# DJjjjhao/FIRA-ICSE

Measured on NVIDIA H100. Metric: train_commits_per_sec, higher is better.
Workload: dtype bf16

## Files before the change

fira_icse_b200/csrc/attention.cu:

```cuda
#include <stdlib.h>
#include "attn_mma.cuh"
#include "common.cuh"
#include "fira_b200.h"

namespace {

bool use_tc(int dtype) {
  if (dtype != FIRA_BF16) return false;
  const char* e = getenv("FIRA_ATTN_TC");
  return e ? atoi(e) != 0 : true;
}

constexpr int KPAD = DH + 1;
constexpr int NWARPS = 8;
constexpr int NTHR = NWARPS * 32;
constexpr int KC = 128;
constexpr int KCB = 64;

template <typename T>
__device__ __forceinline__ void load_rows(float* dst, const T* src, long ld, const int* rows_idx, int row0, int nrows) {
  constexpr int EPV = 16 / sizeof(T);
  constexpr int VPR = DH / EPV;
#pragma unroll 4
  for (int idx = threadIdx.x; idx < nrows * VPR; idx += NTHR) {
// ... 262 lines not shown
  for (int i = 0; i < nblk; ++i) {
    cp_async_wait<FST - 1>();
    __syncthreads();
    const unsigned char* kt = Ks + (i % FST) * FKB * ROWB;
    const unsigned char* vt = Vs + (i % FST) * FKB * ROWB;
    const int c0 = i * FKB;
    float s[8][4];
#pragma unroll
    for (int n = 0; n < 8; ++n) s[n][0] = s[n][1] = s[n][2] = s[n][3] = 0.f;
    mma_abt(s, qa, kt, lane);
    softmax_pv(s, rk, a.causal, c0, nv, k2, m, l, o, vt, lane);
    __syncthreads();
    if (i + FST < nblk)
      stage_kv(Ks + (i % FST) * FKB * ROWB, Vs + (i % FST) * FKB * ROWB, kh, a.ldk, vh, a.ldv, kidx, (i + FST) * FKB,
               min(FKB, nv - (i + FST) * FKB), FKB, threadIdx.x, blockDim.x);
    cp_async_commit();
  }
  softmax_finish(o, l, m, rk, t, a.Lq, stats ? stats + ((long)b * a.H + h) * a.Lq * 2 : nullptr, lane);
#pragma unroll
  for (int r = 0; r < 2; ++r) {
    if (t[r] >= a.Lq) continue;
    __nv_bfloat16* dst = ctx + ((long)b * a.Lq + t[r]) * ldo + h * DH + 2 * q;
#pragma unroll
    for (int n = 0; n < 4; ++n)
      *reinterpret_cast<__nv_bfloat162*>(dst + 8 * n) = __floats2bfloat162_rn(o[n][2 * r], o[n][2 * r + 1]);
  }
}

__global__ void __launch_bounds__(BWARPS * 32, 1)
attn_mma_bwd_kernel(AttnArgs a, const __nv_bfloat16* __restrict__ out, const __nv_bfloat16* __restrict__ d_ctx, long ldo,
                    const float* __restrict__ stats, __nv_bfloat16* __restrict__ dq, long lddq,
                    __nv_bfloat16* __restrict__ dk, long lddk, __nv_bfloat16* __restrict__ dv, long lddv) {
  pdl_wait(); pdl_trigger();
  extern __shared__ __align__(16) unsigned char mma_smem[];
  __shared__ int nv_s, filled_s;
  __shared__ float delta_s[LQ_MAX], m2_s[LQ_MAX], inv_s[LQ_MAX];
  unsigned char* Qs = mma_smem;
  unsigned char* Os = Qs + LQ_MAX * ROWB;
  unsigned char* Ws = Os + LQ_MAX * ROWB;
  int* kidx = reinterpret_cast<int*>(Ws + BWARPS * BWARP_SMEM);
  const int b = blockIdx.x / a.H, h = blockIdx.x % a.H;
  const int lane = threadIdx.x & 31, warp = threadIdx.x >> 5, q = lane & 3;
  const unsigned char* km = a.key_mask ? a.key_mask + (long)b * a.Lk : nullptr;
  const int* rg = a.ranges ? a.ranges + 4 * b : nullptr;
  const long kvb = rg ? 0 : (long)b * a.Lk;
  const __nv_bfloat16* kh = (const __nv_bfloat16*)a.k + kvb * a.ldk + h * DH;
  const __nv_bfloat16* vh = (const __nv_bfloat16*)a.v + kvb * a.ldv + h * DH;
  unsigned char* Kw = Ws + warp * BWARP_SMEM;
  unsigned char* Vw = Kw + BKB * ROWB;
  unsigned char* Pw = Vw + BKB * ROWB;
  unsigned char* Sw = Pw + LQ_MAX * ROWB;
  float* dQw = reinterpret_cast<float*>(Sw + LQ_MAX * ROWB);
  compact_keys(km, a.Lk, a.causal, kidx, &nv_s, &filled_s, rg);
  const int nv = nv_s;
  const bool filled = filled_s != 0;
  if (warp * BKB < nv) stage_kv(Kw, Vw, kh, a.ldk, vh, a.ldv, kidx, warp * BKB, min(BKB, nv - warp * BKB), BKB, lane, 32);
  for (int i = threadIdx.x; i < 2 * LQ_MAX * 4; i += blockDim.x) {
    const int which = i / (LQ_MAX * 4), r = (i >> 2) & (LQ_MAX - 1), c = i & 3;
    unsigned char* dst = (which ? Os : Qs) + swz(r, c);
    if (r < a.Lq) cp_async16(su32(dst), which ? d_ctx + ((long)b * a.Lq + r) * ldo + h * DH + c * 8
                                              : (const __nv_bfloat16*)a.q + ((long)b * a.Lq + r) * a.ldq + h * DH + c * 8);
    else *reinterpret_cast<uint4*>(dst) = make_uint4(0, 0, 0, 0);
  }
  cp_async_commit();
  if (threadIdx.x < a.Lq) {
    const int t = threadIdx.x;
    const __nv_bfloat16* orow = out + ((long)b * a.Lq + t) * ldo + h * DH;
    const __nv_bfloat16* grow = d_ctx + ((long)b * a.Lq + t) * ldo + h * DH;
    float d = 0.f;
#pragma unroll
    for (int c = 0; c < 4; ++c) {
      float ov[8], gv[8];
      Act<__nv_bfloat16>::load8(orow + c * 8, ov);
      Act<__nv_bfloat16>::load8(grow + c * 8, gv);
#pragma unroll
      for (int e = 0; e < 8; ++e) d = fmaf(ov[e], gv[e], d);
    }
    const float* st = stats + (((long)b * a.H + h) * a.Lq + t) * 2;
    delta_s[t] = d; m2_s[t] = st[0] * kLog2e; inv_s[t] = 1.f / st[1];
  }
  if (!filled && !a.causal && km) {
    const int L = rg ? rg[1] + rg[3] : a.Lk;
    for (int s0 = 32 * warp; s0 < L; s0 += 32 * BWARPS) {
      uint32_t dead = __ballot_sync(0xffffffffu, s0 + lane < L && km[s0 + lane] == 0);
      while (dead) {
        const int s = s0 + __ffs(dead) - 1;
        dead &= dead - 1;
        const long row = rg ? (s < rg[1] ? rg[0] + s : rg[2] + (s - rg[1])) : (long)b * a.Lk + s;
        dk[row * lddk + h * DH + lane] = __float2bfloat16_rn(0.f);
        dv[row * lddv + h * DH + lane] = __float2bfloat16_rn(0.f);
      }
    }
  }
  cp_async_wait<0>();
  __syncthreads();

  const float k2 = a.scale * kLog2e;
  const uint32_t mb = causal_mask_bits(a, km, lane);
  for (int i = lane; i < LQ_MAX * DH / 4; i += 32) reinterpret_cast<float4*>(dQw)[i] = make_float4(0.f, 0.f, 0.f, 0.f);

  for (int blk = warp; blk * BKB < nv; blk += BWARPS) {
    const int c0 = blk * BKB, nc = min(BKB, nv - c0);
    if (blk != warp) {
      __syncwarp();
      stage_kv(Kw, Vw, kh, a.ldk, vh, a.ldv, kidx, c0, nc, BKB, lane, 32);
      cp_async_commit();
      cp_async_wait<0>();
    }
    __syncwarp();
#pragma unroll
    for (int mt = 0; mt < 2; ++mt) {
// ... 72 lines not shown
#pragma unroll
      for (int kk = 0; kk < 2; ++kk) {
        if (16 * kk >= a.Lq) break;
#pragma unroll
        for (int mk = 0; mk < 2; ++mk) {
          uint32_t at[4];
          ldsm4_t(su32(At + swz(16 * kk + (lane & 7) + (lane >> 4) * 8, 2 * mk + ((lane >> 3) & 1))), at);
          mma_ax(acc[mk], at, Bt, kk, lane);
        }
      }
      __nv_bfloat16* dst = which ? dv : dk;
      const long ld = which ? lddv : lddk;
#pragma unroll
      for (int mk = 0; mk < 2; ++mk)
#pragma unroll
        for (int r = 0; r < 2; ++r) {
          const int j = 16 * mk + (lane >> 2) + 8 * r;
          if (j < nc) {
            __nv_bfloat16* row = dst + (kvb + kidx[c0 + j]) * ld + h * DH + 2 * q;
#pragma unroll
            for (int n = 0; n < 4; ++n)
              *reinterpret_cast<__nv_bfloat162*>(row + 8 * n) = __floats2bfloat162_rn(acc[mk][n][2 * r], acc[mk][n][2 * r + 1]);
          }
        }
    }
  }
  __syncthreads();
  for (int i = threadIdx.x; i < a.Lq * DH; i += blockDim.x) {
    const int t = i / DH, f = i % DH;
    float x = 0.f;
#pragma unroll
    for (int w = 0; w < BWARPS; ++w)
      x += reinterpret_cast<const float*>(Ws + w * BWARP_SMEM + 4 * BKB * ROWB)[swz_f32(t, f)];
    dq[((long)b * a.Lq + t) * lddq + h * DH + f] = __float2bfloat16_rn(x);
  }
}

size_t fwd_smem(int Lk) { return (size_t)2 * FST * FKB * ROWB + sizeof(int) * (size_t)Lk; }
size_t bwd_smem(int Lk) { return (size_t)2 * LQ_MAX * ROWB + (size_t)BWARPS * BWARP_SMEM + sizeof(int) * (size_t)Lk; }

}

size_t fwd_smem(int Lq, int Lk) {
  return sizeof(float) * ((size_t)2 * KC * KPAD + (size_t)Lq * KPAD + (size_t)NWARPS * 2 * KC) + sizeof(int) * (size_t)Lk;
}
size_t bwd_smem(int Lq, int Lk) {
  return sizeof(float) * ((size_t)2 * KCB * KPAD + (size_t)2 * Lq * KPAD + (size_t)2 * Lq * (KCB + 1)) +
         sizeof(int) * (size_t)Lk;
}

template <typename K>
int set_smem(K kernel, size_t bytes, const char* name) {
  if (bytes > 227 * 1024) {
    fira_set_error(FIRA_ERR_SHAPE, "%s: needs %zu B shared memory (> 227 KB)", name, bytes);
    return FIRA_ERR_SHAPE;
  }
  if (bytes > 48 * 1024) {
    cudaError_t e = cudaFuncSetAttribute(kernel, cudaFuncAttributeMaxDynamicSharedMemorySize, (int)bytes);
    if (e != cudaSuccess) { fira_set_error(FIRA_ERR_CUDA, "%s: %s", name, cudaGetErrorString(e)); return FIRA_ERR_CUDA; }
  }
  return FIRA_OK;
}

int check_layout(const char* name, const void* p, long ld, int dtype) {
  const long esz = dtype == FIRA_F32 ? 4 : 2;
  if ((reinterpret_cast<uintptr_t>(p) & 15) != 0 || (ld * esz) % 16 != 0) {
    fira_set_error(FIRA_ERR_ALIGN, "%s: operands must be 16-B aligned with 16-B row pitch", name);
// ... 10 lines not shown
                  const unsigned char* key_mask, const int* ranges, int causal, void* ctx, long ldo, float* stats, int B, int H, int Lq, int Lk, int d_head, int dtype, void* stream) {
  FIRA_CHECK_ARG(d_head == DH, FIRA_ERR_SHAPE, "attn_fwd: d_head %d != 32", d_head);
  FIRA_CHECK_ARG(B > 0 && H > 0 && Lq > 0 && Lk > 0 && Lq <= LQ_MAX, FIRA_ERR_SHAPE, "attn_fwd: shape (Lq <= 32)");
  FIRA_CHECK_ARG(!causal || (Lq == Lk && !ranges), FIRA_ERR_SHAPE, "attn_fwd: causal needs Lq == Lk and no ranges");
  FIRA_CHECK_ARG(key_mask || ranges, FIRA_ERR_ARG, "attn_fwd: key_mask may only be NULL with ranges");
  FIRA_CHECK_ARG(dtype == FIRA_F32 || dtype == FIRA_BF16, FIRA_ERR_DTYPE, "attn_fwd: dtype %d", dtype);
  int rc;
  if ((rc = check_layout("attn_fwd", q, ldq, dtype)) || (rc = check_layout("attn_fwd", k, ldk, dtype)) ||
      (rc = check_layout("attn_fwd", v, ldv, dtype)))
    return rc;
  AttnArgs a{q, ldq, k, ldk, v, ldv, key_mask, ranges, causal, B, H, Lq, Lk, 1.f / sqrtf((float)d_head)};
  if (use_tc(dtype)) {
    const size_t smem = mma::fwd_smem(Lk);
    if ((rc = set_smem(mma::attn_mma_fwd_kernel, smem, "attn_fwd"))) return rc;
    launch_k(mma::attn_mma_fwd_kernel, dim3(B * H), dim3(32 * ((Lq + 15) / 16)), smem, (cudaStream_t)stream, a,
             (__nv_bfloat16*)ctx, ldo, stats);
    FIRA_CHECK_LAUNCH("fira_attn_fwd (mma)");
    return FIRA_OK;
  }
  const size_t smem = fwd_smem(Lq, Lk);
  if (dtype == FIRA_F32) {
    if ((rc = set_smem(attn_fwd_kernel<float>, smem, "attn_fwd"))) return rc;
    launch_k(attn_fwd_kernel<float>, dim3(B * H), dim3(NTHR), smem, (cudaStream_t)stream, a, (float*)ctx, ldo, stats);
  } else {
    if ((rc = set_smem(attn_fwd_kernel<__nv_bfloat16>, smem, "attn_fwd"))) return rc;
    launch_k(attn_fwd_kernel<__nv_bfloat16>, dim3(B * H), dim3(NTHR), smem, (cudaStream_t)stream, a, (__nv_bfloat16*)ctx, ldo, stats);
  }
  FIRA_CHECK_LAUNCH("fira_attn_fwd");
  return FIRA_OK;
}

int attn_bwd_impl(const void* q, long ldq, const void* k, long ldk, const void* v, long ldv,
                  const unsigned char* key_mask, const int* ranges, int causal, const void* ctx, const void* d_ctx, long ldo, const float* stats, void* dq, long lddq, void* dk,
                  long lddk, void* dv, long lddv, int B, int H, int Lq, int Lk, int d_head, int dtype, void* stream) {
  FIRA_CHECK_ARG(d_head == DH, FIRA_ERR_SHAPE, "attn_bwd: d_head %d != 32", d_head);
  FIRA_CHECK_ARG(B > 0 && H > 0 && Lq > 0 && Lk > 0 && Lq <= LQ_MAX, FIRA_ERR_SHAPE, "attn_bwd: shape (Lq <= 32)");
  FIRA_CHECK_ARG(key_mask || ranges, FIRA_ERR_ARG, "attn_bwd: key_mask may only be NULL with ranges");
  FIRA_CHECK_ARG(dtype == FIRA_F32 || dtype == FIRA_BF16, FIRA_ERR_DTYPE, "attn_bwd: dtype %d", dtype);
  int rc;
  if ((rc = check_layout("attn_bwd", q, ldq, dtype)) || (rc = check_layout("attn_bwd", k, ldk, dtype)) ||
      (rc = check_layout("attn_bwd", v, ldv, dtype)) || (rc = check_layout("attn_bwd", ctx, ldo, dtype)) ||
      (rc = check_layout("attn_bwd", d_ctx, ldo, dtype)))
    return rc;
  AttnArgs a{q, ldq, k, ldk, v, ldv, key_mask, ranges, causal, B, H, Lq, Lk, 1.f / sqrtf((float)d_head)};
  if (use_tc(dtype) && (lddk % 8) == 0 && (lddv % 8) == 0 && (lddq % 8) == 0) {
    const size_t smem = mma::bwd_smem(Lk);
    if ((rc = set_smem(mma::attn_mma_bwd_kernel, smem, "attn_bwd"))) return rc;
    launch_k(mma::attn_mma_bwd_kernel, dim3(B * H), dim3(mma::BWARPS * 32), smem, (cudaStream_t)stream, a,
             (const __nv_bfloat16*)ctx, (const __nv_bfloat16*)d_ctx, ldo, stats, (__nv_bfloat16*)dq, lddq,
             (__nv_bfloat16*)dk, lddk, (__nv_bfloat16*)dv, lddv);
    FIRA_CHECK_LAUNCH("fira_attn_bwd (mma)");
    return FIRA_OK;
  }
  const size_t smem = bwd_smem(Lq, Lk);
  if (dtype == FIRA_F32) {
    if ((rc = set_smem(attn_bwd_kernel<float>, smem, "attn_bwd"))) return rc;
    launch_k(attn_bwd_kernel<float>, dim3(B * H), dim3(NTHR), smem, (cudaStream_t)stream, 
        a, (const float*)ctx, (const float*)d_ctx, ldo, stats, (float*)dq, lddq, (float*)dk, lddk, (float*)dv, lddv);
  } else {
    if ((rc = set_smem(attn_bwd_kernel<__nv_bfloat16>, smem, "attn_bwd"))) return rc;
    launch_k(attn_bwd_kernel<__nv_bfloat16>, dim3(B * H), dim3(NTHR), smem, (cudaStream_t)stream, 
        a, (const __nv_bfloat16*)ctx, (const __nv_bfloat16*)d_ctx, ldo, stats, (__nv_bfloat16*)dq, lddq,
        (__nv_bfloat16*)dk, lddk, (__nv_bfloat16*)dv, lddv);
  }
  FIRA_CHECK_LAUNCH("fira_attn_bwd");
  return FIRA_OK;
}

}

extern "C" {

int fira_attn_fwd(const void* q, long ldq, const void* k, long ldk, const void* v, long ldv,
                  const unsigned char* key_mask, int causal, void* ctx, long ldo, float* stats, int B, int H, int Lq,
                  int Lk, int d_head, int dtype, void* stream) {
  FIRA_CHECK_ARG(key_mask, FIRA_ERR_ARG, "attn_fwd: null key_mask");
  return attn_fwd_impl(q, ldq, k, ldk, v, ldv, key_mask, nullptr, causal, ctx, ldo, stats,
                       B, H, Lq, Lk, d_head, dtype, stream);
}

int fira_attn_bwd(const void* q, long ldq, const void* k, long ldk, const void* v, long ldv,
                  const unsigned char* key_mask, int causal, const void* ctx, const void* d_ctx, long ldo,
                  const float* stats, void* dq, long lddq, void* dk, long lddk, void* dv, long lddv, int B, int H,
                  int Lq, int Lk, int d_head, int dtype, void* stream) {
  FIRA_CHECK_ARG(key_mask, FIRA_ERR_ARG, "attn_bwd: null key_mask");
  return attn_bwd_impl(q, ldq, k, ldk, v, ldv, key_mask, nullptr, causal, ctx, d_ctx, ldo,
                       stats, dq, lddq, dk, lddk, dv, lddv, B, H, Lq, Lk, d_head, dtype, stream);
}

int fira_attn_packed_fwd(const void* q, long ldq, const void* k, long ldk, const void* v, long ldv, const int* ranges,
                         long kv_rows, const unsigned char* key_mask, int mask_pitch, int max_chunks, void* ctx, long ldo,
                         float* stats, int B, int H, int Lq, int d_head, int dtype, void* stream) {
  FIRA_CHECK_ARG(ranges && kv_rows > 0, FIRA_ERR_ARG, "attn_packed_fwd: ranges / kv_rows");
  return attn_fwd_impl(q, ldq, k, ldk, v, ldv, key_mask, ranges, 0, ctx, ldo, stats, B, H, Lq,
                       mask_pitch, d_head, dtype, stream);
}

int fira_attn_packed_bwd(const void* q, long ldq, const void* k, long ldk, const void* v, long ldv, const int* ranges,
                         long kv_rows, const unsigned char* key_mask, int mask_pitch, int max_chunks, const void* ctx,
                         const void* d_ctx, long ldo, const float* stats, void* dq, long lddq, void* dk, long lddk,
                         void* dv, long lddv, int B, int H, int Lq, int d_head, int dtype, void* stream) {
  FIRA_CHECK_ARG(ranges && kv_rows > 0, FIRA_ERR_ARG, "attn_packed_bwd: ranges / kv_rows");
  return attn_bwd_impl(q, ldq, k, ldk, v, ldv, key_mask, ranges, 0, ctx, d_ctx, ldo, stats, dq, lddq,
                       dk, lddk, dv, lddv, B, H, Lq, mask_pitch, d_head, dtype, stream);
}

}
```

fira_icse_b200/csrc/attn_mma.cuh:

```cuda
#pragma once
#include "common.cuh"

namespace {

constexpr int DH = 32;
constexpr int LQ_MAX = 32;

struct AttnArgs {
  const void* q; long ldq;
  const void* k; long ldk;
  const void* v; long ldv;
  const unsigned char* key_mask;
  const int* ranges;
  int causal;
  int B, H, Lq, Lk;
  float scale;
};

__device__ __forceinline__ void compact_keys(const unsigned char* km, int Lk, int causal, int* kidx, int* nv_out,
                                             int* filled, const int* rg = nullptr) {
  if (threadIdx.x < 32) {
    const int lane = threadIdx.x;
    const int L = rg ? rg[1] + rg[3] : Lk;
    int n = 0;
    for (int s0 = 0; s0 < L && !causal; s0 += 32) {
      const int s = s0 + lane;
      const bool ok = s < L && (km == nullptr || km[s] != 0);
      const unsigned bal = __ballot_sync(0xffffffffu, ok);
      if (ok) kidx[n + __popc(bal & ((1u << lane) - 1u))] = rg ? (s < rg[1] ? rg[0] + s : rg[2] + (s - rg[1])) : s;
      n += __popc(bal);
    }
    if (n == 0) {
      for (int s = lane; s < L; s += 32) kidx[s] = rg ? (s < rg[1] ? rg[0] + s : rg[2] + (s - rg[1])) : s;
      n = L;
      if (lane == 0) *filled = causal ? 0 : 1;
    } else if (lane == 0) *filled = 0;
    if (lane == 0) *nv_out = n;
  }
  __syncthreads();
}

namespace mma {

constexpr int ROWB = DH * 2;
constexpr float kLog2e = 1.4426950408889634f;

__device__ __forceinline__ uint32_t swz(int r, int c) { return r * ROWB + ((c ^ ((r >> 1) & 3)) << 4); }
__device__ __forceinline__ uint32_t su32(const void* p) { return (uint32_t)__cvta_generic_to_shared(p); }

// ... 157 lines not shown
```

fira_icse_b200/csrc/decoder_fwd.cu:

```cuda
#include <string.h>
#include <cooperative_groups.h>
#include "attn_mma.cuh"
#include "common.cuh"
#include "fira_b200.h"

namespace {

namespace cg = cooperative_groups;
using namespace mma;
using bf16 = __nv_bfloat16;

constexpr int D = 256, F = 1024, NH = 8;
constexpr int TP = 32;
constexpr int NWARP = 16, NTHR = NWARP * 32;
constexpr int LDA = D + 32, LDF = F + 32;
constexpr int XT = TP * LDA * 2;
constexpr int HT = TP * ROWB;
constexpr int CKB = 32;
constexpr int MAX_LAYERS = 8;

struct LayerW {
  const bf16* wqkv; const float* bqkv;
  const bf16* swo; const float* sbo; const float* slw; const float* slb;
  const bf16* cwq; const float* cbq;
  const bf16* cwo; const float* cbo; const float* clw; const float* clb;
  const bf16* w1; const float* b1; const bf16* w2; const float* b2;
  const float* flw; const float* flb;
};
static_assert(sizeof(LayerW) == 18 * sizeof(void*), "LayerW is the host's [L][18] pointer table");

struct DecParams {
  const int* tar; const float* emb; const float* pe; const unsigned char* tar_mask;
  const bf16* kv; long ldkv;
  const unsigned char* mem_mask; const int* ranges; int S;
  bf16* X;
  bf16* qkv; bf16* ctx1; float* st1; bf16* z1; float* ls1; bf16* x1;
  bf16* q; bf16* ctx2; float* st2; bf16* z2; float* ls2; bf16* x2;
  bf16* hh; bf16* z3; float* ls3;
  int B, T, L;
  float scale, p_drop;
  uint64_t seed; const uint64_t* seed_ctr; uint32_t stream_id;
  LayerW w[MAX_LAYERS];
};

constexpr int OFF_X = 0, OFF_X1 = XT, OFF_X2 = 2 * XT, OFF_Y = 3 * XT, OFF_Z = 4 * XT, OFF_BIG = 5 * XT;
constexpr int BIG_BYTES = TP * LDF * 2;
static_assert(BIG_BYTES >= 12 * HT && BIG_BYTES >= 4 * HT + 2 * 2 * 4 * CKB * ROWB,
              "the region also holds the q|k|v head tiles of four heads, and their q tiles + two K / V stages");
constexpr int SMEM_FIXED = OFF_BIG + BIG_BYTES;

__device__ __forceinline__ uint32_t word(const uint4& v, int i) { return i == 0 ? v.x : i == 1 ? v.y : i == 2 ? v.z : v.w; }
__device__ __forceinline__ uint4 ldg16(const bf16* p) { return __ldg(reinterpret_cast<const uint4*>(p)); }
__device__ __forceinline__ void pair_bar(int h) { asm volatile("bar.sync %0, 64;" ::"r"(1 + h) : "memory"); }

template <int K, int NT8, int PF>
__device__ __forceinline__ void warp_mma(float (&acc)[2][NT8][4], const bf16* As, const bf16* __restrict__ W, int n0,
                                         int lane) {
  constexpr int lda = K + 32;
  const int g = lane >> 2, q = lane & 3;
#pragma unroll
  for (int mt = 0; mt < 2; ++mt)
#pragma unroll
    for (int j = 0; j < NT8; ++j) acc[mt][j][0] = acc[mt][j][1] = acc[mt][j][2] = acc[mt][j][3] = 0.f;
  const bf16* wp = W + (long)(n0 + g) * K + 8 * q;
  const bf16* ap = As + g * lda + 8 * q;
  constexpr int nks = K / 32;
  uint4 bq[PF][NT8];
#pragma unroll
  for (int s = 0; s < PF; ++s)
#pragma unroll
    for (int j = 0; j < NT8; ++j) bq[s][j] = ldg16(wp + (long)8 * j * K + 32 * s);
// ... 33 lines not shown
  for (int n0 = 8 * NT8 * warp; n0 < N / 2; n0 += 8 * NT8 * NWARP) {
    const int c0 = gcol(n0, rank);
    float acc[2][NT8][4];
    warp_mma<K, NT8, PF>(acc, As, W, c0, lane);
#pragma unroll
    for (int j = 0; j < NT8; ++j) {
      const int n = n0 + 8 * j + 2 * q, c = c0 + 8 * j + 2 * q;
      const float2 bb = *reinterpret_cast<const float2*>(bias + c);
#pragma unroll
      for (int mt = 0; mt < 2; ++mt)
#pragma unroll
        for (int hr = 0; hr < 2; ++hr) {
          float v0 = acc[mt][j][2 * hr] + bb.x, v1 = acc[mt][j][2 * hr + 1] + bb.y;
          if (RELU) { v0 = fmaxf(v0, 0.f); v1 = fmaxf(v1, 0.f); }
          epi(16 * mt + 8 * hr + g, n, c, pack_bf16(v0, v1));
        }
    }
  }
}

__device__ __forceinline__ uint32_t head_off(int t, int n) {
  return (n >> 5) * HT + swz(t, (n & 31) >> 3) + (n & 7) * 2;
}

template <typename Src>
__device__ __forceinline__ void copy_out(bf16* __restrict__ dst, int N, int T, int rank, int warp, int lane, Src src) {
  for (int t = warp; t < T; t += NWARP)
    for (int n = 8 * lane; n < N / 2; n += 256)
      *reinterpret_cast<uint4*>(dst + (long)t * N + gcol(n, rank)) = *reinterpret_cast<const uint4*>(src(t, n));
}

__device__ __forceinline__ void ln_rows(const unsigned char* sm, int off_z, int off_res, int off_out, const float* gamma,
                                        const float* beta, bf16* __restrict__ zg, bf16* __restrict__ og,
                                        float* __restrict__ stats, long rows, long r0, int T, float p_drop, uint64_t seed,
                                        const uint64_t* seed_ctr, uint32_t sid, int rank, int warp, int lane) {
  if (seed_ctr) seed += *seed_ctr;
  float g[8], bt[8];
  Act<float>::load8(gamma + lane * 8, g);
  Act<float>::load8(beta + lane * 8, bt);
  const float keep_scale = p_drop > 0.f ? 1.f / (1.f - p_drop) : 1.f;
  for (int t = 2 * warp; t < 2 * warp + 2; ++t) {
    const int o = (t * LDA + lane * 8) * 2;
    bf16* os = (bf16*)(sm + off_out + o);
    if (t >= T) { *reinterpret_cast<uint4*>(os) = make_uint4(0, 0, 0, 0); continue; }
    const long r = r0 + t;
    const bool mine = (t & 1) == rank;
    const uint4 zraw = *reinterpret_cast<const uint4*>(sm + off_z + o);
    if (mine) *reinterpret_cast<uint4*>(zg + r * D + lane * 8) = zraw;
    float y[8], x[8];
    Act<bf16>::load8((const bf16*)&zraw, y);
    Act<bf16>::load8((const bf16*)(sm + off_res + o), x);
    if (p_drop > 0.f) {
      uint32_t m = dropout_keep8(seed, sid, (uint64_t)r * 32 + lane, p_drop);
#pragma unroll
      for (int i = 0; i < 8; ++i) y[i] = ((m >> i) & 1) ? y[i] * keep_scale : 0.f;
    }
    float s = 0.f;
#pragma unroll
    for (int i = 0; i < 8; ++i) { y[i] += x[i]; s += y[i]; }
    const float mean = warp_sum(s) * (1.f / D);
    float qv = 0.f;
#pragma unroll
    for (int i = 0; i < 8; ++i) { float d = y[i] - mean; qv += d * d; }
    const float rstd = rsqrtf(warp_sum(qv) * (1.f / D) + kLnEps);
#pragma unroll
    for (int i = 0; i < 8; ++i) y[i] = (y[i] - mean) * rstd * g[i] + bt[i];
    Act<bf16>::store8(os, y);
    if (mine) {
      *reinterpret_cast<uint4*>(og + r * D + lane * 8) = *reinterpret_cast<const uint4*>(os);
      if (lane == 0) { stats[r] = mean; stats[rows + r] = rstd; }
    }
  }
}

struct AttnRows {
  int t[2];
  RowKeys rk[2];
  float m[2], l[2], o[4][4];
  uint32_t qa[2][4];
  __device__ __forceinline__ void init(const unsigned char* qtile, int r0, int lane) {
    ld_a(qtile, r0, lane, qa);
    m[0] = m[1] = -INFINITY;
    l[0] = l[1] = 0.f;
#pragma unroll
    for (int n = 0; n < 4; ++n) o[n][0] = o[n][1] = o[n][2] = o[n][3] = 0.f;
#pragma unroll
    for (int r = 0; r < 2; ++r) t[r] = r0 + (lane >> 2) + 8 * r;
  }
  __device__ __forceinline__ void block(const unsigned char* kt, const unsigned char* vt, int causal, int c0, int nv,
                                        float k2, int lane) {
    float s[4][4];
#pragma unroll
    for (int n = 0; n < 4; ++n) s[n][0] = s[n][1] = s[n][2] = s[n][3] = 0.f;
    mma_abt(s, qa, kt, lane);
    softmax_pv(s, rk, causal, c0, nv, k2, m, l, o, vt, lane);
  }
  __device__ __forceinline__ void finish(unsigned char* ytile, unsigned char* ytile_peer, int h, int T, float* st,
                                         int lane) {
    softmax_finish(o, l, m, rk, t, T, st, lane);
#pragma unroll
    for (int r = 0; r < 2; ++r)
#pragma unroll
      for (int n = 0; n < 4; ++n) {
        const int off = (t[r] * LDA + h * DH + 8 * n + 2 * (lane & 3)) * 2;
        const uint32_t v = pack_bf16(o[n][2 * r], o[n][2 * r + 1]);
        *reinterpret_cast<uint32_t*>(ytile + off) = v;
        *reinterpret_cast<uint32_t*>(ytile_peer + off) = v;
      }
  }
};

__global__ void __cluster_dims__(2, 1, 1) __launch_bounds__(NTHR, 1)
decoder_fwd_kernel(const __grid_constant__ DecParams p) {
  pdl_wait(); pdl_trigger();
  extern __shared__ __align__(16) unsigned char sm[];
  __shared__ int nv_s, filled_s;
  cg::cluster_group cluster = cg::this_cluster();
  const int rank = (int)cluster.block_rank();
  unsigned char* peer = cluster.map_shared_rank(sm, rank ^ 1);
  const int b = blockIdx.x >> 1, T = p.T;
  const int lane = threadIdx.x & 31, warp = threadIdx.x >> 5, hl = (warp >> 1) & 3, r0q = 16 * (warp & 1);
  const long Mt = (long)p.B * T, grow0 = (long)b * T;
  int* kidx = reinterpret_cast<int*>(sm + SMEM_FIXED);
  bf16* Xs = (bf16*)(sm + OFF_X);
  bf16* Ys = (bf16*)(sm + OFF_Y);
  unsigned char* big = sm + OFF_BIG;
  auto to_both = [&](int off, uint32_t v) {
    *reinterpret_cast<uint32_t*>(sm + off) = v;
    *reinterpret_cast<uint32_t*>(peer + off) = v;
  };

  compact_keys(p.mem_mask ? p.mem_mask + (long)b * p.S : nullptr, p.S, 0, kidx, &nv_s, &filled_s,
               p.ranges ? p.ranges + 4 * b : nullptr);

  for (int t = warp; t < TP; t += NWARP) {
    float v[8];
    if (t < T) {
      float pe[8];
      Act<float>::load8(p.emb + (long)p.tar[grow0 + t] * D + lane * 8, v);
      Act<float>::load8(p.pe + (long)t * D + lane * 8, pe);
#pragma unroll
      for (int i = 0; i < 8; ++i) v[i] += pe[i];
      if ((t & 1) == rank) Act<bf16>::store8(p.X + (grow0 + t) * D + lane * 8, v);
    } else {
#pragma unroll
      for (int i = 0; i < 8; ++i) v[i] = 0.f;
    }
    Act<bf16>::store8(Xs + t * LDA + lane * 8, v);
  }
  cluster.sync();

  for (int i = 0; i < p.L; ++i) {
    const LayerW& w = p.w[i];
    const long o256 = i * Mt * D;

    product<D, 1, 8, false>(Xs, w.wqkv, w.bqkv, 3 * D, rank, warp, lane,
                            [&](int t, int n, int, uint32_t v) { *reinterpret_cast<uint32_t*>(big + head_off(t, n)) = v; });
    __syncthreads();
    copy_out(p.qkv + (i * Mt + grow0) * 3 * D, 3 * D, T, rank, warp, lane, [&](int t, int n) { return big + head_off(t, n); });
    if (warp < 8) {
      AttnArgs sa{};
      sa.causal = 1;
      sa.Lk = T;
      const uint32_t mb = causal_mask_bits(sa, p.tar_mask + grow0, lane);
      AttnRows ar;
      ar.init(big + hl * HT, r0q, lane);
#pragma unroll
      for (int r = 0; r < 2; ++r) ar.rk[r] = row_keys(sa, mb, T, false, ar.t[r]);
      ar.block(big + (4 + hl) * HT, big + (8 + hl) * HT, 1, 0, T, p.scale * kLog2e, lane);
      const int h = 4 * rank + hl;
      ar.finish(sm + OFF_Y, peer + OFF_Y, h, T, p.st1 + (((long)i * p.B + b) * NH + h) * T * 2, lane);
    }
    cluster.sync();
    copy_out(p.ctx1 + o256 + grow0 * D, D, T, rank, warp, lane, [&](int t, int n) { return Ys + t * LDA + gcol(n, rank); });
    product<D, 1, 8, false>(Ys, w.swo, w.sbo, D, rank, warp, lane,
                            [&](int t, int, int c, uint32_t v) { to_both(OFF_Z + (t * LDA + c) * 2, v); });
    cluster.sync();
    ln_rows(sm, OFF_Z, OFF_X, OFF_X1, w.slw, w.slb, p.z1 + o256, p.x1 + o256, p.ls1 + 2 * i * Mt, Mt, grow0, T,
            p.p_drop, p.seed, p.seed_ctr, p.stream_id + 8 * i + 0, rank, warp, lane);
    __syncthreads();

    product<D, 1, 8, false>((const bf16*)(sm + OFF_X1), w.cwq, w.cbq, D, rank, warp, lane,
                            [&](int t, int n, int, uint32_t v) { *reinterpret_cast<uint32_t*>(big + head_off(t, n)) = v; });
    __syncthreads();
    copy_out(p.q + o256 + grow0 * D, D, T, rank, warp, lane, [&](int t, int n) { return big + head_off(t, n); });
    if (warp < 8) {
      const int h = 4 * rank + hl;
      const int nv = nv_s, nblk = (nv + CKB - 1) / CKB;
      const float k2 = p.scale * kLog2e;
      const long kvb = p.ranges ? 0 : (long)b * p.S;
      const bf16* kh = p.kv + kvb * p.ldkv + (long)i * 2 * D + h * DH;
      const bf16* vh = kh + D;
      unsigned char* stage = big + 4 * HT;
      auto kt = [&](int s) { return stage + ((s * 2 + 0) * 4 + hl) * CKB * ROWB; };
      auto vt = [&](int s) { return stage + ((s * 2 + 1) * 4 + hl) * CKB * ROWB; };
      const int tid = threadIdx.x & 63;
#pragma unroll
      for (int s = 0; s < 2; ++s) {
        if (s < nblk) stage_kv(kt(s), vt(s), kh, p.ldkv, vh, p.ldkv, kidx, s * CKB, min(CKB, nv - s * CKB), CKB, tid, 64);
        cp_async_commit();
      }
      AttnRows ar;
      ar.init(big + hl * HT, r0q, lane);
      ar.rk[0] = ar.rk[1] = RowKeys{0u, filled_s != 0};
      for (int blk = 0; blk < nblk; ++blk) {
        cp_async_wait<1>();
        pair_bar(hl);
        ar.block(kt(blk & 1), vt(blk & 1), 0, blk * CKB, nv, k2, lane);
        pair_bar(hl);
        if (blk + 2 < nblk)
          stage_kv(kt(blk & 1), vt(blk & 1), kh, p.ldkv, vh, p.ldkv, kidx, (blk + 2) * CKB,
                   min(CKB, nv - (blk + 2) * CKB), CKB, tid, 64);
        cp_async_commit();
      }
      ar.finish(sm + OFF_Y, peer + OFF_Y, h, T, p.st2 + (((long)i * p.B + b) * NH + h) * T * 2, lane);
    }
    cluster.sync();
    copy_out(p.ctx2 + o256 + grow0 * D, D, T, rank, warp, lane, [&](int t, int n) { return Ys + t * LDA + gcol(n, rank); });
    product<D, 1, 8, false>(Ys, w.cwo, w.cbo, D, rank, warp, lane,
                            [&](int t, int, int c, uint32_t v) { to_both(OFF_Z + (t * LDA + c) * 2, v); });
    cluster.sync();
    ln_rows(sm, OFF_Z, OFF_X1, OFF_X2, w.clw, w.clb, p.z2 + o256, p.x2 + o256, p.ls2 + 2 * i * Mt, Mt, grow0, T,
            p.p_drop, p.seed, p.seed_ctr, p.stream_id + 8 * i + 1, rank, warp, lane);
    __syncthreads();

    bf16* Hs = (bf16*)big;
    product<D, 2, 4, true>((const bf16*)(sm + OFF_X2), w.w1, w.b1, F, rank, warp, lane,
                           [&](int t, int, int c, uint32_t v) { to_both(OFF_BIG + (t * LDF + c) * 2, v); });
    cluster.sync();
    copy_out(p.hh + (i * Mt + grow0) * F, F, T, rank, warp, lane, [&](int t, int n) { return Hs + t * LDF + gcol(n, rank); });
    product<F, 1, 8, false>(Hs, w.w2, w.b2, D, rank, warp, lane,
                            [&](int t, int, int c, uint32_t v) { to_both(OFF_Z + (t * LDA + c) * 2, v); });
    cluster.sync();
    ln_rows(sm, OFF_Z, OFF_X2, OFF_X, w.flw, w.flb, p.z3 + o256, p.X + o256 + Mt * D, p.ls3 + 2 * i * Mt, Mt, grow0, T,
            p.p_drop, p.seed, p.seed_ctr, p.stream_id + 8 * i + 2, rank, warp, lane);
    __syncthreads();
  }
}

}

extern "C" int fira_decoder_fwd(const int* tar, const float* dec_emb, const float* pos_table,
                                const unsigned char* tar_mask, const void* kv, long ldkv, const unsigned char* mem_mask,
                                const int* ranges, int S, const void* const* layer_ptrs, int L, void* X, void* qkv,
                                void* ctx1, float* st1, void* z1, float* ls1, void* x1, void* q, void* ctx2, float* st2,
                                void* z2, float* ls2, void* x2, void* hh, void* z3, float* ls3, int B, int T,
                                float p_drop, uint64_t seed, const uint64_t* seed_ctr, uint32_t stream_id,
                                void* stream) {
  FIRA_CHECK_ARG(B > 0 && T > 0 && T <= TP, FIRA_ERR_SHAPE, "decoder_fwd: B %d, T %d (T <= 32)", B, T);
  FIRA_CHECK_ARG(L > 0 && L <= MAX_LAYERS, FIRA_ERR_SHAPE, "decoder_fwd: %d layers (1..%d)", L, MAX_LAYERS);
  FIRA_CHECK_ARG(S > 0, FIRA_ERR_SHAPE, "decoder_fwd: S %d", S);
  FIRA_CHECK_ARG(mem_mask || ranges, FIRA_ERR_ARG, "decoder_fwd: mem_mask may only be NULL with ranges");
  FIRA_CHECK_ARG(layer_ptrs && tar && dec_emb && pos_table && tar_mask && kv, FIRA_ERR_ARG, "decoder_fwd: null input");
  FIRA_CHECK_ARG(fira_aligned16(kv) && ldkv % 8 == 0 && ldkv >= (long)L * 2 * D, FIRA_ERR_ALIGN,
                 "decoder_fwd: kv must be 16-B aligned with ldkv a multiple of 8 and >= L*512");
  void* outs[] = {X, qkv, ctx1, z1, x1, q, ctx2, z2, x2, hh, z3};
  for (void* o : outs) FIRA_CHECK_ARG(o && fira_aligned16(o), FIRA_ERR_ALIGN, "decoder_fwd: outputs must be 16-B aligned");
  FIRA_CHECK_ARG(st1 && ls1 && st2 && ls2 && ls3, FIRA_ERR_ARG, "decoder_fwd: null statistics");
  DecParams p{tar, dec_emb, pos_table, tar_mask, (const bf16*)kv, ldkv, mem_mask, ranges, S,
              (bf16*)X, (bf16*)qkv, (bf16*)ctx1, st1, (bf16*)z1, ls1, (bf16*)x1,
              (bf16*)q, (bf16*)ctx2, st2, (bf16*)z2, ls2, (bf16*)x2, (bf16*)hh, (bf16*)z3, ls3,
              B, T, L, 1.f / sqrtf((float)DH), p_drop, seed, seed_ctr, stream_id, {}};
  for (int i = 0; i < L; ++i) {
    const void* const* t = layer_ptrs + 18 * i;
    for (int j = 0; j < 18; ++j)
      FIRA_CHECK_ARG(t[j] && fira_aligned16(t[j]), FIRA_ERR_ALIGN, "decoder_fwd: layer %d pointer %d null or unaligned", i, j);
    memcpy(&p.w[i], t, sizeof(LayerW));
  }
  const size_t smem = SMEM_FIXED + sizeof(int) * (size_t)S;
  FIRA_CHECK_ARG(smem <= 227 * 1024, FIRA_ERR_SHAPE, "decoder_fwd: S %d needs %zu B shared memory", S, smem);
  cudaError_t e = cudaFuncSetAttribute(decoder_fwd_kernel, cudaFuncAttributeMaxDynamicSharedMemorySize, (int)smem);
  if (e != cudaSuccess) { fira_set_error(FIRA_ERR_CUDA, "decoder_fwd: %s", cudaGetErrorString(e)); return FIRA_ERR_CUDA; }
  launch_k(decoder_fwd_kernel, dim3(2 * B), dim3(NTHR), smem, (cudaStream_t)stream, p);
  FIRA_CHECK_LAUNCH("fira_decoder_fwd");
  return FIRA_OK;
}
```

fira_icse_b200/csrc/head.cu:

```cuda
#include "common.cuh"
#include "fira_b200.h"

namespace {

constexpr int D = 256;
constexpr int TMAX = 32;

__device__ __forceinline__ long src_row(const int* __restrict__ ranges, int b, int S, int s) {
  if (!ranges) return (long)b * S + s;
  const int* r = ranges + 4 * b;
  if (s < r[1]) return r[0] + s;
  s -= r[1];
  return s < r[3] ? (long)(r[2] + s) : -1;
}

template <typename T>
__global__ void __launch_bounds__(256) copy_scores_fwd_kernel(const T* __restrict__ src, const T* __restrict__ tgt,
                                                              const float* __restrict__ w_res,
                                                              const float* __restrict__ b_res_p,
                                                              const unsigned char* __restrict__ src_mask,
                                                              const unsigned char* __restrict__ row_mask,
                                                              const int* __restrict__ ranges,
                                                              float* __restrict__ sc, int B, int Tn, int S) {
  pdl_wait(); pdl_trigger();
// ... 143 lines not shown
    u.s = __shfl_xor_sync(0xffffffffu, v.s, o);
    v = ms_merge(v, u);
  }
  return v;
}
struct ArgMax { float v; int i; };
__device__ __forceinline__ ArgMax am_better(ArgMax a, ArgMax b) {
  return (b.v > a.v || (b.v == a.v && b.i < a.i)) ? b : a;
}

constexpr int kRowsThreads = 1024;
__global__ void __launch_bounds__(kRowsThreads) vocab_rows_kernel(const int* __restrict__ label, long rows, int V,
                                                                  int* __restrict__ vslot, int* __restrict__ vrows,
                                                                  int cap) {
  pdl_wait(); pdl_trigger();
  __shared__ int warp_sum_s[kRowsThreads / 32];
  const int lane = threadIdx.x & 31, warp = threadIdx.x >> 5;
  const long per = (rows + kRowsThreads - 1) / kRowsThreads;
  const long r0 = min(rows, (long)threadIdx.x * per), r1 = min(rows, r0 + per);
  int n = 0;
  for (long r = r0; r < r1; ++r) n += (label[r] != 0 && label[r] < V);
  int incl = n;
#pragma unroll
  for (int o = 1; o < 32; o <<= 1) { const int u = __shfl_up_sync(0xffffffffu, incl, o); if (lane >= o) incl += u; }
  if (lane == 31) warp_sum_s[warp] = incl;
  for (int s = threadIdx.x; s < cap; s += kRowsThreads) vrows[s] = -1;
  __syncthreads();
  int slot = incl - n;
  for (int w = 0; w < warp; ++w) slot += warp_sum_s[w];
  for (long r = r0; r < r1; ++r) {
    const bool v = label[r] != 0 && label[r] < V && slot < cap;
    vslot[r] = v ? slot : -1;
    if (v) vrows[slot++] = (int)r;
  }
}

template <typename T>
__global__ void __launch_bounds__(256) gather_rows_kernel(const T* __restrict__ src, long ld_src,
                                                          const int* __restrict__ idx, T* __restrict__ dst, long ld_dst,
                                                          long n, int width) {
  pdl_wait(); pdl_trigger();
  const int lane = threadIdx.x & 31;
  for (long i = (long)blockIdx.x * 8 + (threadIdx.x >> 5); i < n; i += (long)gridDim.x * 8) {
    const int r = idx[i];
    for (int c = lane * 8; c < width; c += 256) {
      float x[8] = {0.f, 0.f, 0.f, 0.f, 0.f, 0.f, 0.f, 0.f};
      if (r >= 0) Act<T>::load8(src + (long)r * ld_src + c, x);
      Act<T>::store8(dst + i * ld_dst + c, x);
    }
  }
}

template <typename T>
__global__ void __launch_bounds__(256) head_fwd_kernel(const T* __restrict__ logits, long ldl,
                                                       const float* __restrict__ sc, const float* __restrict__ gate_logit,
                                                       const unsigned char* __restrict__ mem_mask,
                                                       const int* __restrict__ label, const int* __restrict__ vslot,
                                                       float* __restrict__ stats, float* __restrict__ nll,
                                                       int* __restrict__ argmax_out, int Tn, int V, int S) {
  pdl_wait(); pdl_trigger();
  __shared__ MaxSum sh_ms[8];
  __shared__ ArgMax sh_am[8];
  __shared__ float bc[8];
  const long row = blockIdx.x;
  const int b = (int)(row / Tn);
  const int lane = threadIdx.x & 31, warp = threadIdx.x >> 5;
// ... 775 lines not shown
                         const unsigned char* src_mask, const unsigned char* row_mask, float* scores,
                         int B, int T_len, int S, int dim, int dtype, void* stream) {
  return copy_scores_fwd_impl(src_proj, tgt_proj, w_res, b_res, src_mask, row_mask, nullptr, scores, B, T_len, S, dim,
                              dtype, stream);
}

int fira_copy_scores_bwd(const void* src_proj, const void* tgt_proj, const float* w_res, const float* d_scores,
                         const unsigned char* row_active, void* d_src_proj, float* d_tgt_proj, float* d_w_res,
                         float* d_b_res, int B, int T_len, int S, int dim, int dtype, void* stream) {
  return copy_scores_bwd_impl(src_proj, tgt_proj, w_res, d_scores, row_active, nullptr, d_src_proj, d_tgt_proj, d_w_res,
                              d_b_res, B, T_len, S, dim, dtype, stream);
}

int fira_copy_scores_packed_fwd(const void* src_proj, const void* tgt_proj, const float* w_res, const float* b_res,
                                const int* ranges, const unsigned char* src_mask, const unsigned char* row_mask,
                                float* scores, int B, int T_len, int S, int dim, int dtype, void* stream) {
  FIRA_CHECK_ARG(ranges, FIRA_ERR_ARG, "copy_scores_packed_fwd: null ranges");
  return copy_scores_fwd_impl(src_proj, tgt_proj, w_res, b_res, src_mask, row_mask, ranges, scores, B, T_len, S, dim,
                              dtype, stream);
}

int fira_copy_scores_packed_bwd(const void* src_proj, const void* tgt_proj, const float* w_res, const float* d_scores,
                                const unsigned char* row_active, const int* ranges, void* d_src_proj, float* d_tgt_proj,
                                float* d_w_res, float* d_b_res, int B, int T_len, int S, int dim, int dtype, void* stream) {
  FIRA_CHECK_ARG(ranges, FIRA_ERR_ARG, "copy_scores_packed_bwd: null ranges");
  return copy_scores_bwd_impl(src_proj, tgt_proj, w_res, d_scores, row_active, ranges, d_src_proj, d_tgt_proj, d_w_res,
                              d_b_res, B, T_len, S, dim, dtype, stream);
}

int fira_vocab_rows(const int* label, long rows, int V, int* vslot, int* vrows, int cap, void* stream) {
  FIRA_CHECK_ARG(label && vslot && vrows && rows >= 0 && V > 0 && cap >= 0, FIRA_ERR_ARG, "vocab_rows: arguments");
  launch_k(vocab_rows_kernel, dim3(1), dim3(kRowsThreads), 0, (cudaStream_t)stream, label, rows, V, vslot, vrows, cap);
  FIRA_CHECK_LAUNCH("fira_vocab_rows");
  return FIRA_OK;
}

int fira_gather_rows(const void* src, long ld_src, const int* idx, void* dst, long ld_dst, long n, int width, int dtype,
                     void* stream) {
  FIRA_CHECK_ARG(idx && n >= 0 && width > 0 && width % 8 == 0 && ld_src >= width && ld_dst >= width, FIRA_ERR_ARG,
                 "gather_rows: arguments");
  FIRA_CHECK_ARG(fira_aligned16(src) && fira_aligned16(dst) && ld_src % 8 == 0 && ld_dst % 8 == 0, FIRA_ERR_ALIGN,
                 "gather_rows: 16-B alignment");
  if (n == 0) return FIRA_OK;
  const long g = (n + 7) / 8, gmax = (long)fira_num_sms() * 16;
  DISPATCH_T(dtype, launch_k(gather_rows_kernel<T>, dim3((unsigned)(g < gmax ? g : gmax)), dim3(256), 0,
      (cudaStream_t)stream, (const T*)src, ld_src, idx, (T*)dst, ld_dst, n, width);)
  FIRA_CHECK_LAUNCH("fira_gather_rows");
  return FIRA_OK;
}

int fira_pointer_mix_nll_fwd_rows(const void* logits, long ld_logits, const float* copy_scores, const float* gate_logits,
                                  const unsigned char* mem_mask, const int* label, const int* vslot, float* stats,
                                  float* nll, int* argmax_out, long rows, int T_len, int V, int S, int dtype,
                                  void* stream) {
  FIRA_CHECK_ARG(rows >= 0 && T_len > 0 && V > 0 && S > 0, FIRA_ERR_SHAPE, "pointer_mix_nll_fwd: shape");
  FIRA_CHECK_ARG(fira_aligned16(logits) && ld_logits % 8 == 0, FIRA_ERR_ALIGN,
                 "pointer_mix_nll_fwd: logits must be 16-byte aligned with a leading dimension that is a multiple of 8");
  FIRA_CHECK_ARG(!(vslot && argmax_out), FIRA_ERR_ARG, "pointer_mix_nll_fwd: the argmax needs the logits of every row");
  if (rows == 0) return FIRA_OK;
  DISPATCH_T(dtype, launch_k(head_fwd_kernel<T>, dim3((unsigned)rows), dim3(256), 0, (cudaStream_t)stream,
      (const T*)logits, ld_logits, copy_scores, gate_logits, mem_mask, label, vslot, stats, nll, argmax_out, T_len, V,
      S);)
  FIRA_CHECK_LAUNCH("fira_pointer_mix_nll_fwd");
  return FIRA_OK;
}

// ... 289 lines not shown
```

fira_icse_b200/csrc/rowops.cu:

```cuda
#include "common.cuh"
#include "fira_b200.h"

namespace {

constexpr int D = 256;
constexpr int ROWS_PER_CTA = 8;
constexpr int CTA = ROWS_PER_CTA * kWarp;

__host__ inline int row_grid(long rows) {
  long g = (rows + ROWS_PER_CTA - 1) / ROWS_PER_CTA;
  const long cap = (long)fira_num_sms() * 16;
  return (int)(g < cap ? (g > 0 ? g : 1) : cap);
}

template <typename T>
__global__ void embed_nodes_kernel(const int* __restrict__ sou, const int* __restrict__ sub, const int* __restrict__ ast,
                                   const float* __restrict__ emb, const float* __restrict__ ast_emb,
                                   const float* __restrict__ pe, const int* __restrict__ pos_idx,
                                   T* __restrict__ out_code, T* __restrict__ out_rest, int B, int n_code, int n_sub,
                                   int n_ast) {
  pdl_wait(); pdl_trigger();
  const long R = (long)B * (n_code + n_sub + n_ast);
  const int lane = threadIdx.x & 31;
  for (long r = (long)blockIdx.x * ROWS_PER_CTA + (threadIdx.x >> 5); r < R; r += (long)gridDim.x * ROWS_PER_CTA) {
// ... 24 lines not shown
                                       float* __restrict__ d_ast_emb, int B, int n_code, int n_sub, int n_ast) {
  pdl_wait(); pdl_trigger();
  const long R = (long)B * (n_code + n_sub + n_ast);
  const int lane = threadIdx.x & 31;
  for (long r = (long)blockIdx.x * ROWS_PER_CTA + (threadIdx.x >> 5); r < R; r += (long)gridDim.x * ROWS_PER_CTA) {
    int id; float* dst; const T* g;
    if (r < (long)B * n_code) { id = sou[r]; dst = d_emb; g = d_code + r * D; }
    else if (r < (long)B * (n_code + n_sub)) { id = sub[r - (long)B * n_code]; dst = d_emb; g = d_rest + r * D; }
    else { id = ast[r - (long)B * (n_code + n_sub)]; dst = d_ast_emb; g = d_rest + r * D; }
    if (id == 0) continue;
    float v[8];
    Act<T>::load8(g + lane * 8, v);
    float* o = dst + (long)id * D + lane * 8;
    atomicAdd(reinterpret_cast<float4*>(o), make_float4(v[0], v[1], v[2], v[3]));
    atomicAdd(reinterpret_cast<float4*>(o + 4), make_float4(v[4], v[5], v[6], v[7]));
  }
}

template <typename T>
__global__ void embed_rows_kernel(const int* __restrict__ ids, const float* __restrict__ emb,
                                  const float* __restrict__ pe, T* __restrict__ out, long rows, int period) {
  pdl_wait(); pdl_trigger();
  const int lane = threadIdx.x & 31;
  for (long r = (long)blockIdx.x * ROWS_PER_CTA + (threadIdx.x >> 5); r < rows; r += (long)gridDim.x * ROWS_PER_CTA) {
    float v[8], q[8];
    Act<float>::load8(emb + (long)ids[r] * D + lane * 8, v);
    Act<float>::load8(pe + (r % period) * D + lane * 8, q);
#pragma unroll
    for (int i = 0; i < 8; ++i) v[i] += q[i];
    Act<T>::store8(out + r * D + lane * 8, v);
  }
}
template <typename T>
__global__ void embed_rows_bwd_kernel(const int* __restrict__ ids, const T* __restrict__ g, float* __restrict__ d_emb,
                                      long rows) {
  pdl_wait(); pdl_trigger();
  const int lane = threadIdx.x & 31;
  for (long r = (long)blockIdx.x * ROWS_PER_CTA + (threadIdx.x >> 5); r < rows; r += (long)gridDim.x * ROWS_PER_CTA) {
    float v[8];
    Act<T>::load8(g + r * D + lane * 8, v);
    bool nz = false;
#pragma unroll
    for (int i = 0; i < 8; ++i) nz |= v[i] != 0.f;
    if (!__any_sync(0xffffffffu, nz)) continue;
    float* o = d_emb + (long)ids[r] * D + lane * 8;
    atomicAdd(reinterpret_cast<float4*>(o), make_float4(v[0], v[1], v[2], v[3]));
    atomicAdd(reinterpret_cast<float4*>(o + 4), make_float4(v[4], v[5], v[6], v[7]));
  }
}

template <typename T>
__global__ void ln_fwd_kernel(const T* __restrict__ z, const T* __restrict__ resid, const float* __restrict__ gamma,
                              const float* __restrict__ beta, T* __restrict__ outA, T* __restrict__ outB, long split,
                              float* __restrict__ mean_out, float* __restrict__ rstd_out, long rows, float p_drop,
                              uint64_t seed, const uint64_t* __restrict__ seed_ctr, uint32_t stream_id) {
  pdl_wait(); pdl_trigger();
  if (seed_ctr) seed += *seed_ctr;
  const int lane = threadIdx.x & 31;
  float g[8], bt[8];
  Act<float>::load8(gamma + lane * 8, g);
  Act<float>::load8(beta + lane * 8, bt);
  const float keep_scale = p_drop > 0.f ? 1.f / (1.f - p_drop) : 1.f;
  for (long r = (long)blockIdx.x * ROWS_PER_CTA + (threadIdx.x >> 5); r < rows; r += (long)gridDim.x * ROWS_PER_CTA) {
    float y[8], x[8];
    Act<T>::load8(z + r * D + lane * 8, y);
    Act<T>::load8(resid + r * D + lane * 8, x);
    if (p_drop > 0.f) {
      uint32_t m = dropout_keep8(seed, stream_id, (uint64_t)r * 32 + lane, p_drop);
#pragma unroll
      for (int i = 0; i < 8; ++i) y[i] = ((m >> i) & 1) ? y[i] * keep_scale : 0.f;
    }
    float s = 0.f;
#pragma unroll
    for (int i = 0; i < 8; ++i) { y[i] += x[i]; s += y[i]; }
    const float mean = warp_sum(s) * (1.f / D);
    float q = 0.f;
#pragma unroll
    for (int i = 0; i < 8; ++i) { float d = y[i] - mean; q += d * d; }
    const float rstd = rsqrtf(warp_sum(q) * (1.f / D) + kLnEps);
#pragma unroll
    for (int i = 0; i < 8; ++i) y[i] = (y[i] - mean) * rstd * g[i] + bt[i];
    T* dst = (r < split ? outA : outB) + r * D + lane * 8;
    Act<T>::store8(dst, y);
    if (lane == 0 && mean_out) { mean_out[r] = mean; rstd_out[r] = rstd; }
  }
}

template <typename T>
__global__ void ln_bwd_kernel(const T* __restrict__ doutA, const T* __restrict__ doutB, long split,
                              const T* __restrict__ z, const T* __restrict__ resid, const float* __restrict__ mean_in,
                              const float* __restrict__ rstd_in, const float* __restrict__ gamma, T* __restrict__ d_z,
                              T* __restrict__ d_resid, int d_resid_accum, float* __restrict__ d_gamma,
                              float* __restrict__ d_beta, long rows, float p_drop, uint64_t seed,
                              const uint64_t* __restrict__ seed_ctr, uint32_t stream_id) {
  pdl_wait(); pdl_trigger();
  if (seed_ctr) seed += *seed_ctr;
  __shared__ __align__(16) float red[2][ROWS_PER_CTA][D];
  const int lane = threadIdx.x & 31, warp = threadIdx.x >> 5;
  float g[8], dg[8], db[8];
  Act<float>::load8(gamma + lane * 8, g);
#pragma unroll
  for (int i = 0; i < 8; ++i) { dg[i] = 0.f; db[i] = 0.f; }
  const float keep_scale = p_drop > 0.f ? 1.f / (1.f - p_drop) : 1.f;
  for (long r = (long)blockIdx.x * ROWS_PER_CTA + warp; r < rows; r += (long)gridDim.x * ROWS_PER_CTA) {
    float y[8], x[8], go[8];
    Act<T>::load8(z + r * D + lane * 8, y);
    Act<T>::load8(resid + r * D + lane * 8, x);
    Act<T>::load8((r < split ? doutA : doutB) + r * D + lane * 8, go);
    uint32_t m = 0xffu;
    if (p_drop > 0.f) {
      m = dropout_keep8(seed, stream_id, (uint64_t)r * 32 + lane, p_drop);
#pragma unroll
      for (int i = 0; i < 8; ++i) y[i] = ((m >> i) & 1) ? y[i] * keep_scale : 0.f;
    }
    const float mean = mean_in[r], rstd = rstd_in[r];
    float s1 = 0.f, s2 = 0.f;
#pragma unroll
    for (int i = 0; i < 8; ++i) {
      float xh = (y[i] + x[i] - mean) * rstd;
      float dxh = go[i] * g[i];
      dg[i] += go[i] * xh; db[i] += go[i];
      s1 += dxh; s2 += dxh * xh;
      y[i] = xh; x[i] = dxh;
    }
    s1 = warp_sum(s1) * (1.f / D);
    s2 = warp_sum(s2) * (1.f / D);
    float dy[8], dz[8];
#pragma unroll
    for (int i = 0; i < 8; ++i) {
      dy[i] = rstd * (x[i] - s1 - y[i] * s2);
      dz[i] = ((m >> i) & 1) ? dy[i] * keep_scale : 0.f;
    }
    Act<T>::store8(d_z + r * D + lane * 8, dz);
    if (d_resid) {
      if (d_resid_accum) {
        float old[8];
        Act<T>::load8(d_resid + r * D + lane * 8, old);
#pragma unroll
        for (int i = 0; i < 8; ++i) dy[i] += old[i];
      }
      Act<T>::store8(d_resid + r * D + lane * 8, dy);
    }
  }
#pragma unroll
// ... 304 lines not shown
  return FIRA_OK;
}

int fira_zero_pad_rows(void* x, long ld, int width, const int* off, int B, int Rc, int Rs, int dtype, void* stream) {
  FIRA_CHECK_ARG(x && off && B > 0 && width > 0 && width % 8 == 0 && ld >= width, FIRA_ERR_ARG, "zero_pad_rows: arguments");
  FIRA_CHECK_ARG(fira_aligned16(x) && (ld % 8) == 0, FIRA_ERR_ALIGN, "zero_pad_rows: 16-B alignment");
  DISPATCH_T(dtype, launch_k(zero_pad_rows_kernel<T>, dim3(fira_num_sms()), dim3(256), 0, (cudaStream_t)stream, (T*)x, ld, width, off, B, Rc, Rs);)
  FIRA_CHECK_LAUNCH("fira_zero_pad_rows");
  return FIRA_OK;
}

int fira_embed_nodes_bwd(const int* sou, const int* sub_token, const int* ast_change, const void* d_code,
                         const void* d_rest, float* d_emb, float* d_ast_emb, int B, int n_code, int n_sub, int n_ast,
                         int dim, int dtype, void* stream) {
  FIRA_CHECK_ARG(dim == D, FIRA_ERR_SHAPE, "embed_nodes_bwd: dim %d != 256", dim);
  const long R = (long)B * (n_code + n_sub + n_ast);
  DISPATCH_T(dtype, launch_k(embed_nodes_bwd_kernel<T>, dim3(row_grid(R)), dim3(CTA), 0, (cudaStream_t)stream, 
      sou, sub_token, ast_change, (const T*)d_code, (const T*)d_rest, d_emb, d_ast_emb, B, n_code, n_sub, n_ast);)
  FIRA_CHECK_LAUNCH("fira_embed_nodes_bwd");
  return FIRA_OK;
}

int fira_embed_rows_fwd(const int* ids, const float* emb, const float* pos_table, void* out, long rows, int period,
                        int dim, int dtype, void* stream) {
  FIRA_CHECK_ARG(dim == D, FIRA_ERR_SHAPE, "embed_rows: dim %d != 256", dim);
  FIRA_CHECK_ARG(period > 0, FIRA_ERR_SHAPE, "embed_rows: period");
  DISPATCH_T(dtype, launch_k(embed_rows_kernel<T>, dim3(row_grid(rows)), dim3(CTA), 0, (cudaStream_t)stream, ids, emb, pos_table,
                                                                                         (T*)out, rows, period);)
  FIRA_CHECK_LAUNCH("fira_embed_rows_fwd");
  return FIRA_OK;
}

int fira_embed_rows_bwd(const int* ids, const void* d_out, float* d_emb, long rows, int dim, int dtype, void* stream) {
  FIRA_CHECK_ARG(dim == D, FIRA_ERR_SHAPE, "embed_rows_bwd: dim %d != 256", dim);
  DISPATCH_T(dtype, launch_k(embed_rows_bwd_kernel<T>, dim3(row_grid(rows)), dim3(CTA), 0, (cudaStream_t)stream, ids, (const T*)d_out,
                                                                                             d_emb, rows);)
  FIRA_CHECK_LAUNCH("fira_embed_rows_bwd");
  return FIRA_OK;
}

int fira_ln_residual_fwd(const void* z, const void* resid, const float* gamma, const float* beta, void* outA,
                         void* outB, long split, float* mean, float* rstd, long rows, int dim, float p_drop,
                         uint64_t seed, const uint64_t* seed_ctr, uint32_t stream_id, int dtype, void* stream) {
  FIRA_CHECK_ARG(dim == D, FIRA_ERR_SHAPE, "ln_residual_fwd: dim %d != 256", dim);
  FIRA_CHECK_ARG(p_drop >= 0.f && p_drop < 1.f, FIRA_ERR_ARG, "ln_residual_fwd: p_drop %f", p_drop);
  FIRA_CHECK_ARG(fira_aligned16(z) && fira_aligned16(resid) && fira_aligned16(outA) && fira_aligned16(outB),
                 FIRA_ERR_ALIGN, "ln_residual_fwd: 16-B alignment");
  if (rows == 0) return FIRA_OK;
  DISPATCH_T(dtype, launch_k(ln_fwd_kernel<T>, dim3(row_grid(rows)), dim3(CTA), 0, (cudaStream_t)stream, 
      (const T*)z, (const T*)resid, gamma, beta, (T*)outA, (T*)outB, split, mean, rstd, rows, p_drop, seed, seed_ctr, stream_id);)
  FIRA_CHECK_LAUNCH("fira_ln_residual_fwd");
  return FIRA_OK;
}

int fira_ln_residual_bwd(const void* d_outA, const void* d_outB, long split, const void* z, const void* resid,
                         const float* mean, const float* rstd, const float* gamma, void* d_z, void* d_resid,
                         int d_resid_accum, float* d_gamma, float* d_beta, long rows, int dim, float p_drop,
                         uint64_t seed, const uint64_t* seed_ctr, uint32_t stream_id, int dtype, void* stream) {
  FIRA_CHECK_ARG(dim == D, FIRA_ERR_SHAPE, "ln_residual_bwd: dim %d != 256", dim);
  if (rows == 0) return FIRA_OK;
  long g = (rows + ROWS_PER_CTA - 1) / ROWS_PER_CTA;
  int grid = (int)(g < (long)fira_num_sms() * 4 ? g : (long)fira_num_sms() * 4);
  DISPATCH_T(dtype, launch_k(ln_bwd_kernel<T>, dim3(grid), dim3(CTA), 0, (cudaStream_t)stream, 
      (const T*)d_outA, (const T*)d_outB, split, (const T*)z, (const T*)resid, mean, rstd, gamma, (T*)d_z,
      (T*)d_resid, d_resid_accum, d_gamma, d_beta, rows, p_drop, seed, seed_ctr, stream_id);)
  FIRA_CHECK_LAUNCH("fira_ln_residual_bwd");
  return FIRA_OK;
}

int fira_comb_gate_fwd(const void* qk, long ld_qk, const float* vtab, const int* mark, void* out, long rows, int dim,
                       int d_head, float p_drop, uint64_t seed, const uint64_t* seed_ctr, uint32_t stream_id, int dtype, void* stream) {
  FIRA_CHECK_ARG(dim == D, FIRA_ERR_SHAPE, "comb_gate_fwd: dim %d != 256", dim);
  FIRA_CHECK_ARG(ld_qk >= 2 * D && (ld_qk % 8) == 0, FIRA_ERR_SHAPE, "comb_gate_fwd: ld_qk %ld", ld_qk);
  if (rows == 0) return FIRA_OK;
  const float scale = 1.f / sqrtf((float)d_head);
  DISPATCH_T(dtype, launch_k(comb_gate_fwd_kernel<T>, dim3(row_grid(rows)), dim3(CTA), 0, (cudaStream_t)stream, 
      (const T*)qk, ld_qk, vtab, mark, (T*)out, rows, scale, p_drop, seed, seed_ctr, stream_id);)
  FIRA_CHECK_LAUNCH("fira_comb_gate_fwd");
  return FIRA_OK;
}

int fira_comb_gate_bwd(const void* qk, long ld_qk, const float* vtab, const int* mark, const void* d_out, void* d_qk,
                       float* d_vtab, long rows, int dim, int d_head, float p_drop, uint64_t seed, const uint64_t* seed_ctr,
                       uint32_t stream_id, int dtype, void* stream) {
  FIRA_CHECK_ARG(dim == D, FIRA_ERR_SHAPE, "comb_gate_bwd: dim %d != 256", dim);
  if (rows == 0) return FIRA_OK;
  const float scale = 1.f / sqrtf((float)d_head);
  long g = (rows + ROWS_PER_CTA - 1) / ROWS_PER_CTA;
  int grid = (int)(g < (long)fira_num_sms() * 4 ? g : (long)fira_num_sms() * 4);
  DISPATCH_T(dtype, launch_k(comb_gate_bwd_kernel<T>, dim3(grid), dim3(CTA), 0, (cudaStream_t)stream, 
      (const T*)qk, ld_qk, vtab, mark, (const T*)d_out, (T*)d_qk, d_vtab, rows, scale, p_drop, seed, seed_ctr, stream_id);)
  FIRA_CHECK_LAUNCH("fira_comb_gate_bwd");
  return FIRA_OK;
}

int fira_comb_gate3_fwd(const void* q, const void* k, const void* v, void* out, long rows, int dim, int d_head,
                        float p_drop, uint64_t seed, const uint64_t* seed_ctr, uint32_t stream_id, int dtype, void* stream) {
  FIRA_CHECK_ARG(dim == D, FIRA_ERR_SHAPE, "comb_gate3_fwd: dim %d != 256", dim);
// ... 68 lines not shown
```

fira_icse_b200/data.py:

```python
import json
import os
import random

import numpy as np
import torch
from torch.utils.data import Dataset

from ._lib import host_call

num_train, num_valid, num_test = 75000, 8000, 7661
lemmatization = {"added": "add", "fixed": "fix", "removed": "remove",
                 "adding": "add", "fixing": "fix", "removing": "remove"}
RAW_FILES = ["difftoken", "diffatt", "diffmark", "msg", "variable", "change", "ast",
             "edge_change_code", "edge_change_ast", "edge_ast_code", "edge_ast"]


def _lower(tok, upper):
    return tok if tok in upper else tok.lower()


def _to_ids(tokens, vocab, upper):
    out = []
    for t in tokens:
        t = _lower(t, upper)
# ... 245 lines not shown


class _Slot:

    def __init__(self, B, lens, msg_len, edge_cap, pin):
        n0, n1, n2 = lens

        def buf(n, dt):
            t = torch.empty(n, dtype=dt)
            return t.pin_memory() if pin else t
        self.sou, self.mark = buf(B * n0, torch.int64), buf(B * n0, torch.int64)
        self.sub_token, self.ast_change = buf(B * n1, torch.int64), buf(B * n2, torch.int64)
        self.tar, self.tar_label = buf(B * msg_len, torch.int64), buf(B * msg_len, torch.int64)
        self.rowptr = buf(B * (n0 + n1 + n2) + 1, torch.int32)
        self.col, self.val = buf(edge_cap, torch.int32), buf(edge_cap, torch.float32)
        self.event = None
        self.batch = None


class PackedBatchLoader:

    def __init__(self, dataset, batch_size, vocab_size, shuffle=False, indices=None, multiples=(8, 8, 8),
                 max_shapes=None, drop_last=False, prefetch=2, pin=None, bucket=0, packed=False, row_buckets=None):
        self.ds, self.B, self.V = dataset, int(batch_size), int(vocab_size)
        self.shuffle, self.drop_last = shuffle, drop_last
        self.bucket = int(bucket)
        self.indices = np.arange(len(dataset), dtype=np.int64) if indices is None else np.asarray(indices, np.int64)
        if len(self.indices) and (self.indices.min() < 0 or self.indices.max() >= len(dataset)):
            raise IndexError(f"PackedBatchLoader: indices must lie in [0, {len(dataset)}) "
                             f"(got {int(self.indices.min())}..{int(self.indices.max())}); the native gather does not "
                             "bounds-check")
        self.multiples = (0, 0, 0) if multiples is None else tuple(int(m) for m in multiples)
        self.max_shapes = max_shapes
        self.shapes = {}
        self.lens = (dataset.diff_len, dataset.sub_token_len, dataset.ast_change_len)
        self.msg_len = dataset.msg_len
        d = dataset.d
        self.tab = {k: np.ascontiguousarray(d[k], dtype=np.int32) for k in TransDataset.ID_KEYS}
        self.deg = np.ascontiguousarray(d["deg"], dtype=np.uint8)
        self.col = np.ascontiguousarray(d["col"], dtype=np.int16)
        self.val = np.ascontiguousarray(d["val"], dtype=np.float64)
        self.edge_ptr = np.ascontiguousarray(d["edge_ptr"], dtype=np.int64)
        self.size = sum((self.tab[k] != 0).sum(1) for k in ("sou", "sub_token", "ast_change"))
        per_commit = int(np.diff(self.edge_ptr).max()) if len(self.edge_ptr) > 1 else 0
        self.edge_cap = max(1, per_commit * self.B)
        self.pin = torch.cuda.is_available() if pin is None else pin
        self.n_slots = max(2, int(prefetch) + 1)
        self.packed = bool(packed)
        if self.packed:
            from . import packed as P
            self.tables = P.PackedTables(dataset)
            self.row_buckets = tuple(row_buckets) if row_buckets else P.SEGMENT_BUCKETS
            self.slots = [P.PackedSlot(self.B, self.lens, self.msg_len, self.edge_cap, self.pin)
                          for _ in range(self.n_slots)]
        else:
            self.slots = [_Slot(self.B, self.lens, self.msg_len, self.edge_cap, self.pin) for _ in range(self.n_slots)]

    def __len__(self):
        n = len(self.indices)
        return n // self.B if self.drop_last else -(-n // self.B)

    def _choose_dims(self, need):
        need = tuple(int(x) for x in need)
        if need in self.shapes or self.max_shapes is None or len(self.shapes) < self.max_shapes:
            self.shapes[need] = self.shapes.get(need, 0) + 1
            return need
        fits = [s for s in self.shapes if all(a >= b for a, b in zip(s, need))]
        if self.packed and not fits:
            self.shapes[need] = 1
            return need
        best = min(fits, key=sum) if fits else self.lens
        self.shapes[best] = self.shapes.get(best, 0) + 1
        return best

    def gather(self, index, slot=None):
        slot = self.slots[0] if slot is None else slot
        index = np.ascontiguousarray(index, dtype=np.int64)
        if self.packed:
            from . import packed as P
            want = P.packed_needs(self.tables, index, self.V, self.row_buckets)
            return P.gather_packed(self.tables, index, self.V, slot, pad_dims=self._choose_dims(want))
        b = len(index)
        n0, n1, n2 = self.lens
        t = self.tab
        dims = np.zeros(3, np.int32)
        host_call("fira_host_batch_dims", t["sou"].ctypes.data, t["sub_token"].ctypes.data,
                  t["ast_change"].ctypes.data, index.ctypes.data, b, n0, n1, n2, *self.multiples, dims.ctypes.data)
        dims = np.asarray(self._choose_dims(dims), np.int32)
        nnz = np.zeros(1, np.int32)
        host_call("fira_host_gather_batch", t["sou"].ctypes.data, t["tar"].ctypes.data, t["mark"].ctypes.data,
                  t["ast_change"].ctypes.data, t["tar_label"].ctypes.data, t["sub_token"].ctypes.data,
                  self.deg.ctypes.data, self.col.ctypes.data, self.val.ctypes.data, self.edge_ptr.ctypes.data,
                  index.ctypes.data, b, n0, n1, n2, self.msg_len, self.V, dims.ctypes.data,
                  slot.sou.data_ptr(), slot.tar.data_ptr(), slot.mark.data_ptr(), slot.ast_change.data_ptr(),
                  slot.tar_label.data_ptr(), slot.sub_token.data_ptr(), slot.rowptr.data_ptr(), slot.col.data_ptr(),
                  slot.val.data_ptr(), self.edge_cap, nnz.ctypes.data)
        c0, c1, c2 = (int(x) for x in dims)
        e = int(nnz[0])
        slot.batch = [slot.sou[:b * c0].view(b, c0), slot.tar[:b * self.msg_len].view(b, self.msg_len), None,
                      slot.mark[:b * c0].view(b, c0), slot.ast_change[:b * c2].view(b, c2),
                      (slot.rowptr[:b * (c0 + c1 + c2) + 1], slot.col[:e], slot.val[:e]),
                      slot.tar_label[:b * self.msg_len].view(b, self.msg_len), slot.sub_token[:b * c1].view(b, c1)]
        return slot.batch

    def epoch_batches(self):
# ... 69 lines not shown
```

fira_icse_b200/engine.py:

```python
import os

import torch
import torch.distributed as dist

from . import optim as _optim
from .graph import PackedEdges
from .optim import FlatAdam
from .packed import PackedBatch
from .parallel import FlatGradBucket

ID_KEYS = ("sou", "tar", "mark", "ast_change", "tar_label", "sub_token")


class _Captured:

    def __init__(self, shapes, B, n_nodes, cap, dev):
        self.ids = {k: torch.zeros((B, n), dtype=torch.int64, device=dev) for k, n in zip(ID_KEYS, shapes)}
        self.rowptr = torch.zeros(B * n_nodes + 1, dtype=torch.int32, device=dev)
        self.col = torch.zeros(cap, dtype=torch.int32, device=dev)
        self.val = torch.zeros(cap, dtype=torch.float32, device=dev)
        self.B, self.n_nodes, self.cap = B, n_nodes, cap
        self.graph = None
        self.grads = None


class _CapturedPacked:

    def __init__(self, pb, cap, dev):
        def z(t, n=None):
            return torch.zeros(t.shape if n is None else (n,), dtype=t.dtype, device=dev)
        t = {k: z(getattr(pb, k)) for k in PackedBatch.FIELDS if k not in ("col", "val")}
        t["col"], t["val"] = z(pb.col, cap), z(pb.val, cap)
        self.pb = PackedBatch(pb.B, pb.Rc, pb.Rs, pb.Ra, pb.S, pb.T, cap, pb.chunks, pb.Rv, **t)
        self.B, self.cap = pb.B, cap
        self.graph = None
        self.grads = None
        self.packed = True

    def copy_from(self, pb):
        for k in PackedBatch.FIELDS:
            src, dst = getattr(pb, k), getattr(self.pb, k)
            if k in ("col", "val"):
                dst[:src.numel()].copy_(src, non_blocking=True)
            else:
                dst.copy_(src, non_blocking=True)


class _OptimizerPair:

    def __init__(self, pair):
        self.pair = pair

    def step(self):
        for o in self.pair:
            o.step()

    def zero_grad(self, set_to_none=True):
        for o in self.pair:
            o.zero_grad(set_to_none=set_to_none)

    def state_dict(self):
        return [o.state_dict() for o in self.pair]


class GraphedTrainStep:
    def __init__(self, model, batch_size, optimizer_factory, edge_capacity=None, group=None, split=None):
# ... 316 lines not shown
```

fira_icse_b200/model.py:

```python
import os

import torch
import torch.nn as nn

from . import ops
from . import optim as _optim
from .modules import Decoder, Encoder, _i32, _u8


class _OutFc(nn.Linear):

    def forward(self, x):
        return ops.LinearFn.apply(x, self.weight, self.bias)


class CopyNet(nn.Module):

    def __init__(self, args):
        super().__init__()
        self.embedding_size = args.embedding_dim
        self.LinearSource = nn.Linear(self.embedding_size, self.embedding_size, bias=False)
        self.LinearTarget = nn.Linear(self.embedding_size, self.embedding_size, bias=False)
        self.LinearRes = nn.Linear(self.embedding_size, 1)
        self.LinearProb = nn.Linear(self.embedding_size, 2)
# ... 39 lines not shown
        dead = {id(p) for p in self.dead_parameters()}
        return [p for p in self.parameters() if id(p) not in dead]

    def flat_groups(self):
        g = []
        for comb, gcn in zip(self.encoder.combination_list2, self.encoder.gcn_list):
            l = comb.linear_layers
            g += [[l[0].weight, l[1].weight], [l[0].bias, l[1].bias], [comb.layernorm.weight, comb.layernorm.bias],
                  [gcn.layernorm.weight, gcn.layernorm.bias]]
        dec = self.decoder
        for a, c, f in zip(dec.attention_list, dec.cross_attention_list, dec.feed_forward_list):
            g += [[a.fc_q.weight, a.fc_k.weight, a.fc_v.weight], [a.fc_q.bias, a.fc_k.bias, a.fc_v.bias],
                  [a.layernorm.weight, a.layernorm.bias], [c.layernorm.weight, c.layernorm.bias],
                  [f.layernorm.weight, f.layernorm.bias]]
        g.append([t for c in dec.cross_attention_list for t in (c.fc_k.weight, c.fc_v.weight)])
        g.append([t for c in dec.cross_attention_list for t in (c.fc_k.bias, c.fc_v.bias)])
        return g

    @staticmethod
    def shifted_label(tar_label):
        pad = torch.zeros((tar_label.shape[0], 1), dtype=tar_label.dtype, device=tar_label.device)
        return torch.cat((tar_label[:, 1:], pad), dim=1)

    def forward_packed(self, pb, stage="train"):
        bf16 = self.precision == "bf16"
        if bf16:
            _optim.ensure_fresh(self)
        self.decoder.prefetch_weights()
        pf_head = ops.prefetch_head(bf16, self.out_fc.weight, self.copy_net.LinearSource.weight,
                                    self.copy_net.LinearTarget.weight)
        memory = self.encoder.encode_memory_packed(pb)
        if self._memory_hook is not None:
            memory = self._memory_hook(memory)
        dec = self.decoder(pb.tar, memory, pb.mem_mask, pb.tar_mask, packed=pb)
        want_ids = stage != "train"
        loss_sum, _, ids = ops.HeadFn.apply(want_ids, bf16, pf_head, memory, dec, pb.mem_mask, pb.label.view(-1),
                                            self.out_fc.weight, self.out_fc.bias, *self.copy_net.flat_params(), pb)
        if stage == "train":
            return loss_sum, (pb.label != 0).sum()
        elif stage == "dev" or stage == "test":
            return ids.long()
        raise ValueError(f"unknown stage {stage!r}")

    def forward(self, sou, tar, attr, mark, ast_change, edge, tar_label, sub_token, stage="train"):
        dev = self.out_fc.weight.device
        sou, tar, mark, ast_change, tar_label, sub_token = (
            t.to(dev, non_blocking=True) for t in (sou, tar, mark, ast_change, tar_label, sub_token))
        mem_mask = torch.cat((sou != 0, sub_token != 0), dim=1)
        bf16 = self.precision == "bf16"
        if bf16:
            _optim.ensure_fresh(self)
        self.decoder.prefetch_weights()
        pf_head = ops.prefetch_head(bf16, self.out_fc.weight, self.copy_net.LinearSource.weight,
                                    self.copy_net.LinearTarget.weight) if sou.is_cuda else None
        memory = self.encoder.encode_memory(sou, mark, ast_change, edge, sub_token)
        if self._memory_hook is not None:
            memory = self._memory_hook(memory)
        dec = self.decoder(tar, memory, mem_mask, tar != 0)
        label = self.shifted_label(tar_label)
        want_ids = stage != "train"
        loss_sum, _, ids = ops.HeadFn.apply(want_ids, bf16, pf_head, memory, dec, _u8(mem_mask),
                                            _i32(label).view(-1),
                                            self.out_fc.weight, self.out_fc.bias, *self.copy_net.flat_params())
        if stage == "train":
            return loss_sum, (label != 0).sum()
        elif stage == "dev" or stage == "test":
            return ids.long()
        raise ValueError(f"unknown stage {stage!r}")
# ... 1 lines not shown
```

fira_icse_b200/modules.py:

```python
import math

import torch
import torch.nn as nn

from . import ops
from .graph import PackedEdges


def position_encoding(length, dmodel):
    inv = [10000 ** (2 * j / dmodel) for j in range(dmodel // 2)]
    rows = []
    for i in range(length):
        row = [0.0] * dmodel
        for j, f in enumerate(inv):
            a = i / f
            row[2 * j] = math.sin(a)
            row[2 * j + 1] = math.cos(a)
        rows.append(row)
    return torch.tensor(rows)


def _i32(t):
    return t.to(torch.int32).contiguous()

# ... 168 lines not shown
    def forward(self, input_token, sou_mask, attr, mark, ast_change, edge, sub_token):
        memory = self.encode_memory(input_token, mark, ast_change, edge, sub_token)
        n_code = input_token.shape[1]
        return memory[:, :n_code], memory[:, n_code:]


class Decoder(nn.Module):

    def __init__(self, args, pad_token_id):
        super().__init__()
        self.embedding_dim = args.embedding_dim
        self.num_head = args.num_head
        self.pad_token_id = pad_token_id
        self.embedding = nn.Embedding(num_embeddings=args.vocab_size, embedding_dim=args.embedding_dim)
        self.pos_encode = position_encoding(args.tar_len, self.embedding_dim)
        self.tar_mask_pos = torch.tril(torch.ones(args.tar_len, args.tar_len))
        self.attention_list = nn.ModuleList(
            [Attention(dmodel=args.embedding_dim, num_head=args.num_head) for _ in range(6)])
        self.cross_attention_list = nn.ModuleList(
            [Attention(dmodel=args.embedding_dim, num_head=args.num_head) for _ in range(6)])
        self.feed_forward_list = nn.ModuleList([FeedForward(args.embedding_dim) for _ in range(6)])

    def _flat(self):
        lp = []
        for a, c, f in zip(self.attention_list, self.cross_attention_list, self.feed_forward_list):
            lp += a.flat_params() + c.flat_params() + f.flat_params()
        return lp

    def prefetch_weights(self):
        dev = self.embedding.weight.device
        if dev.type == "cuda":
            self._prefetched = ops.prefetch_decoder(bool(getattr(self, "bf16", False)), self._flat(), dev)

    def forward(self, output_token, input_em, sou_mask, tar_mask_pad, packed=None):
        dev = self.embedding.weight.device
        if self.pos_encode.device != dev:
            self.pos_encode = self.pos_encode.to(dev)
        cfg = _run_cfg(self)
        cfg.update(p_dec=self.attention_list[0].dropout.p, prefetch=getattr(self, "_prefetched", None), packed=packed)
        self._prefetched = None
        lp = self._flat()
        return ops.DecoderFn.apply(cfg, _i32(output_token), input_em, _u8(sou_mask), _u8(tar_mask_pad),
                                   self.pos_encode, self.embedding.weight, *lp)
```

fira_icse_b200/ops.py:

```python
import ctypes
import os

import torch

from . import _lib
from . import optim as _optim
from ._lib import FIRA_BF16, FIRA_F32, call

D = 256

if hasattr(torch.autograd.graph, "set_warn_on_accumulate_grad_stream_mismatch"):
    torch.autograd.graph.set_warn_on_accumulate_grad_stream_mismatch(False)


def _stream():
    return torch.cuda.current_stream().cuda_stream


def _ptr(t, off=0):
    if t is None:
        return None
    return t.data_ptr() + off * t.element_size()


# ... 145 lines not shown
            out = torch.empty((M, K), dtype=torch.bfloat16, device=dy.device)
            call("fira_gemm_bf16_tc_dx_relu", _ptr(dy), ld_dy, _ptr(self.w(W)), K, _ptr(out), K, _ptr(h), M, K, N, _stream())
            return out
        out = self.linear_dx(dy, ld_dy, W, M)
        call("fira_relu_bwd", _ptr(h), _ptr(out), M * K, self.code, _stream())
        return out

    def linear_dw(self, dy, ld_dy, x, ldx, M, N, K, dy_off=0, x_off=0, out=None, dbias=None):
        if not self.bf16:
            if dbias is not None:
                colsum(dy, ld_dy, M, N, x_off=dy_off, out=dbias)
            return linear_dw(dy, ld_dy, x, ldx, M, N, K, dy_off=dy_off, x_off=x_off, out=out)
        dW = torch.empty((N, K), dtype=torch.float32, device=dy.device) if out is None else out
        bn = 256 if K > 128 else (128 if K > 64 else 64)
        splits = _tc_splits(_ceil(N, 128) * _ceil(K, bn), _ceil(M, 64))
        if dbias is not None and os.environ.get("FIRA_DBIAS_FUSED", "1") != "0":
            call("fira_gemm_bf16_tc_dbias", _ptr(dy, dy_off), ld_dy, _ptr(x, x_off), ldx, 0, _ptr(dW), K, 0, N, K, M, 0, splits,
                 _ptr(dbias), _stream())
            return dW
        if dbias is not None:
            colsum(dy, ld_dy, M, N, x_off=dy_off, out=dbias)
        return gemm_tc(dy, ld_dy, 0, x, ldx, 0, dW, K, N, K, M, splits=splits, a_off=dy_off, b_off=x_off)

    def linear_ln(self, x, W, b, resid, gamma, beta, outA, outB, split, rows, p, seed, sid, rs=None, rc=None):
        z = self.linear(x, W, b, rs=rs, rc=rc, M=rows)
        return z, self.ln_fwd(z, resid, gamma, beta, outA, outB, split, rows, p, seed, sid)

    def ln_fwd(self, z, resid, gamma, beta, outA, outB, split, rows, p, seed, sid):
        stats = torch.empty((2, rows), dtype=torch.float32, device=z.device)
        call("fira_ln_residual_fwd", _ptr(z), _ptr(resid), _ptr(gamma), _ptr(beta), _ptr(outA), _ptr(outB), split,
             _ptr(stats), _ptr(stats, rows), rows, D, float(p), seed, _ptr(self.seed_ctr), sid, self.code, _stream())
        return stats

    def ln_bwd(self, dA, dB, split, z, resid, stats, gamma, rows, p, seed, sid, d_resid=None, accum=False, beta=None):
        dz = torch.empty_like(z)
        if d_resid is None:
            d_resid = torch.empty_like(z)
        dgb = _gdest((gamma, beta), (2, D), zero=True) if beta is not None else \
            torch.zeros((2, D), dtype=torch.float32, device=z.device)
        call("fira_ln_residual_bwd", _ptr(dA), _ptr(dB), split, _ptr(z), _ptr(resid), _ptr(stats), _ptr(stats, rows),
             _ptr(gamma), _ptr(dz), _ptr(d_resid), int(accum), _ptr(dgb), _ptr(dgb, D), rows, D, float(p), seed,
             _ptr(self.seed_ctr), sid, self.code, _stream())
        return dz, d_resid, dgb[0], dgb[1]


_F32 = Prec(False)


def ln_fwd(z, resid, gamma, beta, outA, outB, split, rows, p, seed, sid):
    return _F32.ln_fwd(z, resid, gamma, beta, outA, outB, split, rows, p, seed, sid)


def ln_bwd(dA, dB, split, z, resid, stats, gamma, rows, p, seed, sid, d_resid=None, accum=False):
    return _F32.ln_bwd(dA, dB, split, z, resid, stats, gamma, rows, p, seed, sid, d_resid=d_resid, accum=accum)


_SIDE_STREAMS = {}
N_SIDE = max(1, int(os.environ.get("FIRA_SIDE_STREAMS", "8")))
FUSE_DX_RELU = os.environ.get("FIRA_DX_RELU", "1") != "0" and os.environ.get("FIRA_GEMM_TMA_STORE", "1") != "0"
MERGE_SPLITS = max(1, int(os.environ.get("FIRA_MERGE_SPLITS", "4")))
_TURN = [0]


class Fork:

    def __init__(self, device, n_side=None):
        self.main = torch.cuda.current_stream(device)
        key = (device.index if device.index is not None else torch.cuda.current_device())
        if key not in _SIDE_STREAMS:
            _SIDE_STREAMS[key] = [torch.cuda.Stream(device=device) for _ in range(N_SIDE)]
        self.sides = _SIDE_STREAMS[key][:n_side] if n_side else _SIDE_STREAMS[key]
        self.side = self.sides[0]
        self.keep = []
        self.used = set()

# ... 278 lines not shown
class DecoderFn(torch.autograd.Function):

    @staticmethod
    def forward(ctx, cfg, tar, memory, mem_mask, tar_mask, pos_table, dec_emb, *lp):
        _require_cuda(tar, memory, dec_emb)
        B, T = tar.shape
        pk = cfg.get("packed")
        S = pk.S if pk is not None else memory.shape[1]
        Mt, Ms = B * T, memory.shape[0] * memory.shape[1]
        L = len(lp) // DEC_LAYER_PARAMS
        H = cfg["heads"]
        training, seed = cfg["training"], cfg["seed"]
        p = cfg["p_dec"] if training else 0.0
        pr = Prec(cfg.get("bf16", False), seed_ctr=cfg.get("seed_ctr"))
        dev = dec_emb.device
        f32 = dict(dtype=torch.float32, device=dev)
        st = _stream()
        mem_dtype = memory.dtype
        memory = memory.contiguous().to(pr.tdt)

        if not pr.bf16:
            X = pr.empty((Mt, D), dev)
            call("fira_embed_rows_fwd", _ptr(tar), _ptr(dec_emb), _ptr(pos_table), _ptr(X), Mt, T, D, pr.code, st)
        pf = cfg.get("prefetch")
        if pf is None:
            pf = prefetch_decoder(pr.bf16, lp, dev)
        torch.cuda.current_stream().wait_event(pf.event)
        pf.fork.join()
        pr.wcache.update(pf.wcache)
        Wkv, bkv, qkv_layers = pf.items
        ldkv = L * 2 * D
        KV = pr.linear(memory.view(Ms, D), Wkv, bkv)
        if pr.bf16:
            bf = dict(dtype=torch.bfloat16, device=dev)
            Xs = torch.empty((L + 1, Mt, D), **bf)
            QKV, Hh = torch.empty((L, Mt, 3 * D), **bf), torch.empty((L, Mt, 4 * D), **bf)
            ctx1, Z1, X1, Q, ctx2, Z2, X2, Z3 = torch.empty((8, L, Mt, D), **bf)
            st1, st2 = torch.empty((2, L, B, H, T, 2), **f32)
            ls1, ls2, ls3 = torch.empty((3, L, 2, Mt), **f32)
            call("fira_decoder_fwd", _ptr(tar), _ptr(dec_emb), _ptr(pos_table), _ptr(tar_mask), _ptr(KV), ldkv,
                 _ptr(mem_mask), _ptr(pk.ranges) if pk is not None else None, S, ctypes.addressof(pf.layer_table), L,
                 _ptr(Xs), _ptr(QKV), _ptr(ctx1), _ptr(st1), _ptr(Z1), _ptr(ls1), _ptr(X1), _ptr(Q), _ptr(ctx2),
                 _ptr(st2), _ptr(Z2), _ptr(ls2), _ptr(X2), _ptr(Hh), _ptr(Z3), _ptr(ls3), B, T, float(p), seed,
                 _ptr(pr.seed_ctr), cfg["stream_base"] + 64, st)
            ctx.saved = [(Xs[i], qkv_layers[i][0], QKV[i], ctx1[i], st1[i], Z1[i], ls1[i], X1[i], Q[i], ctx2[i], st2[i],
                          Z2[i], ls2[i], X2[i], Hh[i], Z3[i], ls3[i]) for i in range(L)]
            ctx.wcache = pr.wcache
            ctx.misc = (cfg, tar, memory, mem_mask, tar_mask, KV, Wkv, B, T, S, p, mem_dtype, Ms)
            ctx.save_for_backward(dec_emb, *lp)
            return Xs[L].view(B, T, D)
        saved = []
        for i in range(L):
            (sWq, sbq, sWk, sbk, sWv, sbv, sWo, sbo, slw, slb,
             cWq, cbq, cWk, cbk, cWv, cbv, cWo, cbo, clw, clb,
             fW1, fb1, fW2, fb2, flw, flb) = lp[i * 26:(i + 1) * 26]
            sid = cfg["stream_base"] + 64 + i * 8
            Wqkv, bqkv = qkv_layers[i]
            QKV = pr.linear(X, Wqkv, bqkv)
            ctx1 = pr.empty((Mt, D), dev)
            st1 = torch.empty((B, H, T, 2), **f32)
            call("fira_attn_fwd", _ptr(QKV), 3 * D, _ptr(QKV, D), 3 * D, _ptr(QKV, 2 * D), 3 * D, _ptr(tar_mask), 1,
                 _ptr(ctx1), D, _ptr(st1), B, H, T, T, D // H, pr.code, st)
            X1 = pr.empty((Mt, D), dev)
            Z1, ls1 = pr.linear_ln(ctx1, sWo, sbo, X, slw, slb, X1, X1, Mt, Mt, p, seed, sid + 0)
            Q = pr.linear(X1, cWq, cbq)
            ctx2 = pr.empty((Mt, D), dev)
            st2 = torch.empty((B, H, T, 2), **f32)
            if pk is not None:
                call("fira_attn_packed_fwd", _ptr(Q), D, _ptr(KV, i * 2 * D), ldkv, _ptr(KV, i * 2 * D + D), ldkv,
                     _ptr(pk.ranges), Ms, _ptr(mem_mask), S, pk.chunks, _ptr(ctx2), D, _ptr(st2), B, H, T, D // H, pr.code, st)
            else:
                call("fira_attn_fwd", _ptr(Q), D, _ptr(KV, i * 2 * D), ldkv, _ptr(KV, i * 2 * D + D), ldkv,
                     _ptr(mem_mask), 0, _ptr(ctx2), D, _ptr(st2), B, H, T, S, D // H, pr.code, st)
            X2 = pr.empty((Mt, D), dev)
            Z2, ls2 = pr.linear_ln(ctx2, cWo, cbo, X1, clw, clb, X2, X2, Mt, Mt, p, seed, sid + 1)
            Hh = pr.linear(X2, fW1, fb1, relu=True)
            X3 = pr.empty((Mt, D), dev)
            Z3, ls3 = pr.linear_ln(Hh, fW2, fb2, X2, flw, flb, X3, X3, Mt, Mt, p, seed, sid + 2)
            saved.append((X, Wqkv, QKV, ctx1, st1, Z1, ls1, X1, Q, ctx2, st2, Z2, ls2, X2, Hh, Z3, ls3))
            X = X3
        ctx.saved = saved
        ctx.wcache = pr.wcache
        ctx.misc = (cfg, tar, memory, mem_mask, tar_mask, KV, Wkv, B, T, S, p, mem_dtype, Ms)
        ctx.save_for_backward(dec_emb, *lp)
        return X.view(B, T, D)

    @staticmethod
    def backward(ctx, d_out):
        cfg, tar, memory, mem_mask, tar_mask, KV, Wkv, B, T, S, p, mem_dtype, Ms = ctx.misc
        dec_emb, *lp = ctx.saved_tensors
        Mt = B * T
        pk = cfg.get("packed")
        L = len(lp) // DEC_LAYER_PARAMS
        H, seed = cfg["heads"], cfg["seed"]
        pr = Prec(cfg.get("bf16", False), ctx.wcache, seed_ctr=cfg.get("seed_ctr"))
        dev = dec_emb.device
        st = _stream()
        ldkv = L * 2 * D
        dX = d_out.contiguous().to(pr.tdt).view(Mt, D)
        dKV = pr.empty((Ms, ldkv), dev)
        if pk is not None:
            call("fira_zero_pad_rows", _ptr(dKV), ldkv, ldkv, _ptr(pk.off), B, pk.Rc, pk.Rs, pr.code, st)
        grads = [None] * len(lp)
        F = 4 * D
        fork = Fork(dev)
        for i in reversed(range(L)):
            (sWq, sbq, sWk, sbk, sWv, sbv, sWo, sbo, slw, slb,
             cWq, cbq, cWk, cbk, cWv, cbv, cWo, cbo, clw, clb,
             fW1, fb1, fW2, fb2, flw, flb) = lp[i * 26:(i + 1) * 26]
            X, Wqkv, QKV, ctx1, st1, Z1, ls1, X1, Q, ctx2, st2, Z2, ls2, X2, Hh, Z3, ls3 = ctx.saved[i]
            sid = cfg["stream_base"] + 64 + i * 8
            dZ3, dX2, d_flw, d_flb = pr.ln_bwd(dX, dX, Mt, Z3, X2, ls3, flw, Mt, p, seed, sid + 2, beta=flb)
            with fork(dZ3, Hh):
                d_fb2 = _gdest(fb2, (D,), zero=True)
                d_fW2 = pr.linear_dw(dZ3, D, Hh, F, Mt, D, F, out=_gdest(fW2, (D, F)), dbias=d_fb2)
            dHh = pr.linear_dx_relu(dZ3, D, fW2, Mt, Hh)
            with fork(dHh, X2):
                d_fb1 = _gdest(fb1, (F,), zero=True)
                d_fW1 = pr.linear_dw(dHh, F, X2, D, Mt, F, D, out=_gdest(fW1, (F, D)), dbias=d_fb1)
            pr.linear_dx(dHh, F, fW1, Mt, out=dX2, accumulate=True)
            dZ2, dX1, d_clw, d_clb = pr.ln_bwd(dX2, dX2, Mt, Z2, X1, ls2, clw, Mt, p, seed, sid + 1, beta=clb)
            with fork(dZ2, ctx2):
                d_cbo = _gdest(cbo, (D,), zero=True)
                d_cWo = pr.linear_dw(dZ2, D, ctx2, D, Mt, D, D, out=_gdest(cWo, (D, D)), dbias=d_cbo)
            dctx2 = pr.linear_dx(dZ2, D, cWo, Mt)
            dQ = pr.empty((Mt, D), dev)
            if pk is not None:
                call("fira_attn_packed_bwd", _ptr(Q), D, _ptr(KV, i * 2 * D), ldkv, _ptr(KV, i * 2 * D + D), ldkv,
                     _ptr(pk.ranges), Ms, _ptr(mem_mask), S, pk.chunks, _ptr(ctx2), _ptr(dctx2), D, _ptr(st2), _ptr(dQ), D,
                     _ptr(dKV, i * 2 * D), ldkv, _ptr(dKV, i * 2 * D + D), ldkv, B, H, T, D // H, pr.code, st)
            else:
                call("fira_attn_bwd", _ptr(Q), D, _ptr(KV, i * 2 * D), ldkv, _ptr(KV, i * 2 * D + D), ldkv,
                     _ptr(mem_mask), 0, _ptr(ctx2), _ptr(dctx2), D, _ptr(st2), _ptr(dQ), D, _ptr(dKV, i * 2 * D), ldkv,
                     _ptr(dKV, i * 2 * D + D), ldkv, B, H, T, S, D // H, pr.code, st)
            with fork(dQ, X1):
                d_cbq = _gdest(cbq, (D,), zero=True)
                d_cWq = pr.linear_dw(dQ, D, X1, D, Mt, D, D, out=_gdest(cWq, (D, D)), dbias=d_cbq)
            pr.linear_dx(dQ, D, cWq, Mt, out=dX1, accumulate=True)
            dZ1, dX0, d_slw, d_slb = pr.ln_bwd(dX1, dX1, Mt, Z1, X, ls1, slw, Mt, p, seed, sid + 0, beta=slb)
            with fork(dZ1, ctx1):
                d_sbo = _gdest(sbo, (D,), zero=True)
                d_sWo = pr.linear_dw(dZ1, D, ctx1, D, Mt, D, D, out=_gdest(sWo, (D, D)), dbias=d_sbo)
            dctx1 = pr.linear_dx(dZ1, D, sWo, Mt)
            dQKV = pr.empty((Mt, 3 * D), dev)
            call("fira_attn_bwd", _ptr(QKV), 3 * D, _ptr(QKV, D), 3 * D, _ptr(QKV, 2 * D), 3 * D, _ptr(tar_mask), 1,
                 _ptr(ctx1), _ptr(dctx1), D, _ptr(st1), _ptr(dQKV), 3 * D, _ptr(dQKV, D), 3 * D, _ptr(dQKV, 2 * D), 3 * D,
                 B, H, T, T, D // H, pr.code, st)
            with fork(dQKV, X):
                d_bqkv = _gdest((sbq, sbk, sbv), (3 * D,), zero=True)
                d_Wqkv = pr.linear_dw(dQKV, 3 * D, X, D, Mt, 3 * D, D, out=_gdest((sWq, sWk, sWv), (3 * D, D)), dbias=d_bqkv)
            pr.linear_dx(dQKV, 3 * D, Wqkv, Mt, out=dX0, accumulate=True)
            grads[i * 26:(i + 1) * 26] = [
                d_Wqkv[:D], d_bqkv[:D], d_Wqkv[D:2 * D], d_bqkv[D:2 * D], d_Wqkv[2 * D:], d_bqkv[2 * D:],
                d_sWo, d_sbo, d_slw, d_slb,
                d_cWq, d_cbq, None, None, None, None, d_cWo, d_cbo, d_clw, d_clb,
                d_fW1, d_fb1, d_fW2, d_fb2, d_flw, d_flb]
            dX = dX0
            ctx.saved[i] = None
        mem2 = memory.view(Ms, D)
        with fork(dKV, mem2):
            kv_w = [t for i in range(L) for t in (lp[i * 26 + 12], lp[i * 26 + 14])]
            kv_b = [t for i in range(L) for t in (lp[i * 26 + 13], lp[i * 26 + 15])]
            d_bkv = _gdest(kv_b, (ldkv,), zero=True)
            d_Wkv = pr.linear_dw(dKV, ldkv, mem2, D, Ms, ldkv, D, out=_gdest(kv_w, (ldkv, D)), dbias=d_bkv)
        d_mem = pr.linear_dx(dKV, ldkv, Wkv, Ms).view(memory.shape).to(mem_dtype)
        for i in range(L):
            o = i * 2 * D
            grads[i * 26 + 12], grads[i * 26 + 13] = d_Wkv[o:o + D], d_bkv[o:o + D]
            grads[i * 26 + 14], grads[i * 26 + 15] = d_Wkv[o + D:o + 2 * D], d_bkv[o + D:o + 2 * D]
        d_emb = _gdest(dec_emb, tuple(dec_emb.shape), zero=True)
        call("fira_embed_rows_bwd", _ptr(tar), _ptr(dX), _ptr(d_emb), Mt, D, pr.code, st)
        fork.join()
        return (None, None, d_mem, None, None, None, d_emb, *grads)


def _ld_logits(V):
    return (V + 63) // 64 * 64


def copy_scores_fwd(pr, memory2, dec2, Ws, Wt, wres, bres, B, T, S, src_mask=None, row_mask=None, ranges=None):
    src = pr.linear(memory2, Ws)
    tgt = pr.linear(dec2, Wt)
    sc = torch.empty((B, T, S), dtype=torch.float32, device=dec2.device)
    if ranges is not None:
        call("fira_copy_scores_packed_fwd", _ptr(src), _ptr(tgt), _ptr(wres), _ptr(bres), _ptr(ranges), _ptr(src_mask),
             _ptr(row_mask), _ptr(sc), B, T, S, D, pr.code, _stream())
    else:
        call("fira_copy_scores_fwd", _ptr(src), _ptr(tgt), _ptr(wres), _ptr(bres), _ptr(src_mask), _ptr(row_mask),
             _ptr(sc), B, T, S, D, pr.code, _stream())
    return src, tgt, sc


class HeadFn(torch.autograd.Function):

    @staticmethod
    def forward(ctx, want_argmax, bf16, pf, memory, dec, mem_mask, label, Wout, bout, Ws, Wt, Wres, bres, Wp, bp,
                pk=None, seq_weight=None):
        _require_cuda(memory, dec, Wout)
        B, T = dec.shape[0], dec.shape[1]
        S = pk.S if pk is not None else memory.shape[1]
        V = Wout.shape[0]
        if seq_weight is not None:
            if pk is not None or want_argmax:
                raise ValueError("HeadFn: seq_weight applies to the padded training path only")
# ... 168 lines not shown
```

fira_icse_b200/packed.py:

```python
import numpy as np
import torch

from ._lib import host_call

SEGMENT_BUCKETS = (1024, 512, 512, 64)
VOCAB_ROW_BUCKET = 128


class PackedBatch:

    FIELDS = ("code", "mark", "pos", "sub", "ast", "off", "ranges", "mem_mask", "tar", "label", "tar_mask",
              "rowptr", "col", "val")

    def __init__(self, B, Rc, Rs, Ra, S, T, nnz, chunks=4, Rv=None, **tensors):
        self.B, self.Rc, self.Rs, self.Ra, self.S, self.T, self.nnz = B, Rc, Rs, Ra, S, T, nnz
        self.chunks = int(chunks)
        self.Rv = B * T if Rv is None else int(Rv)
        for k in self.FIELDS:
            setattr(self, k, tensors[k])

    @property
    def shape_key(self):
        return (self.B, self.Rc, self.Rs, self.Ra, self.S, self.chunks, self.Rv)

    @property
    def rows(self):
        return self.Rc + self.Rs + self.Ra

    @property
    def mem_rows(self):
        return self.Rc + self.Rs

    def to(self, device, non_blocking=True):
        t = {k: getattr(self, k).to(device, non_blocking=non_blocking) for k in self.FIELDS}
        return PackedBatch(self.B, self.Rc, self.Rs, self.Ra, self.S, self.T, self.nnz, self.chunks, self.Rv, **t)

    def h2d_bytes(self):
        return sum(getattr(self, k).numel() * getattr(self, k).element_size() for k in self.FIELDS)


def _round_up(x, m):
    return max(m, -(-int(x) // m) * m)


class PackedTables:

    ID_KEYS = ("sou", "tar", "mark", "ast_change", "tar_label", "sub_token")

    def __init__(self, dataset):
        d = dataset.d
        self.tab = {k: np.ascontiguousarray(d[k], dtype=np.int32) for k in self.ID_KEYS}
        self.deg = np.ascontiguousarray(d["deg"], dtype=np.uint8)
        self.col = np.ascontiguousarray(d["col"], dtype=np.int16)
        self.val = np.ascontiguousarray(d["val"], dtype=np.float64)
        self.edge_ptr = np.ascontiguousarray(d["edge_ptr"], dtype=np.int64)
        self.lens = (dataset.diff_len, dataset.sub_token_len, dataset.ast_change_len)
        self.msg_len = dataset.msg_len
        self.n = len(self.tab["sou"])

    def dims(self, index):
        index = np.ascontiguousarray(index, dtype=np.int64)
        t = self.tab
        out = np.zeros(6, np.int32)
        host_call("fira_host_packed_dims", t["sou"].ctypes.data, t["sub_token"].ctypes.data, t["ast_change"].ctypes.data,
                  self.deg.ctypes.data, index.ctypes.data, len(index), *self.lens, out.ctypes.data)
        return tuple(int(x) for x in out)

    def vocab_rows(self, index, vocab_size):
        lab = self.tab["tar_label"][np.asarray(index, dtype=np.int64), 1:]
        return int(np.count_nonzero((lab > 0) & (lab < vocab_size)))


class PackedSlot:

    def __init__(self, B, lens, msg_len, edge_cap, pin):
        n0, n1, n2 = lens

        def buf(n, dt):
            t = torch.empty(n, dtype=dt)
            return t.pin_memory() if pin else t
        i32, u8 = torch.int32, torch.uint8
        self.cap = (_round_up(B * n0, SEGMENT_BUCKETS[0]), _round_up(B * n1, SEGMENT_BUCKETS[1]),
                    _round_up(B * n2, SEGMENT_BUCKETS[2]), _round_up(n0 + n1, SEGMENT_BUCKETS[3]))
        Rc, Rs, Ra, S = self.cap
        self.code, self.mark, self.pos = buf(Rc, i32), buf(Rc, i32), buf(Rc, i32)
        self.sub, self.ast = buf(Rs, i32), buf(Ra, i32)
        self.off, self.ranges = buf(3 * (B + 1), i32), buf(4 * B, i32)
        self.mem_mask = buf(B * S, u8)
        self.tar, self.label, self.tar_mask = buf(B * msg_len, i32), buf(B * msg_len, i32), buf(B * msg_len, u8)
        self.rowptr = buf(Rc + Rs + Ra + 1, i32)
        self.col, self.val = buf(edge_cap, i32), buf(edge_cap, torch.float32)
        self.edge_cap = edge_cap
        self.event = None
        self.batch = None


def gather_packed(tables, index, vocab_size, slot, pad_dims=None, buckets=SEGMENT_BUCKETS):
    index = np.ascontiguousarray(index, dtype=np.int64)
    b = len(index)
    need = tables.dims(index)
    if pad_dims is None:
        pad_dims = packed_needs(tables, index, vocab_size, buckets)
    elif len(pad_dims) == 4:
        pad_dims = tuple(pad_dims) + packed_needs(tables, index, vocab_size, buckets)[4:]
    Rc, Rs, Ra, S, Rv = (int(x) for x in pad_dims)
    if Rc > slot.cap[0] or Rs > slot.cap[1] or Ra > slot.cap[2] or S > slot.cap[3]:
        raise ValueError(f"packed batch {pad_dims} exceeds the staging capacity {slot.cap}")
    if Rv < tables.vocab_rows(index, vocab_size):
        raise ValueError(f"packed batch: Rv = {Rv} is below its vocabulary-label rows")
    t = tables.tab
    pd = np.asarray((Rc, Rs, Ra, S), np.int32)
    nnz = np.zeros(1, np.int32)
    host_call("fira_host_gather_packed", t["sou"].ctypes.data, t["tar"].ctypes.data, t["mark"].ctypes.data,
              t["ast_change"].ctypes.data, t["tar_label"].ctypes.data, t["sub_token"].ctypes.data,
              tables.deg.ctypes.data, tables.col.ctypes.data, tables.val.ctypes.data, tables.edge_ptr.ctypes.data,
              index.ctypes.data, b, *tables.lens, tables.msg_len, int(vocab_size), pd.ctypes.data,
              slot.code.data_ptr(), slot.mark.data_ptr(), slot.pos.data_ptr(), slot.sub.data_ptr(), slot.ast.data_ptr(),
              slot.off.data_ptr(), slot.ranges.data_ptr(), slot.mem_mask.data_ptr(), slot.tar.data_ptr(),
              slot.label.data_ptr(), slot.tar_mask.data_ptr(), slot.rowptr.data_ptr(), slot.col.data_ptr(),
              slot.val.data_ptr(), slot.edge_cap, nnz.ctypes.data)
    e, T = int(nnz[0]), tables.msg_len
    slot.batch = PackedBatch(
        b, Rc, Rs, Ra, S, T, e, max(3, need[5]), min(Rv, b * T),
        code=slot.code[:Rc], mark=slot.mark[:Rc], pos=slot.pos[:Rc], sub=slot.sub[:Rs], ast=slot.ast[:Ra],
        off=slot.off[:3 * (b + 1)].view(3, b + 1), ranges=slot.ranges[:4 * b].view(b, 4),
        mem_mask=slot.mem_mask[:b * S].view(b, S), tar=slot.tar[:b * T].view(b, T), label=slot.label[:b * T].view(b, T),
        tar_mask=slot.tar_mask[:b * T].view(b, T), rowptr=slot.rowptr[:Rc + Rs + Ra + 1], col=slot.col[:e],
        val=slot.val[:e])
    return slot.batch


def packed_needs(tables, index, vocab_size, buckets=SEGMENT_BUCKETS):
    need = tables.dims(index)
    return tuple(_round_up(need[i], buckets[i]) for i in range(4)) + \
        (_round_up(tables.vocab_rows(index, vocab_size), VOCAB_ROW_BUCKET),)


def pack_from_dataset(dataset, index, vocab_size, pin=False, pad_dims=None, buckets=SEGMENT_BUCKETS):
    tables = dataset if isinstance(dataset, PackedTables) else PackedTables(dataset)
    per_commit = int(np.diff(tables.edge_ptr).max()) if len(tables.edge_ptr) > 1 else 0
    slot = PackedSlot(len(index), tables.lens, tables.msg_len, max(1, per_commit * len(index)), pin)
    return gather_packed(tables, index, vocab_size, slot, pad_dims=pad_dims, buckets=buckets)
```

include/fira_b200.h:

```cpp
#ifndef FIRA_B200_H_
#define FIRA_B200_H_

#include <stdint.h>

#ifdef __cplusplus
extern "C" {
#endif

#define FIRA_F32 0
#define FIRA_BF16 1
#define FIRA_EDGE_F32 0
#define FIRA_EDGE_BF16 1
#define FIRA_EDGE_F64 2

int fira_version(void);
const char* fira_last_error_string(void);
int fira_built_arch(void);
int fira_num_sms(void);
int fira_set_pdl(int on);
int fira_get_pdl(void);

int fira_gemm_f32(const float* A, long lda, int a_kcontig, const float* B, long ldb, int b_kcontig, float* C,
                  long ldc, int M, int N, int K, const float* bias, const float* rs, const float* rc, int relu,
                  int accumulate, int splits, void* stream);

int fira_gemm_bf16_tc(const void* A, long lda, int a_kmajor, const void* B, long ldb, int b_kmajor, void* C,
                      long ldc, int c_is_bf16, int M, int N, int K, const float* bias, const float* rs,
                      const float* rc, int relu, int accumulate, int splits, void* stream);

int fira_gemm_bf16_tc_dbias(const void* A, long lda, const void* B, long ldb, int b_kmajor, void* C, long ldc,
                            int c_is_bf16, int M, int N, int K, int accumulate, int splits, float* d_bias, void* stream);

int fira_gemm_bf16_tc_dx_relu(const void* dy, long lddy, const void* W, long ldw, void* dx, long lddx, const void* h,
                              int M, int N, int K, void* stream);

int fira_debug_set_probe(void* probe);

int fira_embed_nodes_fwd(const int* sou, const int* sub_token, const int* ast_change, const float* emb,
                         const float* ast_emb, const float* pos_table, void* out_code, void* out_rest, int B,
                         int n_code, int n_sub, int n_ast, int dim, int dtype, void* stream);
int fira_embed_nodes_pos_fwd(const int* sou, const int* pos, const int* sub_token, const int* ast_change,
                             const float* emb, const float* ast_emb, const float* pos_table, void* out_code,
                             void* out_rest, int B, int n_code, int n_sub, int n_ast, int dim, int dtype, void* stream);
int fira_zero_pad_rows(void* x, long ld, int width, const int* off, int B, int Rc, int Rs, int dtype, void* stream);
int fira_embed_nodes_bwd(const int* sou, const int* sub_token, const int* ast_change, const void* d_code,
                         const void* d_rest, float* d_emb, float* d_ast_emb, int B, int n_code, int n_sub, int n_ast,
                         int dim, int dtype, void* stream);
int fira_embed_rows_fwd(const int* ids, const float* emb, const float* pos_table, void* out, long rows, int period,
                        int dim, int dtype, void* stream);
int fira_embed_rows_bwd(const int* ids, const void* d_out, float* d_emb, long rows, int dim, int dtype, void* stream);

int fira_ln_residual_fwd(const void* z, const void* resid, const float* gamma, const float* beta, void* outA,
                         void* outB, long split, float* mean, float* rstd, long rows, int dim, float p_drop,
                         uint64_t seed, const uint64_t* seed_ctr, uint32_t stream_id, int dtype, void* stream);
int fira_ln_residual_bwd(const void* d_outA, const void* d_outB, long split, const void* z, const void* resid,
                         const float* mean, const float* rstd, const float* gamma, void* d_z, void* d_resid,
                         int d_resid_accum, float* d_gamma, float* d_beta, long rows, int dim, float p_drop,
                         uint64_t seed, const uint64_t* seed_ctr, uint32_t stream_id, int dtype, void* stream);

int fira_comb_gate_fwd(const void* qk, long ld_qk, const float* vtab, const int* mark, void* out, long rows, int dim,
                       int d_head, float p_drop, uint64_t seed, const uint64_t* seed_ctr, uint32_t stream_id, int dtype, void* stream);
int fira_comb_gate_bwd(const void* qk, long ld_qk, const float* vtab, const int* mark, const void* d_out, void* d_qk,
                       float* d_vtab, long rows, int dim, int d_head, float p_drop, uint64_t seed, const uint64_t* seed_ctr,
                       uint32_t stream_id, int dtype, void* stream);

int fira_comb_gate3_fwd(const void* q, const void* k, const void* v, void* out, long rows, int dim, int d_head,
                        float p_drop, uint64_t seed, const uint64_t* seed_ctr, uint32_t stream_id, int dtype, void* stream);
int fira_comb_gate3_bwd(const void* q, const void* k, const void* v, const void* d_out, void* d_q, void* d_k, void* d_v,
                        long rows, int dim, int d_head, float p_drop, uint64_t seed, const uint64_t* seed_ctr,
                        uint32_t stream_id, int dtype, void* stream);

int fira_relu_bwd(const void* h, void* d, long n, int dtype, void* stream);
int fira_colsum(const void* x, long ld, long M, int N, const float* row_weight, float* out, int dtype, void* stream);

int fira_adam_flat(float* p, const float* g, float* m, float* v, void* p_bf16, long n, float lr, float beta1, float beta2,
                   float eps, const float* step, const float* grad_scale, void* stream);
int fira_cast_bf16(const float* x, void* y, long n, void* stream);

int fira_pack_memory(const void* code, const void* rest, void* mem, int B, int n_code, int n_sub, int dim, int dtype,
                     void* stream);
int fira_unpack_memory(const void* d_mem, void* d_code, void* d_rest, int B, int n_code, int n_sub, int n_ast, int dim,
                       int dtype, void* stream);

int fira_csr_count_dense(const void* edge, int edge_dtype, long stride_b, long stride_i, long stride_j, int B, int N,
                         int* counts, int* rowptr, void* stream);
int fira_csr_fill_dense(const void* edge, int edge_dtype, long stride_b, long stride_i, long stride_j, int B, int N,
                        const int* rowptr, int* col, float* val, void* stream);
int fira_csr_rowsum(const int* rowptr, const float* val, int B, int n_code, int n_sub, int n_ast, float* out,
                    void* stream);
int fira_gcn_aggregate(const int* rowptr, const int* col, const float* val, const void* x, const void* addend,
                       void* y, int B, int n_code, int n_sub, int n_ast, int dim, int dtype, void* stream);

int fira_csr_to_rows(const int* rowptr, const int* col, const float* val, int B, int n_code, int n_sub, int n_ast,
                     int* counts, int* rowptr_rows, int* col_rows, float* val_rows, void* stream);
int fira_gcn_layer_fwd(const int* rowptr_rows, const int* col_rows, const float* val_rows, const void* h,
                       const void* w_merged, const float* bias, const float* c1, const float* gamma, const float* beta,
                       void* z, void* outA, void* outB, long split, float* mean, float* rstd, long rows, int dim,
                       float p_drop, uint64_t seed, const uint64_t* seed_ctr, uint32_t stream_id, void* stream);
int fira_gcn_layer_bwd(const int* rowptr_rows_t, const int* col_rows_t, const float* val_rows_t, const void* d_z,
                       const void* w_merged_t, const void* d_resid, void* agg_dz, void* d_h, long rows, int dim,
                       void* stream);

int fira_attn_fwd(const void* q, long ldq, const void* k, long ldk, const void* v, long ldv,
                  const unsigned char* key_mask, int causal, void* ctx, long ldo, float* stats, int B, int H, int Lq,
                  int Lk, int d_head, int dtype, void* stream);
int fira_attn_bwd(const void* q, long ldq, const void* k, long ldk, const void* v, long ldv,
                  const unsigned char* key_mask, int causal, const void* ctx, const void* d_ctx, long ldo,
                  const float* stats, void* dq, long lddq, void* dk, long lddk, void* dv, long lddv, int B, int H,
                  int Lq, int Lk, int d_head, int dtype, void* stream);

int fira_attn_packed_fwd(const void* q, long ldq, const void* k, long ldk, const void* v, long ldv, const int* ranges,
                         long kv_rows, const unsigned char* key_mask, int mask_pitch, int max_chunks, void* ctx, long ldo,
                         float* stats, int B, int H, int Lq, int d_head, int dtype, void* stream);
int fira_attn_packed_bwd(const void* q, long ldq, const void* k, long ldk, const void* v, long ldv, const int* ranges,
                         long kv_rows, const unsigned char* key_mask, int mask_pitch, int max_chunks, const void* ctx,
                         const void* d_ctx, long ldo, const float* stats, void* dq, long lddq, void* dk, long lddk,
                         void* dv, long lddv, int B, int H, int Lq, int d_head, int dtype, void* stream);

int fira_decoder_fwd(const int* tar, const float* dec_emb, const float* pos_table, const unsigned char* tar_mask,
                     const void* kv, long ldkv, const unsigned char* mem_mask, const int* ranges, int S,
                     const void* const* layer_ptrs, int L, void* X, void* qkv, void* ctx1, float* st1, void* z1,
                     float* ls1, void* x1, void* q, void* ctx2, float* st2, void* z2, float* ls2, void* x2, void* hh,
                     void* z3, float* ls3, int B, int T, float p_drop, uint64_t seed, const uint64_t* seed_ctr,
                     uint32_t stream_id, void* stream);

int fira_copy_scores_fwd(const void* src_proj, const void* tgt_proj, const float* w_res, const float* b_res,
                         const unsigned char* src_mask, const unsigned char* row_mask, float* scores,
                         int B, int T_len, int S, int dim, int dtype, void* stream);
int fira_copy_scores_bwd(const void* src_proj, const void* tgt_proj, const float* w_res, const float* d_scores,
                         const unsigned char* row_active, void* d_src_proj, float* d_tgt_proj, float* d_w_res,
                         float* d_b_res, int B, int T_len, int S, int dim, int dtype, void* stream);

int fira_copy_scores_packed_fwd(const void* src_proj, const void* tgt_proj, const float* w_res, const float* b_res,
                                const int* ranges, const unsigned char* src_mask, const unsigned char* row_mask,
                                float* scores, int B, int T_len, int S, int dim, int dtype, void* stream);
int fira_copy_scores_packed_bwd(const void* src_proj, const void* tgt_proj, const float* w_res, const float* d_scores,
                                const unsigned char* row_active, const int* ranges, void* d_src_proj, float* d_tgt_proj,
                                float* d_w_res, float* d_b_res, int B, int T_len, int S, int dim, int dtype, void* stream);

int fira_pointer_mix_nll_fwd(const void* logits, long ld_logits, const float* copy_scores, const float* gate_logits,
                             const unsigned char* mem_mask, const int* label, float* stats, float* nll,
                             int* argmax_out, long rows, int T_len, int V, int S, int dtype, void* stream);
int fira_pointer_mix_nll_bwd(const void* logits, long ld_logits, const float* copy_scores,
                             const unsigned char* mem_mask, const int* label, const float* stats,
                             const float* upstream, void* d_logits, float* d_copy_scores, float* d_gate_logits,
                             unsigned char* row_active, long rows, int T_len, int V, int S, int dtype, void* stream);

int fira_vocab_rows(const int* label, long rows, int V, int* vslot, int* vrows, int cap, void* stream);
int fira_gather_rows(const void* src, long ld_src, const int* idx, void* dst, long ld_dst, long n, int width, int dtype,
                     void* stream);
int fira_pointer_mix_nll_fwd_rows(const void* logits, long ld_logits, const float* copy_scores, const float* gate_logits,
                                  const unsigned char* mem_mask, const int* label, const int* vslot, float* stats,
                                  float* nll, int* argmax_out, long rows, int T_len, int V, int S, int dtype,
                                  void* stream);
int fira_pointer_mix_nll_bwd_rows(const void* logits, long ld_logits, const float* copy_scores,
                                  const unsigned char* mem_mask, const int* label, const int* vslot, const int* vrows,
                                  int cap, const float* stats, const float* upstream, void* d_logits,
                                  float* d_copy_scores, float* d_gate_logits, unsigned char* row_active, long rows,
                                  int T_len, int V, int S, int dtype, void* stream);
int fira_pointer_mix_nll_bwd_rows_weighted(const void* logits, long ld_logits, const float* copy_scores,
                                           const unsigned char* mem_mask, const int* label, const int* vslot,
                                           const int* vrows, int cap, const float* stats, const float* upstream,
                                           void* d_logits, float* d_copy_scores, float* d_gate_logits,
                                           unsigned char* row_active, long rows, int T_len, int V, int S, int dtype,
                                           void* stream, const float* seq_weight);

int fira_pointer_mix_sample(const void* logits, long ld_logits, const float* copy_scores, const float* gate_logits,
                            const unsigned char* mem_mask, const int* copy_src, const uint64_t* seed,
                            const int* first_index, const float* uniforms, float temperature, int top_k, float top_p,
                            int eos_id, int pad_id, int* next_tok, int* seq, int* raw, float* token_logprob,
                            unsigned char* tok_mask, long ld_out, int pos, unsigned char* finished, int* length,
                            float* logprob, int B, int N, int V, int S, int dtype, void* stream);

int fira_pointer_mix_beam_step(const void* logits, long ld_logits, const float* copy_scores, const float* gate_logits,
                               const unsigned char* mem_mask, const int* copy_src, float length_penalty, int eos_id,
                               int pad_id, uint64_t* workspace, int* seq, int* raw, float* token_logprob, int* length,
                               float* logprob, float* score, unsigned char* status, long* parent, int* next_tok,
                               int T_len, int pos, int B, int K, int V, int S, int dtype, void* stream);

int fira_pointer_mix_diverse_beam_step(const void* logits, long ld_logits, const float* copy_scores,
                                       const float* gate_logits, const unsigned char* mem_mask, const int* copy_src,
// ... 91 lines not shown
```

Baseline: 21140.

## Pack decoder target rows to live tokens and skip padded rows

Adds a packed-row decoder path. Per-batch target lengths and offsets (toff/tlen) let the decoder forward, the attention backward, the LN backward and the embedding backward work only on live target rows (up to the last non-zero label) and store activations compactly in R rows instead of B*T. Padding rows are zero-filled, and the Python packer computes a new Rt bucket. The aim is less memory traffic and fewer GEMM rows for short messages, at the cost of more index bookkeeping and new shape keys that can trigger recompiles or graph captures.

```diff
diff --git a/fira_icse_b200/csrc/attention.cu b/fira_icse_b200/csrc/attention.cu
--- a/fira_icse_b200/csrc/attention.cu
+++ b/fira_icse_b200/csrc/attention.cu
@@ -318,6 +318,25 @@
                     const float* __restrict__ stats, __nv_bfloat16* __restrict__ dq, long lddq,
                     __nv_bfloat16* __restrict__ dk, long lddk, __nv_bfloat16* __restrict__ dv, long lddv) {
   pdl_wait(); pdl_trigger();
+  const int sp = a.Lq, kp = a.Lk;
+  const long qb = a.qoff ? (long)a.qoff[blockIdx.x / a.H] : (long)(blockIdx.x / a.H) * sp;
+  if (a.qoff) {
+    a.Lq = a.qoff[blockIdx.x / a.H + 1] - (int)qb;
+    if (a.causal) a.Lk = a.Lq;
+    if (blockIdx.x / a.H == a.B - 1) {
+      const int h = blockIdx.x % a.H;
+      const long p0 = a.qoff[a.B];
+      for (long i = threadIdx.x; i < (a.qrows - p0) * 4; i += blockDim.x) {
+        const long r = p0 + (i >> 2);
+        const int c = (int)(i & 3) * 8 + h * DH;
+        *reinterpret_cast<uint4*>(dq + r * lddq + c) = make_uint4(0, 0, 0, 0);
+        if (a.causal) {
+          *reinterpret_cast<uint4*>(dk + r * lddk + c) = make_uint4(0, 0, 0, 0);
+          *reinterpret_cast<uint4*>(dv + r * lddv + c) = make_uint4(0, 0, 0, 0);
+        }
+      }
+    }
+  }
   extern __shared__ __align__(16) unsigned char mma_smem[];
   __shared__ int nv_s, filled_s;
   __shared__ float delta_s[LQ_MAX], m2_s[LQ_MAX], inv_s[LQ_MAX];
@@ -327,9 +346,9 @@
   int* kidx = reinterpret_cast<int*>(Ws + BWARPS * BWARP_SMEM);
   const int b = blockIdx.x / a.H, h = blockIdx.x % a.H;
   const int lane = threadIdx.x & 31, warp = threadIdx.x >> 5, q = lane & 3;
-  const unsigned char* km = a.key_mask ? a.key_mask + (long)b * a.Lk : nullptr;
+  const unsigned char* km = a.key_mask ? a.key_mask + (long)b * kp : nullptr;
   const int* rg = a.ranges ? a.ranges + 4 * b : nullptr;
-  const long kvb = rg ? 0 : (long)b * a.Lk;
+  const long kvb = rg ? 0 : a.qoff && a.causal ? qb : (long)b * kp;
   const __nv_bfloat16* kh = (const __nv_bfloat16*)a.k + kvb * a.ldk + h * DH;
   const __nv_bfloat16* vh = (const __nv_bfloat16*)a.v + kvb * a.ldv + h * DH;
   unsigned char* Kw = Ws + warp * BWARP_SMEM;
@@ -344,15 +363,15 @@
   for (int i = threadIdx.x; i < 2 * LQ_MAX * 4; i += blockDim.x) {
     const int which = i / (LQ_MAX * 4), r = (i >> 2) & (LQ_MAX - 1), c = i & 3;
     unsigned char* dst = (which ? Os : Qs) + swz(r, c);
-    if (r < a.Lq) cp_async16(su32(dst), which ? d_ctx + ((long)b * a.Lq + r) * ldo + h * DH + c * 8
-                                              : (const __nv_bfloat16*)a.q + ((long)b * a.Lq + r) * a.ldq + h * DH + c * 8);
+    if (r < a.Lq) cp_async16(su32(dst), which ? d_ctx + (qb + r) * ldo + h * DH + c * 8
+                                              : (const __nv_bfloat16*)a.q + (qb + r) * a.ldq + h * DH + c * 8);
     else *reinterpret_cast<uint4*>(dst) = make_uint4(0, 0, 0, 0);
   }
   cp_async_commit();
   if (threadIdx.x < a.Lq) {
     const int t = threadIdx.x;
-    const __nv_bfloat16* orow = out + ((long)b * a.Lq + t) * ldo + h * DH;
-    const __nv_bfloat16* grow = d_ctx + ((long)b * a.Lq + t) * ldo + h * DH;
+    const __nv_bfloat16* orow = out + (qb + t) * ldo + h * DH;
+    const __nv_bfloat16* grow = d_ctx + (qb + t) * ldo + h * DH;
     float d = 0.f;
 #pragma unroll
     for (int c = 0; c < 4; ++c) {
@@ -362,7 +381,7 @@
 #pragma unroll
       for (int e = 0; e < 8; ++e) d = fmaf(ov[e], gv[e], d);
     }
-    const float* st = stats + (((long)b * a.H + h) * a.Lq + t) * 2;
+    const float* st = stats + (((long)b * a.H + h) * sp + t) * 2;
     delta_s[t] = d; m2_s[t] = st[0] * kLog2e; inv_s[t] = 1.f / st[1];
   }
   if (!filled && !a.causal && km) {
@@ -501,7 +520,7 @@
 #pragma unroll
     for (int w = 0; w < BWARPS; ++w)
       x += reinterpret_cast<const float*>(Ws + w * BWARP_SMEM + 4 * BKB * ROWB)[swz_f32(t, f)];
-    dq[((long)b * a.Lq + t) * lddq + h * DH + f] = __float2bfloat16_rn(x);
+    dq[(qb + t) * lddq + h * DH + f] = __float2bfloat16_rn(x);
   }
 }
 
@@ -578,7 +597,8 @@
 
 int attn_bwd_impl(const void* q, long ldq, const void* k, long ldk, const void* v, long ldv,
                   const unsigned char* key_mask, const int* ranges, int causal, const void* ctx, const void* d_ctx, long ldo, const float* stats, void* dq, long lddq, void* dk,
-                  long lddk, void* dv, long lddv, int B, int H, int Lq, int Lk, int d_head, int dtype, void* stream) {
+                  long lddk, void* dv, long lddv, int B, int H, int Lq, int Lk, int d_head, int dtype, void* stream,
+                  const int* qoff = nullptr, long qrows = 0) {
   FIRA_CHECK_ARG(d_head == DH, FIRA_ERR_SHAPE, "attn_bwd: d_head %d != 32", d_head);
   FIRA_CHECK_ARG(B > 0 && H > 0 && Lq > 0 && Lk > 0 && Lq <= LQ_MAX, FIRA_ERR_SHAPE, "attn_bwd: shape (Lq <= 32)");
   FIRA_CHECK_ARG(key_mask || ranges, FIRA_ERR_ARG, "attn_bwd: key_mask may only be NULL with ranges");
@@ -588,8 +608,11 @@
       (rc = check_layout("attn_bwd", v, ldv, dtype)) || (rc = check_layout("attn_bwd", ctx, ldo, dtype)) ||
       (rc = check_layout("attn_bwd", d_ctx, ldo, dtype)))
     return rc;
-  AttnArgs a{q, ldq, k, ldk, v, ldv, key_mask, ranges, causal, B, H, Lq, Lk, 1.f / sqrtf((float)d_head)};
-  if (use_tc(dtype) && (lddk % 8) == 0 && (lddv % 8) == 0 && (lddq % 8) == 0) {
+  AttnArgs a{q, ldq, k, ldk, v, ldv, key_mask, ranges, causal, B, H, Lq, Lk, 1.f / sqrtf((float)d_head), qoff, qrows};
+  FIRA_CHECK_ARG(!qoff || (dtype == FIRA_BF16 && (lddk % 8) == 0 && (lddv % 8) == 0 && (lddq % 8) == 0 &&
+                           (!causal || (Lq == Lk && !ranges))),
+                 FIRA_ERR_ARG, "attn_bwd_rows: bf16, 16-B gradient pitches, causal with Lq == Lk and no ranges");
+  if (qoff || (use_tc(dtype) && (lddk % 8) == 0 && (lddv % 8) == 0 && (lddq % 8) == 0)) {
     const size_t smem = mma::bwd_smem(Lk);
     if ((rc = set_smem(mma::attn_mma_bwd_kernel, smem, "attn_bwd"))) return rc;
     launch_k(mma::attn_mma_bwd_kernel, dim3(B * H), dim3(mma::BWARPS * 32), smem, (cudaStream_t)stream, a,
@@ -651,4 +674,13 @@
                        dk, lddk, dv, lddv, B, H, Lq, mask_pitch, d_head, dtype, stream);
 }
 
-}
+int fira_attn_bwd_rows(const void* q, long ldq, const void* k, long ldk, const void* v, long ldv, const int* ranges,
+                       const unsigned char* key_mask, int mask_pitch, int causal, const int* qoff, long rows,
+                       const void* ctx, const void* d_ctx, long ldo, const float* stats, void* dq, long lddq, void* dk,
+                       long lddk, void* dv, long lddv, int B, int H, int Lq, int d_head, int dtype, void* stream) {
+  FIRA_CHECK_ARG(qoff && rows > 0, FIRA_ERR_ARG, "attn_bwd_rows: null qoff or no rows");
+  return attn_bwd_impl(q, ldq, k, ldk, v, ldv, key_mask, ranges, causal, ctx, d_ctx, ldo, stats, dq, lddq, dk, lddk,
+                       dv, lddv, B, H, Lq, mask_pitch, d_head, dtype, stream, qoff, rows);
+}
+
+}
diff --git a/fira_icse_b200/csrc/attn_mma.cuh b/fira_icse_b200/csrc/attn_mma.cuh
--- a/fira_icse_b200/csrc/attn_mma.cuh
+++ b/fira_icse_b200/csrc/attn_mma.cuh
@@ -15,6 +15,8 @@
   int causal;
   int B, H, Lq, Lk;
   float scale;
+  const int* qoff = nullptr;
+  long qrows = 0;
 };
 
 __device__ __forceinline__ void compact_keys(const unsigned char* km, int Lk, int causal, int* kidx, int* nv_out,
diff --git a/fira_icse_b200/csrc/decoder_fwd.cu b/fira_icse_b200/csrc/decoder_fwd.cu
--- a/fira_icse_b200/csrc/decoder_fwd.cu
+++ b/fira_icse_b200/csrc/decoder_fwd.cu
@@ -34,9 +34,12 @@
   const bf16* kv; long ldkv;
   const unsigned char* mem_mask; const int* ranges; int S;
   bf16* X;
+  bf16* out;
   bf16* qkv; bf16* ctx1; float* st1; bf16* z1; float* ls1; bf16* x1;
   bf16* q; bf16* ctx2; float* st2; bf16* z2; float* ls2; bf16* x2;
   bf16* hh; bf16* z3; float* ls3;
+  const int* tlen; const int* toff;
+  long R;
   int B, T, L;
   float scale, p_drop;
   uint64_t seed; const uint64_t* seed_ctr; uint32_t stream_id;
@@ -136,8 +139,9 @@
 
 __device__ __forceinline__ void ln_rows(const unsigned char* sm, int off_z, int off_res, int off_out, const float* gamma,
                                         const float* beta, bf16* __restrict__ zg, bf16* __restrict__ og,
-                                        float* __restrict__ stats, long rows, long r0, int T, float p_drop, uint64_t seed,
-                                        const uint64_t* seed_ctr, uint32_t sid, int rank, int warp, int lane) {
+                                        float* __restrict__ stats, long rows, long r0, long s0, int T, int n, int tl,
+                                        bool out_rows, float p_drop, uint64_t seed, const uint64_t* seed_ctr,
+                                        uint32_t sid, int rank, int warp, int lane) {
   if (seed_ctr) seed += *seed_ctr;
   float g[8], bt[8];
   Act<float>::load8(gamma + lane * 8, g);
@@ -147,10 +151,10 @@
     const int o = (t * LDA + lane * 8) * 2;
     bf16* os = (bf16*)(sm + off_out + o);
     if (t >= T) { *reinterpret_cast<uint4*>(os) = make_uint4(0, 0, 0, 0); continue; }
-    const long r = r0 + t;
+    const long r = r0 + t, sl = s0 + t;
     const bool mine = (t & 1) == rank;
     const uint4 zraw = *reinterpret_cast<const uint4*>(sm + off_z + o);
-    if (mine) *reinterpret_cast<uint4*>(zg + r * D + lane * 8) = zraw;
+    if (mine && t < n) *reinterpret_cast<uint4*>(zg + sl * D + lane * 8) = zraw;
     float y[8], x[8];
     Act<bf16>::load8((const bf16*)&zraw, y);
     Act<bf16>::load8((const bf16*)(sm + off_res + o), x);
@@ -171,8 +175,14 @@
     for (int i = 0; i < 8; ++i) y[i] = (y[i] - mean) * rstd * g[i] + bt[i];
     Act<bf16>::store8(os, y);
     if (mine) {
-      *reinterpret_cast<uint4*>(og + r * D + lane * 8) = *reinterpret_cast<const uint4*>(os);
-      if (lane == 0) { stats[r] = mean; stats[rows + r] = rstd; }
+      if (out_rows) {
+        const uint32_t fill = t < tl ? 0x7fc07fc0u : 0u;
+        *reinterpret_cast<uint4*>(og + r * D + lane * 8) =
+            t < n ? *reinterpret_cast<const uint4*>(os) : make_uint4(fill, fill, fill, fill);
+      } else if (t < n) {
+        *reinterpret_cast<uint4*>(og + sl * D + lane * 8) = *reinterpret_cast<const uint4*>(os);
+      }
+      if (lane == 0 && t < n) { stats[sl] = mean; stats[rows + sl] = rstd; }
     }
   }
 }
@@ -218,13 +228,13 @@
 decoder_fwd_kernel(const __grid_constant__ DecParams p) {
   pdl_wait(); pdl_trigger();
   extern __shared__ __align__(16) unsigned char sm[];
-  __shared__ int nv_s, filled_s;
+  __shared__ int nv_s, filled_s, s0_s, n_s, tl_s;
   cg::cluster_group cluster = cg::this_cluster();
   const int rank = (int)cluster.block_rank();
   unsigned char* peer = cluster.map_shared_rank(sm, rank ^ 1);
   const int b = blockIdx.x >> 1, T = p.T;
   const int lane = threadIdx.x & 31, warp = threadIdx.x >> 5, hl = (warp >> 1) & 3, r0q = 16 * (warp & 1);
-  const long Mt = (long)p.B * T, grow0 = (long)b * T;
+  const long grow0 = (long)b * T, R = p.R;
   int* kidx = reinterpret_cast<int*>(sm + SMEM_FIXED);
   bf16* Xs = (bf16*)(sm + OFF_X);
   bf16* Ys = (bf16*)(sm + OFF_Y);
@@ -234,6 +244,33 @@
     *reinterpret_cast<uint32_t*>(peer + off) = v;
   };
 
+  if (threadIdx.x == 0) {
+    s0_s = p.toff ? p.toff[b] : (int)grow0;
+    n_s = p.toff ? p.toff[b + 1] - s0_s : T;
+    tl_s = p.tlen ? p.tlen[b] : T;
+  }
+  if (p.toff) {
+    const int c = 8 * threadIdx.x;
+    for (long sl = p.toff[p.B] + blockIdx.x; sl < R; sl += gridDim.x)
+      for (int i = 0; i < p.L; ++i) {
+        const long ro = i * R + sl;
+        bf16* dst;
+        switch (c >> 8) {
+          case 0: dst = p.X + ro * D + c; break;
+          case 1: dst = p.ctx1 + ro * D + c - 256; break;
+          case 2: dst = p.z1 + ro * D + c - 512; break;
+          case 3: dst = p.x1 + ro * D + c - 768; break;
+          case 4: dst = p.q + ro * D + c - 1024; break;
+          case 5: dst = p.ctx2 + ro * D + c - 1280; break;
+          case 6: dst = p.z2 + ro * D + c - 1536; break;
+          case 7: dst = p.x2 + ro * D + c - 1792; break;
+          case 8: dst = p.z3 + ro * D + c - 2048; break;
+          case 9: case 10: case 11: dst = p.qkv + ro * 3 * D + c - 2304; break;
+          default: dst = p.hh + ro * F + c - 3072; break;
+        }
+        *reinterpret_cast<uint4*>(dst) = make_uint4(0, 0, 0, 0);
+      }
+  }
   compact_keys(p.mem_mask ? p.mem_mask + (long)b * p.S : nullptr, p.S, 0, kidx, &nv_s, &filled_s,
                p.ranges ? p.ranges + 4 * b : nullptr);
 
@@ -245,7 +282,7 @@
       Act<float>::load8(p.pe + (long)t * D + lane * 8, pe);
 #pragma unroll
       for (int i = 0; i < 8; ++i) v[i] += pe[i];
-      if ((t & 1) == rank) Act<bf16>::store8(p.X + (grow0 + t) * D + lane * 8, v);
+      if ((t & 1) == rank && t < n_s) Act<bf16>::store8(p.X + ((long)s0_s + t) * D + lane * 8, v);
     } else {
 #pragma unroll
       for (int i = 0; i < 8; ++i) v[i] = 0.f;
@@ -256,12 +293,13 @@
 
   for (int i = 0; i < p.L; ++i) {
     const LayerW& w = p.w[i];
-    const long o256 = i * Mt * D;
+    const long o256 = i * R * D, s0 = s0_s;
+    const int n = n_s;
 
     product<D, 1, 8, false>(Xs, w.wqkv, w.bqkv, 3 * D, rank, warp, lane,
                             [&](int t, int n, int, uint32_t v) { *reinterpret_cast<uint32_t*>(big + head_off(t, n)) = v; });
     __syncthreads();
-    copy_out(p.qkv + (i * Mt + grow0) * 3 * D, 3 * D, T, rank, warp, lane, [&](int t, int n) { return big + head_off(t, n); });
+    copy_out(p.qkv + (i * R + s0) * 3 * D, 3 * D, n, rank, warp, lane, [&](int t, int n) { return big + head_off(t, n); });
     if (warp < 8) {
       AttnArgs sa{};
       sa.causal = 1;
@@ -276,18 +314,18 @@
       ar.finish(sm + OFF_Y, peer + OFF_Y, h, T, p.st1 + (((long)i * p.B + b) * NH + h) * T * 2, lane);
     }
     cluster.sync();
-    copy_out(p.ctx1 + o256 + grow0 * D, D, T, rank, warp, lane, [&](int t, int n) { return Ys + t * LDA + gcol(n, rank); });
+    copy_out(p.ctx1 + o256 + s0 * D, D, n, rank, warp, lane, [&](int t, int n) { return Ys + t * LDA + gcol(n, rank); });
     product<D, 1, 8, false>(Ys, w.swo, w.sbo, D, rank, warp, lane,
                             [&](int t, int, int c, uint32_t v) { to_both(OFF_Z + (t * LDA + c) * 2, v); });
     cluster.sync();
-    ln_rows(sm, OFF_Z, OFF_X, OFF_X1, w.slw, w.slb, p.z1 + o256, p.x1 + o256, p.ls1 + 2 * i * Mt, Mt, grow0, T,
-            p.p_drop, p.seed, p.seed_ctr, p.stream_id + 8 * i + 0, rank, warp, lane);
+    ln_rows(sm, OFF_Z, OFF_X, OFF_X1, w.slw, w.slb, p.z1 + o256, p.x1 + o256, p.ls1 + 2 * i * R, R, grow0, s0, T, n,
+            T, false, p.p_drop, p.seed, p.seed_ctr, p.stream_id + 8 * i + 0, rank, warp, lane);
     __syncthreads();
 
     product<D, 1, 8, false>((const bf16*)(sm + OFF_X1), w.cwq, w.cbq, D, rank, warp, lane,
                             [&](int t, int n, int, uint32_t v) { *reinterpret_cast<uint32_t*>(big + head_off(t, n)) = v; });
     __syncthreads();
-    copy_out(p.q + o256 + grow0 * D, D, T, rank, warp, lane, [&](int t, int n) { return big + head_off(t, n); });
+    copy_out(p.q + o256 + s0 * D, D, n, rank, warp, lane, [&](int t, int n) { return big + head_off(t, n); });
     if (warp < 8) {
       const int h = 4 * rank + hl;
       const int nv = nv_s, nblk = (nv + CKB - 1) / CKB;
@@ -320,28 +358,68 @@
       ar.finish(sm + OFF_Y, peer + OFF_Y, h, T, p.st2 + (((long)i * p.B + b) * NH + h) * T * 2, lane);
     }
     cluster.sync();
-    copy_out(p.ctx2 + o256 + grow0 * D, D, T, rank, warp, lane, [&](int t, int n) { return Ys + t * LDA + gcol(n, rank); });
+    copy_out(p.ctx2 + o256 + s0 * D, D, n, rank, warp, lane, [&](int t, int n) { return Ys + t * LDA + gcol(n, rank); });
     product<D, 1, 8, false>(Ys, w.cwo, w.cbo, D, rank, warp, lane,
                             [&](int t, int, int c, uint32_t v) { to_both(OFF_Z + (t * LDA + c) * 2, v); });
     cluster.sync();
-    ln_rows(sm, OFF_Z, OFF_X1, OFF_X2, w.clw, w.clb, p.z2 + o256, p.x2 + o256, p.ls2 + 2 * i * Mt, Mt, grow0, T,
-            p.p_drop, p.seed, p.seed_ctr, p.stream_id + 8 * i + 1, rank, warp, lane);
+    ln_rows(sm, OFF_Z, OFF_X1, OFF_X2, w.clw, w.clb, p.z2 + o256, p.x2 + o256, p.ls2 + 2 * i * R, R, grow0, s0, T, n,
+            T, false, p.p_drop, p.seed, p.seed_ctr, p.stream_id + 8 * i + 1, rank, warp, lane);
     __syncthreads();
 
     bf16* Hs = (bf16*)big;
     product<D, 2, 4, true>((const bf16*)(sm + OFF_X2), w.w1, w.b1, F, rank, warp, lane,
                            [&](int t, int, int c, uint32_t v) { to_both(OFF_BIG + (t * LDF + c) * 2, v); });
     cluster.sync();
-    copy_out(p.hh + (i * Mt + grow0) * F, F, T, rank, warp, lane, [&](int t, int n) { return Hs + t * LDF + gcol(n, rank); });
+    copy_out(p.hh + (i * R + s0) * F, F, n, rank, warp, lane, [&](int t, int n) { return Hs + t * LDF + gcol(n, rank); });
     product<F, 1, 8, false>(Hs, w.w2, w.b2, D, rank, warp, lane,
                             [&](int t, int, int c, uint32_t v) { to_both(OFF_Z + (t * LDA + c) * 2, v); });
     cluster.sync();
-    ln_rows(sm, OFF_Z, OFF_X2, OFF_X, w.flw, w.flb, p.z3 + o256, p.X + o256 + Mt * D, p.ls3 + 2 * i * Mt, Mt, grow0, T,
-            p.p_drop, p.seed, p.seed_ctr, p.stream_id + 8 * i + 2, rank, warp, lane);
+    const bool last = i == p.L - 1;
+    ln_rows(sm, OFF_Z, OFF_X2, OFF_X, w.flw, w.flb, p.z3 + o256, last ? p.out : p.X + o256 + R * D, p.ls3 + 2 * i * R, R,
+            grow0, s0, T, n, tl_s, last, p.p_drop, p.seed, p.seed_ctr, p.stream_id + 8 * i + 2, rank, warp, lane);
     __syncthreads();
   }
 }
 
+}
+
+extern "C" int fira_decoder_fwd_rows(const int* tar, const float* dec_emb, const float* pos_table,
+                                     const unsigned char* tar_mask, const void* kv, long ldkv,
+                                     const unsigned char* mem_mask, const int* ranges, int S,
+                                     const void* const* layer_ptrs, int L, void* X, void* out, void* qkv, void* ctx1,
+                                     float* st1, void* z1, float* ls1, void* x1, void* q, void* ctx2, float* st2,
+                                     void* z2, float* ls2, void* x2, void* hh, void* z3, float* ls3, const int* tlen,
+                                     const int* toff, long R, int B, int T, float p_drop, uint64_t seed,
+                                     const uint64_t* seed_ctr, uint32_t stream_id, void* stream) {
+  FIRA_CHECK_ARG(B > 0 && T > 0 && T <= TP, FIRA_ERR_SHAPE, "decoder_fwd: B %d, T %d (T <= 32)", B, T);
+  FIRA_CHECK_ARG(L > 0 && L <= MAX_LAYERS, FIRA_ERR_SHAPE, "decoder_fwd: %d layers (1..%d)", L, MAX_LAYERS);
+  FIRA_CHECK_ARG(S > 0, FIRA_ERR_SHAPE, "decoder_fwd: S %d", S);
+  FIRA_CHECK_ARG(!tlen == !toff && (toff ? R > 0 && R <= (long)B * T : R == (long)B * T), FIRA_ERR_ARG,
+                 "decoder_fwd: tlen and toff both or neither, 0 < R <= B*T (R = B*T without them)");
+  FIRA_CHECK_ARG(mem_mask || ranges, FIRA_ERR_ARG, "decoder_fwd: mem_mask may only be NULL with ranges");
+  FIRA_CHECK_ARG(layer_ptrs && tar && dec_emb && pos_table && tar_mask && kv, FIRA_ERR_ARG, "decoder_fwd: null input");
+  FIRA_CHECK_ARG(fira_aligned16(kv) && ldkv % 8 == 0 && ldkv >= (long)L * 2 * D, FIRA_ERR_ALIGN,
+                 "decoder_fwd: kv must be 16-B aligned with ldkv a multiple of 8 and >= L*512");
+  void* outs[] = {X, out, qkv, ctx1, z1, x1, q, ctx2, z2, x2, hh, z3};
+  for (void* o : outs) FIRA_CHECK_ARG(o && fira_aligned16(o), FIRA_ERR_ALIGN, "decoder_fwd: outputs must be 16-B aligned");
+  FIRA_CHECK_ARG(st1 && ls1 && st2 && ls2 && ls3, FIRA_ERR_ARG, "decoder_fwd: null statistics");
+  DecParams p{tar, dec_emb, pos_table, tar_mask, (const bf16*)kv, ldkv, mem_mask, ranges, S,
+              (bf16*)X, (bf16*)out, (bf16*)qkv, (bf16*)ctx1, st1, (bf16*)z1, ls1, (bf16*)x1,
+              (bf16*)q, (bf16*)ctx2, st2, (bf16*)z2, ls2, (bf16*)x2, (bf16*)hh, (bf16*)z3, ls3, tlen, toff, R,
+              B, T, L, 1.f / sqrtf((float)DH), p_drop, seed, seed_ctr, stream_id, {}};
+  for (int i = 0; i < L; ++i) {
+    const void* const* t = layer_ptrs + 18 * i;
+    for (int j = 0; j < 18; ++j)
+      FIRA_CHECK_ARG(t[j] && fira_aligned16(t[j]), FIRA_ERR_ALIGN, "decoder_fwd: layer %d pointer %d null or unaligned", i, j);
+    memcpy(&p.w[i], t, sizeof(LayerW));
+  }
+  const size_t smem = SMEM_FIXED + sizeof(int) * (size_t)S;
+  FIRA_CHECK_ARG(smem <= 227 * 1024, FIRA_ERR_SHAPE, "decoder_fwd: S %d needs %zu B shared memory", S, smem);
+  cudaError_t e = cudaFuncSetAttribute(decoder_fwd_kernel, cudaFuncAttributeMaxDynamicSharedMemorySize, (int)smem);
+  if (e != cudaSuccess) { fira_set_error(FIRA_ERR_CUDA, "decoder_fwd: %s", cudaGetErrorString(e)); return FIRA_ERR_CUDA; }
+  launch_k(decoder_fwd_kernel, dim3(2 * B), dim3(NTHR), smem, (cudaStream_t)stream, p);
+  FIRA_CHECK_LAUNCH("fira_decoder_fwd");
+  return FIRA_OK;
 }
 
 extern "C" int fira_decoder_fwd(const int* tar, const float* dec_emb, const float* pos_table,
@@ -351,31 +429,9 @@
                                 void* z2, float* ls2, void* x2, void* hh, void* z3, float* ls3, int B, int T,
                                 float p_drop, uint64_t seed, const uint64_t* seed_ctr, uint32_t stream_id,
                                 void* stream) {
-  FIRA_CHECK_ARG(B > 0 && T > 0 && T <= TP, FIRA_ERR_SHAPE, "decoder_fwd: B %d, T %d (T <= 32)", B, T);
-  FIRA_CHECK_ARG(L > 0 && L <= MAX_LAYERS, FIRA_ERR_SHAPE, "decoder_fwd: %d layers (1..%d)", L, MAX_LAYERS);
-  FIRA_CHECK_ARG(S > 0, FIRA_ERR_SHAPE, "decoder_fwd: S %d", S);
-  FIRA_CHECK_ARG(mem_mask || ranges, FIRA_ERR_ARG, "decoder_fwd: mem_mask may only be NULL with ranges");
-  FIRA_CHECK_ARG(layer_ptrs && tar && dec_emb && pos_table && tar_mask && kv, FIRA_ERR_ARG, "decoder_fwd: null input");
-  FIRA_CHECK_ARG(fira_aligned16(kv) && ldkv % 8 == 0 && ldkv >= (long)L * 2 * D, FIRA_ERR_ALIGN,
-                 "decoder_fwd: kv must be 16-B aligned with ldkv a multiple of 8 and >= L*512");
-  void* outs[] = {X, qkv, ctx1, z1, x1, q, ctx2, z2, x2, hh, z3};
-  for (void* o : outs) FIRA_CHECK_ARG(o && fira_aligned16(o), FIRA_ERR_ALIGN, "decoder_fwd: outputs must be 16-B aligned");
-  FIRA_CHECK_ARG(st1 && ls1 && st2 && ls2 && ls3, FIRA_ERR_ARG, "decoder_fwd: null statistics");
-  DecParams p{tar, dec_emb, pos_table, tar_mask, (const bf16*)kv, ldkv, mem_mask, ranges, S,
-              (bf16*)X, (bf16*)qkv, (bf16*)ctx1, st1, (bf16*)z1, ls1, (bf16*)x1,
-              (bf16*)q, (bf16*)ctx2, st2, (bf16*)z2, ls2, (bf16*)x2, (bf16*)hh, (bf16*)z3, ls3,
-              B, T, L, 1.f / sqrtf((float)DH), p_drop, seed, seed_ctr, stream_id, {}};
-  for (int i = 0; i < L; ++i) {
-    const void* const* t = layer_ptrs + 18 * i;
-    for (int j = 0; j < 18; ++j)
-      FIRA_CHECK_ARG(t[j] && fira_aligned16(t[j]), FIRA_ERR_ALIGN, "decoder_fwd: layer %d pointer %d null or unaligned", i, j);
-    memcpy(&p.w[i], t, sizeof(LayerW));
-  }
-  const size_t smem = SMEM_FIXED + sizeof(int) * (size_t)S;
-  FIRA_CHECK_ARG(smem <= 227 * 1024, FIRA_ERR_SHAPE, "decoder_fwd: S %d needs %zu B shared memory", S, smem);
-  cudaError_t e = cudaFuncSetAttribute(decoder_fwd_kernel, cudaFuncAttributeMaxDynamicSharedMemorySize, (int)smem);
-  if (e != cudaSuccess) { fira_set_error(FIRA_ERR_CUDA, "decoder_fwd: %s", cudaGetErrorString(e)); return FIRA_ERR_CUDA; }
-  launch_k(decoder_fwd_kernel, dim3(2 * B), dim3(NTHR), smem, (cudaStream_t)stream, p);
-  FIRA_CHECK_LAUNCH("fira_decoder_fwd");
-  return FIRA_OK;
-}
+  FIRA_CHECK_ARG(X && L > 0 && B > 0 && T > 0, FIRA_ERR_ARG, "decoder_fwd: arguments");
+  void* out = (bf16*)X + (long)L * B * T * D;
+  return fira_decoder_fwd_rows(tar, dec_emb, pos_table, tar_mask, kv, ldkv, mem_mask, ranges, S, layer_ptrs, L, X, out,
+                               qkv, ctx1, st1, z1, ls1, x1, q, ctx2, st2, z2, ls2, x2, hh, z3, ls3, nullptr, nullptr,
+                               (long)B * T, B, T, p_drop, seed, seed_ctr, stream_id, stream);
+}
diff --git a/fira_icse_b200/csrc/head.cu b/fira_icse_b200/csrc/head.cu
--- a/fira_icse_b200/csrc/head.cu
+++ b/fira_icse_b200/csrc/head.cu
@@ -199,6 +199,33 @@
     const bool v = label[r] != 0 && label[r] < V && slot < cap;
     vslot[r] = v ? slot : -1;
     if (v) vrows[slot++] = (int)r;
+  }
+}
+
+__global__ void __launch_bounds__(kRowsThreads) target_rows_kernel(const int* __restrict__ label, int B, int T,
+                                                                   int* __restrict__ tlen, int* __restrict__ toff,
+                                                                   int* __restrict__ trows, int cap) {
+  pdl_wait(); pdl_trigger();
+  __shared__ int warp_sum_s[kRowsThreads / 32];
+  const int lane = threadIdx.x & 31, warp = threadIdx.x >> 5, b = threadIdx.x;
+  int n = 0;
+  if (b < B)
+    for (int t = T - 1; t >= 0; --t)
+      if (label[(long)b * T + t] != 0) { n = t + 1; break; }
+  int incl = n;
+#pragma unroll
+  for (int o = 1; o < 32; o <<= 1) { const int u = __shfl_up_sync(0xffffffffu, incl, o); if (lane >= o) incl += u; }
+  if (lane == 31) warp_sum_s[warp] = incl;
+  for (int s = threadIdx.x; s < cap; s += kRowsThreads) trows[s] = -1;
+  __syncthreads();
+  int off = incl - n;
+  for (int w = 0; w < warp; ++w) off += warp_sum_s[w];
+  if (b < B) {
+    const int s0 = min(off, cap), s1 = min(off + n, cap);
+    tlen[b] = n;
+    toff[b] = s0;
+    if (b == B - 1) toff[B] = s1;
+    for (int s = s0; s < s1; ++s) trows[s] = b * T + (s - off);
   }
 }
 
@@ -1040,6 +1067,14 @@
   FIRA_CHECK_ARG(label && vslot && vrows && rows >= 0 && V > 0 && cap >= 0, FIRA_ERR_ARG, "vocab_rows: arguments");
   launch_k(vocab_rows_kernel, dim3(1), dim3(kRowsThreads), 0, (cudaStream_t)stream, label, rows, V, vslot, vrows, cap);
   FIRA_CHECK_LAUNCH("fira_vocab_rows");
+  return FIRA_OK;
+}
+
+int fira_target_rows(const int* label, int B, int T, int* tlen, int* toff, int* trows, int cap, void* stream) {
+  FIRA_CHECK_ARG(label && tlen && toff && trows && B > 0 && B <= kRowsThreads && T > 0 && cap >= 0, FIRA_ERR_ARG,
+                 "target_rows: arguments (B <= %d)", kRowsThreads);
+  launch_k(target_rows_kernel, dim3(1), dim3(kRowsThreads), 0, (cudaStream_t)stream, label, B, T, tlen, toff, trows, cap);
+  FIRA_CHECK_LAUNCH("fira_target_rows");
   return FIRA_OK;
 }
 
diff --git a/fira_icse_b200/csrc/rowops.cu b/fira_icse_b200/csrc/rowops.cu
--- a/fira_icse_b200/csrc/rowops.cu
+++ b/fira_icse_b200/csrc/rowops.cu
@@ -80,18 +80,20 @@
   }
 }
 template <typename T>
-__global__ void embed_rows_bwd_kernel(const int* __restrict__ ids, const T* __restrict__ g, float* __restrict__ d_emb,
-                                      long rows) {
+__global__ void embed_rows_bwd_kernel(const int* __restrict__ ids, const int* __restrict__ rmap, const T* __restrict__ g,
+                                      float* __restrict__ d_emb, long rows) {
   pdl_wait(); pdl_trigger();
   const int lane = threadIdx.x & 31;
   for (long r = (long)blockIdx.x * ROWS_PER_CTA + (threadIdx.x >> 5); r < rows; r += (long)gridDim.x * ROWS_PER_CTA) {
+    const long src = rmap ? rmap[r] : r;
+    if (src < 0) continue;
     float v[8];
     Act<T>::load8(g + r * D + lane * 8, v);
     bool nz = false;
 #pragma unroll
     for (int i = 0; i < 8; ++i) nz |= v[i] != 0.f;
     if (!__any_sync(0xffffffffu, nz)) continue;
-    float* o = d_emb + (long)ids[r] * D + lane * 8;
+    float* o = d_emb + (long)ids[src] * D + lane * 8;
     atomicAdd(reinterpret_cast<float4*>(o), make_float4(v[0], v[1], v[2], v[3]));
     atomicAdd(reinterpret_cast<float4*>(o + 4), make_float4(v[4], v[5], v[6], v[7]));
   }
@@ -140,7 +142,7 @@
                               const float* __restrict__ rstd_in, const float* __restrict__ gamma, T* __restrict__ d_z,
                               T* __restrict__ d_resid, int d_resid_accum, float* __restrict__ d_gamma,
                               float* __restrict__ d_beta, long rows, float p_drop, uint64_t seed,
-                              const uint64_t* __restrict__ seed_ctr, uint32_t stream_id) {
+                              const uint64_t* __restrict__ seed_ctr, uint32_t stream_id, const int* __restrict__ rmap) {
   pdl_wait(); pdl_trigger();
   if (seed_ctr) seed += *seed_ctr;
   __shared__ __align__(16) float red[2][ROWS_PER_CTA][D];
@@ -151,13 +153,21 @@
   for (int i = 0; i < 8; ++i) { dg[i] = 0.f; db[i] = 0.f; }
   const float keep_scale = p_drop > 0.f ? 1.f / (1.f - p_drop) : 1.f;
   for (long r = (long)blockIdx.x * ROWS_PER_CTA + warp; r < rows; r += (long)gridDim.x * ROWS_PER_CTA) {
+    const long pr = rmap ? rmap[r] : r;
     float y[8], x[8], go[8];
+    if (pr < 0) {
+#pragma unroll
+      for (int i = 0; i < 8; ++i) y[i] = 0.f;
+      Act<T>::store8(d_z + r * D + lane * 8, y);
+      if (d_resid && !d_resid_accum) Act<T>::store8(d_resid + r * D + lane * 8, y);
+      continue;
+    }
     Act<T>::load8(z + r * D + lane * 8, y);
     Act<T>::load8(resid + r * D + lane * 8, x);
     Act<T>::load8((r < split ? doutA : doutB) + r * D + lane * 8, go);
     uint32_t m = 0xffu;
     if (p_drop > 0.f) {
-      m = dropout_keep8(seed, stream_id, (uint64_t)r * 32 + lane, p_drop);
+      m = dropout_keep8(seed, stream_id, (uint64_t)pr * 32 + lane, p_drop);
 #pragma unroll
       for (int i = 0; i < 8; ++i) y[i] = ((m >> i) & 1) ? y[i] * keep_scale : 0.f;
     }
@@ -528,9 +538,15 @@
 }
 
 int fira_embed_rows_bwd(const int* ids, const void* d_out, float* d_emb, long rows, int dim, int dtype, void* stream) {
+  return fira_embed_rows_bwd_rows(ids, nullptr, d_out, d_emb, rows, dim, dtype, stream);
+}
+
+int fira_embed_rows_bwd_rows(const int* ids, const int* rows_map, const void* d_out, float* d_emb, long rows, int dim,
+                             int dtype, void* stream) {
   FIRA_CHECK_ARG(dim == D, FIRA_ERR_SHAPE, "embed_rows_bwd: dim %d != 256", dim);
-  DISPATCH_T(dtype, launch_k(embed_rows_bwd_kernel<T>, dim3(row_grid(rows)), dim3(CTA), 0, (cudaStream_t)stream, ids, (const T*)d_out,
-                                                                                             d_emb, rows);)
+  if (rows == 0) return FIRA_OK;
+  DISPATCH_T(dtype, launch_k(embed_rows_bwd_kernel<T>, dim3(row_grid(rows)), dim3(CTA), 0, (cudaStream_t)stream, ids,
+                             rows_map, (const T*)d_out, d_emb, rows);)
   FIRA_CHECK_LAUNCH("fira_embed_rows_bwd");
   return FIRA_OK;
 }
@@ -553,13 +569,22 @@
                          const float* mean, const float* rstd, const float* gamma, void* d_z, void* d_resid,
                          int d_resid_accum, float* d_gamma, float* d_beta, long rows, int dim, float p_drop,
                          uint64_t seed, const uint64_t* seed_ctr, uint32_t stream_id, int dtype, void* stream) {
+  return fira_ln_residual_bwd_rows(d_outA, d_outB, split, z, resid, mean, rstd, gamma, d_z, d_resid, d_resid_accum,
+                                   d_gamma, d_beta, nullptr, rows, dim, p_drop, seed, seed_ctr, stream_id, dtype, stream);
+}
+
+int fira_ln_residual_bwd_rows(const void* d_outA, const void* d_outB, long split, const void* z, const void* resid,
+                              const float* mean, const float* rstd, const float* gamma, void* d_z, void* d_resid,
+                              int d_resid_accum, float* d_gamma, float* d_beta, const int* rows_map, long rows, int dim,
+                              float p_drop, uint64_t seed, const uint64_t* seed_ctr, uint32_t stream_id, int dtype,
+                              void* stream) {
   FIRA_CHECK_ARG(dim == D, FIRA_ERR_SHAPE, "ln_residual_bwd: dim %d != 256", dim);
   if (rows == 0) return FIRA_OK;
   long g = (rows + ROWS_PER_CTA - 1) / ROWS_PER_CTA;
   int grid = (int)(g < (long)fira_num_sms() * 4 ? g : (long)fira_num_sms() * 4);
   DISPATCH_T(dtype, launch_k(ln_bwd_kernel<T>, dim3(grid), dim3(CTA), 0, (cudaStream_t)stream, 
       (const T*)d_outA, (const T*)d_outB, split, (const T*)z, (const T*)resid, mean, rstd, gamma, (T*)d_z,
-      (T*)d_resid, d_resid_accum, d_gamma, d_beta, rows, p_drop, seed, seed_ctr, stream_id);)
+      (T*)d_resid, d_resid_accum, d_gamma, d_beta, rows, p_drop, seed, seed_ctr, stream_id, rows_map);)
   FIRA_CHECK_LAUNCH("fira_ln_residual_bwd");
   return FIRA_OK;
 }
diff --git a/fira_icse_b200/data.py b/fira_icse_b200/data.py
--- a/fira_icse_b200/data.py
+++ b/fira_icse_b200/data.py
@@ -301,7 +301,7 @@
                              "bounds-check")
         self.multiples = (0, 0, 0) if multiples is None else tuple(int(m) for m in multiples)
         self.max_shapes = max_shapes
-        self.shapes = {}
+        self.dims_used = {}
         self.lens = (dataset.diff_len, dataset.sub_token_len, dataset.ast_change_len)
         self.msg_len = dataset.msg_len
         d = dataset.d
@@ -329,17 +329,25 @@
         n = len(self.indices)
         return n // self.B if self.drop_last else -(-n // self.B)
 
+    @property
+    def shapes(self):
+        out = {}
+        for k, n in self.dims_used.items():
+            out[k[:5]] = out.get(k[:5], 0) + n
+        return out
+
     def _choose_dims(self, need):
         need = tuple(int(x) for x in need)
-        if need in self.shapes or self.max_shapes is None or len(self.shapes) < self.max_shapes:
-            self.shapes[need] = self.shapes.get(need, 0) + 1
+        used = self.dims_used
+        if need in used or self.max_shapes is None or len(used) < self.max_shapes:
+            used[need] = used.get(need, 0) + 1
             return need
-        fits = [s for s in self.shapes if all(a >= b for a, b in zip(s, need))]
+        fits = [s for s in used if all(a >= b for a, b in zip(s, need))]
         if self.packed and not fits:
-            self.shapes[need] = 1
+            used[need] = 1
             return need
         best = min(fits, key=sum) if fits else self.lens
-        self.shapes[best] = self.shapes.get(best, 0) + 1
+        used[best] = used.get(best, 0) + 1
         return best
 
     def gather(self, index, slot=None):
diff --git a/fira_icse_b200/engine.py b/fira_icse_b200/engine.py
--- a/fira_icse_b200/engine.py
+++ b/fira_icse_b200/engine.py
@@ -31,7 +31,7 @@
             return torch.zeros(t.shape if n is None else (n,), dtype=t.dtype, device=dev)
         t = {k: z(getattr(pb, k)) for k in PackedBatch.FIELDS if k not in ("col", "val")}
         t["col"], t["val"] = z(pb.col, cap), z(pb.val, cap)
-        self.pb = PackedBatch(pb.B, pb.Rc, pb.Rs, pb.Ra, pb.S, pb.T, cap, pb.chunks, pb.Rv, **t)
+        self.pb = PackedBatch(pb.B, pb.Rc, pb.Rs, pb.Ra, pb.S, pb.T, cap, pb.chunks, pb.Rv, pb.Rt, **t)
         self.B, self.cap = pb.B, cap
         self.graph = None
         self.grads = None
diff --git a/fira_icse_b200/model.py b/fira_icse_b200/model.py
--- a/fira_icse_b200/model.py
+++ b/fira_icse_b200/model.py
@@ -95,8 +95,8 @@
         memory = self.encoder.encode_memory_packed(pb)
         if self._memory_hook is not None:
             memory = self._memory_hook(memory)
-        dec = self.decoder(pb.tar, memory, pb.mem_mask, pb.tar_mask, packed=pb)
         want_ids = stage != "train"
+        dec = self.decoder(pb.tar, memory, pb.mem_mask, pb.tar_mask, packed=pb, label=None if want_ids else pb.label)
         loss_sum, _, ids = ops.HeadFn.apply(want_ids, bf16, pf_head, memory, dec, pb.mem_mask, pb.label.view(-1),
                                             self.out_fc.weight, self.out_fc.bias, *self.copy_net.flat_params(), pb)
         if stage == "train":
diff --git a/fira_icse_b200/modules.py b/fira_icse_b200/modules.py
--- a/fira_icse_b200/modules.py
+++ b/fira_icse_b200/modules.py
@@ -224,12 +224,13 @@
         if dev.type == "cuda":
             self._prefetched = ops.prefetch_decoder(bool(getattr(self, "bf16", False)), self._flat(), dev)
 
-    def forward(self, output_token, input_em, sou_mask, tar_mask_pad, packed=None):
+    def forward(self, output_token, input_em, sou_mask, tar_mask_pad, packed=None, label=None):
         dev = self.embedding.weight.device
         if self.pos_encode.device != dev:
             self.pos_encode = self.pos_encode.to(dev)
         cfg = _run_cfg(self)
-        cfg.update(p_dec=self.attention_list[0].dropout.p, prefetch=getattr(self, "_prefetched", None), packed=packed)
+        cfg.update(p_dec=self.attention_list[0].dropout.p, prefetch=getattr(self, "_prefetched", None), packed=packed,
+                   label=None if label is None else _i32(label))
         self._prefetched = None
         lp = self._flat()
         return ops.DecoderFn.apply(cfg, _i32(output_token), input_em, _u8(sou_mask), _u8(tar_mask_pad),
diff --git a/fira_icse_b200/ops.py b/fira_icse_b200/ops.py
--- a/fira_icse_b200/ops.py
+++ b/fira_icse_b200/ops.py
@@ -201,15 +201,16 @@
              _ptr(stats), _ptr(stats, rows), rows, D, float(p), seed, _ptr(self.seed_ctr), sid, self.code, _stream())
         return stats
 
-    def ln_bwd(self, dA, dB, split, z, resid, stats, gamma, rows, p, seed, sid, d_resid=None, accum=False, beta=None):
+    def ln_bwd(self, dA, dB, split, z, resid, stats, gamma, rows, p, seed, sid, d_resid=None, accum=False, beta=None,
+               rows_map=None):
         dz = torch.empty_like(z)
         if d_resid is None:
             d_resid = torch.empty_like(z)
         dgb = _gdest((gamma, beta), (2, D), zero=True) if beta is not None else \
             torch.zeros((2, D), dtype=torch.float32, device=z.device)
-        call("fira_ln_residual_bwd", _ptr(dA), _ptr(dB), split, _ptr(z), _ptr(resid), _ptr(stats), _ptr(stats, rows),
-             _ptr(gamma), _ptr(dz), _ptr(d_resid), int(accum), _ptr(dgb), _ptr(dgb, D), rows, D, float(p), seed,
-             _ptr(self.seed_ctr), sid, self.code, _stream())
+        call("fira_ln_residual_bwd_rows", _ptr(dA), _ptr(dB), split, _ptr(z), _ptr(resid), _ptr(stats),
+             _ptr(stats, rows), _ptr(gamma), _ptr(dz), _ptr(d_resid), int(accum), _ptr(dgb), _ptr(dgb, D), _ptr(rows_map),
+             rows, D, float(p), seed, _ptr(self.seed_ctr), sid, self.code, _stream())
         return dz, d_resid, dgb[0], dgb[1]
 
 
@@ -554,23 +555,31 @@
         ldkv = L * 2 * D
         KV = pr.linear(memory.view(Ms, D), Wkv, bkv)
         if pr.bf16:
+            label = cfg.get("label")
+            rmap = None
+            R = Mt
+            if label is not None and pk is not None:
+                R = pk.Rt
+                rmap = torch.empty((2 * B + 1 + R,), dtype=torch.int32, device=dev)
+                call("fira_target_rows", _ptr(label), B, T, _ptr(rmap), _ptr(rmap, B), _ptr(rmap, 2 * B + 1), R, st)
             bf = dict(dtype=torch.bfloat16, device=dev)
-            Xs = torch.empty((L + 1, Mt, D), **bf)
-            QKV, Hh = torch.empty((L, Mt, 3 * D), **bf), torch.empty((L, Mt, 4 * D), **bf)
-            ctx1, Z1, X1, Q, ctx2, Z2, X2, Z3 = torch.empty((8, L, Mt, D), **bf)
+            Xs = torch.empty((L, R, D), **bf)
+            out = torch.empty((Mt, D), **bf)
+            QKV, Hh = torch.empty((L, R, 3 * D), **bf), torch.empty((L, R, 4 * D), **bf)
+            ctx1, Z1, X1, Q, ctx2, Z2, X2, Z3 = torch.empty((8, L, R, D), **bf)
             st1, st2 = torch.empty((2, L, B, H, T, 2), **f32)
-            ls1, ls2, ls3 = torch.empty((3, L, 2, Mt), **f32)
-            call("fira_decoder_fwd", _ptr(tar), _ptr(dec_emb), _ptr(pos_table), _ptr(tar_mask), _ptr(KV), ldkv,
+            ls1, ls2, ls3 = torch.empty((3, L, 2, R), **f32)
+            call("fira_decoder_fwd_rows", _ptr(tar), _ptr(dec_emb), _ptr(pos_table), _ptr(tar_mask), _ptr(KV), ldkv,
                  _ptr(mem_mask), _ptr(pk.ranges) if pk is not None else None, S, ctypes.addressof(pf.layer_table), L,
-                 _ptr(Xs), _ptr(QKV), _ptr(ctx1), _ptr(st1), _ptr(Z1), _ptr(ls1), _ptr(X1), _ptr(Q), _ptr(ctx2),
-                 _ptr(st2), _ptr(Z2), _ptr(ls2), _ptr(X2), _ptr(Hh), _ptr(Z3), _ptr(ls3), B, T, float(p), seed,
-                 _ptr(pr.seed_ctr), cfg["stream_base"] + 64, st)
+                 _ptr(Xs), _ptr(out), _ptr(QKV), _ptr(ctx1), _ptr(st1), _ptr(Z1), _ptr(ls1), _ptr(X1), _ptr(Q),
+                 _ptr(ctx2), _ptr(st2), _ptr(Z2), _ptr(ls2), _ptr(X2), _ptr(Hh), _ptr(Z3), _ptr(ls3), _ptr(rmap),
+                 _ptr(rmap, B), R, B, T, float(p), seed, _ptr(pr.seed_ctr), cfg["stream_base"] + 64, st)
             ctx.saved = [(Xs[i], qkv_layers[i][0], QKV[i], ctx1[i], st1[i], Z1[i], ls1[i], X1[i], Q[i], ctx2[i], st2[i],
                           Z2[i], ls2[i], X2[i], Hh[i], Z3[i], ls3[i]) for i in range(L)]
             ctx.wcache = pr.wcache
-            ctx.misc = (cfg, tar, memory, mem_mask, tar_mask, KV, Wkv, B, T, S, p, mem_dtype, Ms)
+            ctx.misc = (cfg, tar, memory, mem_mask, tar_mask, KV, Wkv, B, T, S, p, mem_dtype, Ms, R, rmap)
             ctx.save_for_backward(dec_emb, *lp)
-            return Xs[L].view(B, T, D)
+            return out.view(B, T, D)
         saved = []
         for i in range(L):
             (sWq, sbq, sWk, sbk, sWv, sbv, sWo, sbo, slw, slb,
@@ -603,13 +612,13 @@
             X = X3
         ctx.saved = saved
         ctx.wcache = pr.wcache
-        ctx.misc = (cfg, tar, memory, mem_mask, tar_mask, KV, Wkv, B, T, S, p, mem_dtype, Ms)
+        ctx.misc = (cfg, tar, memory, mem_mask, tar_mask, KV, Wkv, B, T, S, p, mem_dtype, Ms, Mt, None)
         ctx.save_for_backward(dec_emb, *lp)
         return X.view(B, T, D)
 
     @staticmethod
     def backward(ctx, d_out):
-        cfg, tar, memory, mem_mask, tar_mask, KV, Wkv, B, T, S, p, mem_dtype, Ms = ctx.misc
+        cfg, tar, memory, mem_mask, tar_mask, KV, Wkv, B, T, S, p, mem_dtype, Ms, R, rmap = ctx.misc
         dec_emb, *lp = ctx.saved_tensors
         Mt = B * T
         pk = cfg.get("packed")
@@ -620,6 +629,12 @@
         st = _stream()
         ldkv = L * 2 * D
         dX = d_out.contiguous().to(pr.tdt).view(Mt, D)
+        toff = trows = None
+        if rmap is not None:
+            toff, trows = rmap[B:2 * B + 1], rmap[2 * B + 1:]
+            dXs = pr.empty((R, D), dev)
+            call("fira_gather_rows", _ptr(dX), D, _ptr(trows), _ptr(dXs), D, R, D, pr.code, st)
+            dX = dXs
         dKV = pr.empty((Ms, ldkv), dev)
         if pk is not None:
             call("fira_zero_pad_rows", _ptr(dKV), ldkv, ldkv, _ptr(pk.off), B, pk.Rc, pk.Rs, pr.code, st)
@@ -632,22 +647,26 @@
              fW1, fb1, fW2, fb2, flw, flb) = lp[i * 26:(i + 1) * 26]
             X, Wqkv, QKV, ctx1, st1, Z1, ls1, X1, Q, ctx2, st2, Z2, ls2, X2, Hh, Z3, ls3 = ctx.saved[i]
             sid = cfg["stream_base"] + 64 + i * 8
-            dZ3, dX2, d_flw, d_flb = pr.ln_bwd(dX, dX, Mt, Z3, X2, ls3, flw, Mt, p, seed, sid + 2, beta=flb)
+            dZ3, dX2, d_flw, d_flb = pr.ln_bwd(dX, dX, R, Z3, X2, ls3, flw, R, p, seed, sid + 2, beta=flb, rows_map=trows)
             with fork(dZ3, Hh):
                 d_fb2 = _gdest(fb2, (D,), zero=True)
-                d_fW2 = pr.linear_dw(dZ3, D, Hh, F, Mt, D, F, out=_gdest(fW2, (D, F)), dbias=d_fb2)
-            dHh = pr.linear_dx_relu(dZ3, D, fW2, Mt, Hh)
+                d_fW2 = pr.linear_dw(dZ3, D, Hh, F, R, D, F, out=_gdest(fW2, (D, F)), dbias=d_fb2)
+            dHh = pr.linear_dx_relu(dZ3, D, fW2, R, Hh)
             with fork(dHh, X2):
                 d_fb1 = _gdest(fb1, (F,), zero=True)
-                d_fW1 = pr.linear_dw(dHh, F, X2, D, Mt, F, D, out=_gdest(fW1, (F, D)), dbias=d_fb1)
-            pr.linear_dx(dHh, F, fW1, Mt, out=dX2, accumulate=True)
-            dZ2, dX1, d_clw, d_clb = pr.ln_bwd(dX2, dX2, Mt, Z2, X1, ls2, clw, Mt, p, seed, sid + 1, beta=clb)
+                d_fW1 = pr.linear_dw(dHh, F, X2, D, R, F, D, out=_gdest(fW1, (F, D)), dbias=d_fb1)
+            pr.linear_dx(dHh, F, fW1, R, out=dX2, accumulate=True)
+            dZ2, dX1, d_clw, d_clb = pr.ln_bwd(dX2, dX2, R, Z2, X1, ls2, clw, R, p, seed, sid + 1, beta=clb, rows_map=trows)
             with fork(dZ2, ctx2):
                 d_cbo = _gdest(cbo, (D,), zero=True)
-                d_cWo = pr.linear_dw(dZ2, D, ctx2, D, Mt, D, D, out=_gdest(cWo, (D, D)), dbias=d_cbo)
-            dctx2 = pr.linear_dx(dZ2, D, cWo, Mt)
-            dQ = pr.empty((Mt, D), dev)
-            if pk is not None:
+                d_cWo = pr.linear_dw(dZ2, D, ctx2, D, R, D, D, out=_gdest(cWo, (D, D)), dbias=d_cbo)
+            dctx2 = pr.linear_dx(dZ2, D, cWo, R)
+            dQ = pr.empty((R, D), dev)
+            if toff is not None:
+                call("fira_attn_bwd_rows", _ptr(Q), D, _ptr(KV, i * 2 * D), ldkv, _ptr(KV, i * 2 * D + D), ldkv,
+                     _ptr(pk.ranges), _ptr(mem_mask), S, 0, _ptr(toff), R, _ptr(ctx2), _ptr(dctx2), D, _ptr(st2), _ptr(dQ), D,
+                     _ptr(dKV, i * 2 * D), ldkv, _ptr(dKV, i * 2 * D + D), ldkv, B, H, T, D // H, pr.code, st)
+            elif pk is not None:
                 call("fira_attn_packed_bwd", _ptr(Q), D, _ptr(KV, i * 2 * D), ldkv, _ptr(KV, i * 2 * D + D), ldkv,
                      _ptr(pk.ranges), Ms, _ptr(mem_mask), S, pk.chunks, _ptr(ctx2), _ptr(dctx2), D, _ptr(st2), _ptr(dQ), D,
                      _ptr(dKV, i * 2 * D), ldkv, _ptr(dKV, i * 2 * D + D), ldkv, B, H, T, D // H, pr.code, st)
@@ -657,21 +676,26 @@
                      _ptr(dKV, i * 2 * D + D), ldkv, B, H, T, S, D // H, pr.code, st)
             with fork(dQ, X1):
                 d_cbq = _gdest(cbq, (D,), zero=True)
-                d_cWq = pr.linear_dw(dQ, D, X1, D, Mt, D, D, out=_gdest(cWq, (D, D)), dbias=d_cbq)
-            pr.linear_dx(dQ, D, cWq, Mt, out=dX1, accumulate=True)
-            dZ1, dX0, d_slw, d_slb = pr.ln_bwd(dX1, dX1, Mt, Z1, X, ls1, slw, Mt, p, seed, sid + 0, beta=slb)
+                d_cWq = pr.linear_dw(dQ, D, X1, D, R, D, D, out=_gdest(cWq, (D, D)), dbias=d_cbq)
+            pr.linear_dx(dQ, D, cWq, R, out=dX1, accumulate=True)
+            dZ1, dX0, d_slw, d_slb = pr.ln_bwd(dX1, dX1, R, Z1, X, ls1, slw, R, p, seed, sid + 0, beta=slb, rows_map=trows)
             with fork(dZ1, ctx1):
                 d_sbo = _gdest(sbo, (D,), zero=True)
-                d_sWo = pr.linear_dw(dZ1, D, ctx1, D, Mt, D, D, out=_gdest(sWo, (D, D)), dbias=d_sbo)
-            dctx1 = pr.linear_dx(dZ1, D, sWo, Mt)
-            dQKV = pr.empty((Mt, 3 * D), dev)
-            call("fira_attn_bwd", _ptr(QKV), 3 * D, _ptr(QKV, D), 3 * D, _ptr(QKV, 2 * D), 3 * D, _ptr(tar_mask), 1,
-                 _ptr(ctx1), _ptr(dctx1), D, _ptr(st1), _ptr(dQKV), 3 * D, _ptr(dQKV, D), 3 * D, _ptr(dQKV, 2 * D), 3 * D,
-                 B, H, T, T, D // H, pr.code, st)
+                d_sWo = pr.linear_dw(dZ1, D, ctx1, D, R, D, D, out=_gdest(sWo, (D, D)), dbias=d_sbo)
+            dctx1 = pr.linear_dx(dZ1, D, sWo, R)
+            dQKV = pr.empty((R, 3 * D), dev)
+            if toff is not None:
+                call("fira_attn_bwd_rows", _ptr(QKV), 3 * D, _ptr(QKV, D), 3 * D, _ptr(QKV, 2 * D), 3 * D, None,
+                     _ptr(tar_mask), T, 1, _ptr(toff), R, _ptr(ctx1), _ptr(dctx1), D, _ptr(st1), _ptr(dQKV), 3 * D,
+                     _ptr(dQKV, D), 3 * D, _ptr(dQKV, 2 * D), 3 * D, B, H, T, D // H, pr.code, st)
+            else:
+                call("fira_attn_bwd", _ptr(QKV), 3 * D, _ptr(QKV, D), 3 * D, _ptr(QKV, 2 * D), 3 * D, _ptr(tar_mask), 1,
+                     _ptr(ctx1), _ptr(dctx1), D, _ptr(st1), _ptr(dQKV), 3 * D, _ptr(dQKV, D), 3 * D, _ptr(dQKV, 2 * D),
+                     3 * D, B, H, T, T, D // H, pr.code, st)
             with fork(dQKV, X):
                 d_bqkv = _gdest((sbq, sbk, sbv), (3 * D,), zero=True)
-                d_Wqkv = pr.linear_dw(dQKV, 3 * D, X, D, Mt, 3 * D, D, out=_gdest((sWq, sWk, sWv), (3 * D, D)), dbias=d_bqkv)
-            pr.linear_dx(dQKV, 3 * D, Wqkv, Mt, out=dX0, accumulate=True)
+                d_Wqkv = pr.linear_dw(dQKV, 3 * D, X, D, R, 3 * D, D, out=_gdest((sWq, sWk, sWv), (3 * D, D)), dbias=d_bqkv)
+            pr.linear_dx(dQKV, 3 * D, Wqkv, R, out=dX0, accumulate=True)
             grads[i * 26:(i + 1) * 26] = [
                 d_Wqkv[:D], d_bqkv[:D], d_Wqkv[D:2 * D], d_bqkv[D:2 * D], d_Wqkv[2 * D:], d_bqkv[2 * D:],
                 d_sWo, d_sbo, d_slw, d_slb,
@@ -691,7 +715,7 @@
             grads[i * 26 + 12], grads[i * 26 + 13] = d_Wkv[o:o + D], d_bkv[o:o + D]
             grads[i * 26 + 14], grads[i * 26 + 15] = d_Wkv[o + D:o + 2 * D], d_bkv[o + D:o + 2 * D]
         d_emb = _gdest(dec_emb, tuple(dec_emb.shape), zero=True)
-        call("fira_embed_rows_bwd", _ptr(tar), _ptr(dX), _ptr(d_emb), Mt, D, pr.code, st)
+        call("fira_embed_rows_bwd_rows", _ptr(tar), _ptr(trows), _ptr(dX), _ptr(d_emb), R, D, pr.code, st)
         fork.join()
         return (None, None, d_mem, None, None, None, d_emb, *grads)
 
diff --git a/fira_icse_b200/packed.py b/fira_icse_b200/packed.py
--- a/fira_icse_b200/packed.py
+++ b/fira_icse_b200/packed.py
@@ -12,16 +12,17 @@
     FIELDS = ("code", "mark", "pos", "sub", "ast", "off", "ranges", "mem_mask", "tar", "label", "tar_mask",
               "rowptr", "col", "val")
 
-    def __init__(self, B, Rc, Rs, Ra, S, T, nnz, chunks=4, Rv=None, **tensors):
+    def __init__(self, B, Rc, Rs, Ra, S, T, nnz, chunks=4, Rv=None, Rt=None, **tensors):
         self.B, self.Rc, self.Rs, self.Ra, self.S, self.T, self.nnz = B, Rc, Rs, Ra, S, T, nnz
         self.chunks = int(chunks)
         self.Rv = B * T if Rv is None else int(Rv)
+        self.Rt = B * T if Rt is None else int(Rt)
         for k in self.FIELDS:
             setattr(self, k, tensors[k])
 
     @property
     def shape_key(self):
-        return (self.B, self.Rc, self.Rs, self.Ra, self.S, self.chunks, self.Rv)
+        return (self.B, self.Rc, self.Rs, self.Ra, self.S, self.chunks, self.Rt, self.Rv)
 
     @property
     def rows(self):
@@ -33,7 +34,7 @@
 
     def to(self, device, non_blocking=True):
         t = {k: getattr(self, k).to(device, non_blocking=non_blocking) for k in self.FIELDS}
-        return PackedBatch(self.B, self.Rc, self.Rs, self.Ra, self.S, self.T, self.nnz, self.chunks, self.Rv, **t)
+        return PackedBatch(self.B, self.Rc, self.Rs, self.Ra, self.S, self.T, self.nnz, self.chunks, self.Rv, self.Rt, **t)
 
     def h2d_bytes(self):
         return sum(getattr(self, k).numel() * getattr(self, k).element_size() for k in self.FIELDS)
@@ -70,6 +71,11 @@
         lab = self.tab["tar_label"][np.asarray(index, dtype=np.int64), 1:]
         return int(np.count_nonzero((lab > 0) & (lab < vocab_size)))
 
+    def live_rows(self, index):
+        lab = self.tab["tar_label"][np.asarray(index, dtype=np.int64), 1:] != 0
+        last = lab.shape[1] - np.argmax(lab[:, ::-1], axis=1)
+        return int(np.where(lab.any(axis=1), last, 0).sum())
+
 
 class PackedSlot:
 
@@ -101,13 +107,17 @@
     need = tables.dims(index)
     if pad_dims is None:
         pad_dims = packed_needs(tables, index, vocab_size, buckets)
-    elif len(pad_dims) == 4:
-        pad_dims = tuple(pad_dims) + packed_needs(tables, index, vocab_size, buckets)[4:]
-    Rc, Rs, Ra, S, Rv = (int(x) for x in pad_dims)
+    elif len(pad_dims) < 6:
+        need_all = packed_needs(tables, index, vocab_size, buckets)
+        pad_dims = tuple(pad_dims) + need_all[len(pad_dims):]
+        pad_dims = pad_dims[:5] + (max(pad_dims[4], pad_dims[5]),)
+    Rc, Rs, Ra, S, Rv, Rt = (int(x) for x in pad_dims)
     if Rc > slot.cap[0] or Rs > slot.cap[1] or Ra > slot.cap[2] or S > slot.cap[3]:
         raise ValueError(f"packed batch {pad_dims} exceeds the staging capacity {slot.cap}")
     if Rv < tables.vocab_rows(index, vocab_size):
         raise ValueError(f"packed batch: Rv = {Rv} is below its vocabulary-label rows")
+    if Rt < max(Rv, tables.live_rows(index)):
+        raise ValueError(f"packed batch: Rt = {Rt} is below its live target rows or Rv = {Rv}")
     t = tables.tab
     pd = np.asarray((Rc, Rs, Ra, S), np.int32)
     nnz = np.zeros(1, np.int32)
@@ -121,7 +131,7 @@
               slot.val.data_ptr(), slot.edge_cap, nnz.ctypes.data)
     e, T = int(nnz[0]), tables.msg_len
     slot.batch = PackedBatch(
-        b, Rc, Rs, Ra, S, T, e, max(3, need[5]), min(Rv, b * T),
+        b, Rc, Rs, Ra, S, T, e, max(3, need[5]), min(Rv, b * T), min(Rt, b * T),
         code=slot.code[:Rc], mark=slot.mark[:Rc], pos=slot.pos[:Rc], sub=slot.sub[:Rs], ast=slot.ast[:Ra],
         off=slot.off[:3 * (b + 1)].view(3, b + 1), ranges=slot.ranges[:4 * b].view(b, 4),
         mem_mask=slot.mem_mask[:b * S].view(b, S), tar=slot.tar[:b * T].view(b, T), label=slot.label[:b * T].view(b, T),
@@ -132,8 +142,10 @@
 
 def packed_needs(tables, index, vocab_size, buckets=SEGMENT_BUCKETS):
     need = tables.dims(index)
-    return tuple(_round_up(need[i], buckets[i]) for i in range(4)) + \
-        (_round_up(tables.vocab_rows(index, vocab_size), VOCAB_ROW_BUCKET),)
+    cap = len(index) * tables.msg_len
+    Rv = min(_round_up(tables.vocab_rows(index, vocab_size), VOCAB_ROW_BUCKET), cap)
+    Rt = min(max(_round_up(tables.live_rows(index), VOCAB_ROW_BUCKET), Rv), cap)
+    return tuple(_round_up(need[i], buckets[i]) for i in range(4)) + (Rv, Rt)
 
 
 def pack_from_dataset(dataset, index, vocab_size, pin=False, pad_dims=None, buckets=SEGMENT_BUCKETS):
diff --git a/include/fira_b200.h b/include/fira_b200.h
--- a/include/fira_b200.h
+++ b/include/fira_b200.h
@@ -49,6 +49,8 @@
 int fira_embed_rows_fwd(const int* ids, const float* emb, const float* pos_table, void* out, long rows, int period,
                         int dim, int dtype, void* stream);
 int fira_embed_rows_bwd(const int* ids, const void* d_out, float* d_emb, long rows, int dim, int dtype, void* stream);
+int fira_embed_rows_bwd_rows(const int* ids, const int* rows_map, const void* d_out, float* d_emb, long rows, int dim,
+                             int dtype, void* stream);
 
 int fira_ln_residual_fwd(const void* z, const void* resid, const float* gamma, const float* beta, void* outA,
                          void* outB, long split, float* mean, float* rstd, long rows, int dim, float p_drop,
@@ -57,6 +59,11 @@
                          const float* mean, const float* rstd, const float* gamma, void* d_z, void* d_resid,
                          int d_resid_accum, float* d_gamma, float* d_beta, long rows, int dim, float p_drop,
                          uint64_t seed, const uint64_t* seed_ctr, uint32_t stream_id, int dtype, void* stream);
+int fira_ln_residual_bwd_rows(const void* d_outA, const void* d_outB, long split, const void* z, const void* resid,
+                              const float* mean, const float* rstd, const float* gamma, void* d_z, void* d_resid,
+                              int d_resid_accum, float* d_gamma, float* d_beta, const int* rows_map, long rows, int dim,
+                              float p_drop, uint64_t seed, const uint64_t* seed_ctr, uint32_t stream_id, int dtype,
+                              void* stream);
 
 int fira_comb_gate_fwd(const void* qk, long ld_qk, const float* vtab, const int* mark, void* out, long rows, int dim,
                        int d_head, float p_drop, uint64_t seed, const uint64_t* seed_ctr, uint32_t stream_id, int dtype, void* stream);
@@ -116,6 +123,10 @@
                          long kv_rows, const unsigned char* key_mask, int mask_pitch, int max_chunks, const void* ctx,
                          const void* d_ctx, long ldo, const float* stats, void* dq, long lddq, void* dk, long lddk,
                          void* dv, long lddv, int B, int H, int Lq, int d_head, int dtype, void* stream);
+int fira_attn_bwd_rows(const void* q, long ldq, const void* k, long ldk, const void* v, long ldv, const int* ranges,
+                       const unsigned char* key_mask, int mask_pitch, int causal, const int* qoff, long rows,
+                       const void* ctx, const void* d_ctx, long ldo, const float* stats, void* dq, long lddq, void* dk,
+                       long lddk, void* dv, long lddv, int B, int H, int Lq, int d_head, int dtype, void* stream);
 
 int fira_decoder_fwd(const int* tar, const float* dec_emb, const float* pos_table, const unsigned char* tar_mask,
                      const void* kv, long ldkv, const unsigned char* mem_mask, const int* ranges, int S,
@@ -123,6 +134,13 @@
                      float* ls1, void* x1, void* q, void* ctx2, float* st2, void* z2, float* ls2, void* x2, void* hh,
                      void* z3, float* ls3, int B, int T, float p_drop, uint64_t seed, const uint64_t* seed_ctr,
                      uint32_t stream_id, void* stream);
+int fira_decoder_fwd_rows(const int* tar, const float* dec_emb, const float* pos_table, const unsigned char* tar_mask,
+                          const void* kv, long ldkv, const unsigned char* mem_mask, const int* ranges, int S,
+                          const void* const* layer_ptrs, int L, void* X, void* out, void* qkv, void* ctx1, float* st1,
+                          void* z1, float* ls1, void* x1, void* q, void* ctx2, float* st2, void* z2, float* ls2,
+                          void* x2, void* hh, void* z3, float* ls3, const int* tlen, const int* toff, long R, int B,
+                          int T, float p_drop, uint64_t seed, const uint64_t* seed_ctr, uint32_t stream_id,
+                          void* stream);
 
 int fira_copy_scores_fwd(const void* src_proj, const void* tgt_proj, const float* w_res, const float* b_res,
                          const unsigned char* src_mask, const unsigned char* row_mask, float* scores,
@@ -147,6 +165,7 @@
                              unsigned char* row_active, long rows, int T_len, int V, int S, int dtype, void* stream);
 
 int fira_vocab_rows(const int* label, long rows, int V, int* vslot, int* vrows, int cap, void* stream);
+int fira_target_rows(const int* label, int B, int T, int* tlen, int* toff, int* trows, int cap, void* stream);
 int fira_gather_rows(const void* src, long ld_src, const int* idx, void* dst, long ld_dst, long n, int width, int dtype,
                      void* stream);
 int fira_pointer_mix_nll_fwd_rows(const void* logits, long ld_logits, const float* copy_scores, const float* gate_logits,
```

New measurement: 22300 (median of 6 runs). 5.5% higher.
